# pyranha-labs/hypergrep

Measured on AMD Instinct MI355X. Metric: GiB/s scanned (256 patterns, 32 GiB synthetic log per GPU, text resident in HBM), higher is better.
Workload: dtype u8

## Files before the change

### hypergrep_amd/csrc/hg_compile.cpp

```cpp
#include "hg_compile.h"
#include "hg_comb.h"
#include "hg_core.h"

#include <algorithm>
#include <array>
#include <bitset>
#include <cmath>
#include <cstdlib>
#include <cstring>
#include <map>
#include <memory>
#include <stdexcept>
#include <unordered_map>

namespace {

using ByteSet = std::bitset<256>;

constexpr int kThisExpression = -2;
struct CompileError : std::runtime_error {
  int index;
  explicit CompileError(const std::string &what, int index = kThisExpression) : std::runtime_error(what), index(index) {}
};

// ... 650 lines not shown
  }
  return 0;
}

struct Cond { uint32_t pos, tt; };
struct Frag {
  uint32_t nullable = 0;
  std::vector<Cond> first, last;
};
struct Edge { uint32_t p, q, tt; };

class Glushkov {
 public:
  std::vector<ByteSet> pos_class;
  std::vector<Edge> edges;

  Frag build(const Node &n) {
    switch (n.kind) {
      case Node::Empty: { Frag f; f.nullable = HG_TT_ALL; return f; }
      case Node::Assert: { Frag f; f.nullable = n.tt; return f; }
      case Node::Class: {
        if (pos_class.size() >= HG_HUGE_MAX_NODES) throw CompileError("pattern too large");
        uint32_t p = static_cast<uint32_t>(pos_class.size());
        pos_class.push_back(n.cls);
        Frag f;
        f.first.push_back({p, HG_TT_ALL});
        f.last.push_back({p, HG_TT_ALL});
        return f;
      }
      case Node::Cat: {
        Frag acc;
        acc.nullable = HG_TT_ALL;
        for (auto &k : n.kids) acc = cat(std::move(acc), build(*k));
        return acc;
      }
      case Node::Alt: {
        Frag acc = build(*n.kids[0]);
        for (size_t i = 1; i < n.kids.size(); i++) acc = alt(std::move(acc), build(*n.kids[i]));
        return acc;
      }
      case Node::Rep: {
        const Node &k = *n.kids[0];
        const bool strip = nullable_tt(k) == HG_TT_ALL;
        auto copy = [&]() {
          Frag f = build(k);
          if (strip) f.nullable = 0;
          return f;
        };
        const int mn = strip ? 0 : n.min;
        Frag acc;
        acc.nullable = HG_TT_ALL;
        for (int i = 0; i < mn; i++) acc = cat(std::move(acc), copy());
        if (n.max < 0) {
          Frag loop = copy();
          link(loop.last, loop.first);
          loop.nullable = HG_TT_ALL;
          acc = cat(std::move(acc), std::move(loop));
        } else if (n.max > mn) {
          Frag opt;
          opt.nullable = HG_TT_ALL;
          for (int i = mn; i < n.max; i++) {
            opt = cat(std::move(opt), copy());
            opt.nullable = HG_TT_ALL;
          }
          acc = cat(std::move(acc), std::move(opt));
        }
        return acc;
      }
    }
    return Frag();
  }

 private:
  void link(const std::vector<Cond> &from, const std::vector<Cond> &to) {
    if (edges.size() + from.size() * to.size() > HG_HUGE_MAX_EDGES) throw CompileError("pattern too large");
    for (auto &l : from)
      for (auto &f : to) {
        uint32_t tt = l.tt & f.tt;
        if (tt) edges.push_back({l.pos, f.pos, tt});
      }
  }
  Frag cat(Frag a, Frag b) {
    link(a.last, b.first);
    Frag r;
    r.nullable = a.nullable & b.nullable;
    r.first = std::move(a.first);
    if (a.nullable)
      for (auto &f : b.first)
        if (f.tt & a.nullable) r.first.push_back({f.pos, f.tt & a.nullable});
    r.last = std::move(b.last);
    if (b.nullable)
      for (auto &l : a.last)
        if (l.tt & b.nullable) r.last.push_back({l.pos, l.tt & b.nullable});
    return r;
  }
  static Frag alt(Frag a, Frag b) {
    Frag r = std::move(a);
    r.nullable |= b.nullable;
    r.first.insert(r.first.end(), b.first.begin(), b.first.end());
    r.last.insert(r.last.end(), b.last.begin(), b.last.end());
    return r;
  }
};

struct Lit {
  std::string bytes, cmask;
  bool operator<(const Lit &o) const { return std::tie(bytes, cmask) < std::tie(o.bytes, o.cmask); }
  bool operator==(const Lit &o) const { return bytes == o.bytes && cmask == o.cmask; }
};
using LitSet = std::vector<Lit>;
constexpr size_t MAX_EXACT = 16;
constexpr size_t MAX_EXACT_LEN = 96;

struct Info {
  bool exact = false;
  LitSet set;
  bool has_cover = false;
  LitSet cover;
  long lead = 0;
};
long add_len(long a, long b) {
  if (a < 0 || b < 0 || a + b > (1 << 20)) return -1;
  return a + b;
}

int byte_commonness(unsigned char b) {
  if (b == ' ') return 10;
  if (b >= 'a' && b <= 'z') return std::strchr("etaoinsrhl", b) ? 8 : 5;
  if (b >= '0' && b <= '9') return 6;
  if (std::strchr("=:-./_", b)) return 4;
  if (b >= 'A' && b <= 'Z') return 2;
  if (b > 32 && b < 127) return 2;
  return 1;
}
size_t min_len(const LitSet &s) {
  size_t m = SIZE_MAX;
  for (auto &l : s) m = std::min(m, l.bytes.size());
  return s.empty() ? 0 : m;
}
void dedupe(LitSet &s) {
  std::sort(s.begin(), s.end());
  s.erase(std::unique(s.begin(), s.end()), s.end());
}
bool better_cover(const LitSet &a, const LitSet &b) {
  size_t ma = std::min<size_t>(min_len(a), 16), mb = std::min<size_t>(min_len(b), 16);
  if (ma != mb) return ma > mb;
  if (a.size() != b.size()) return a.size() < b.size();
  return min_len(a) > min_len(b);
}
void offer(Info &info, const LitSet &cand, long lead) {
  if (cand.empty() || min_len(cand) == 0 || cand.size() > MAX_EXACT) return;
  if (!info.has_cover || better_cover(cand, info.cover)) {
    info.has_cover = true;
    info.cover = cand;
    info.lead = lead;
  }
}
bool cross(const LitSet &a, const LitSet &b, LitSet &out) {
  if (a.size() * b.size() > MAX_EXACT) return false;
  out.clear();
  for (auto &x : a)
    for (auto &y : b) {
      if (x.bytes.size() + y.bytes.size() > MAX_EXACT_LEN) return false;
      out.push_back({x.bytes + y.bytes, x.cmask + y.cmask});
    }
  dedupe(out);
  return true;
}

Info analyze(const Node &n) {
  Info r;
  switch (n.kind) {
    case Node::Empty: case Node::Assert:
      r.exact = true;
      r.set.push_back({"", ""});
      return r;
    case Node::Class: {
      size_t cnt = n.cls.count();
      ByteSet folded;
      for (int b = 0; b < 256; b++) if (n.cls[b]) folded.set((b >= 'A' && b <= 'Z') ? b + 32 : b);
      bool case_closed = true;
      for (int b = 'a'; b <= 'z'; b++) if (n.cls[b] != n.cls[b - 32]) case_closed = false;
      if (cnt <= 10 || (case_closed && folded.count() <= 10)) {
        r.exact = true;
        for (int b = 0; b < 256; b++) {
          if (!n.cls[b]) continue;
          if (b >= 'A' && b <= 'Z' && n.cls[b + 32]) continue;
          bool both = b >= 'a' && b <= 'z' && n.cls[b - 32];
          r.set.push_back({std::string(1, static_cast<char>(b)), std::string(1, static_cast<char>(both ? 0xDF : 0xFF))});
        }
      }
      return r;
    }
    case Node::Cat: {
      LitSet run{{"", ""}};
      bool all_exact = true;
      long before = 0;
      long run_lead = 0;
      auto flush = [&]() {
        offer(r, run, run_lead);
        run = LitSet{{"", ""}};
      };
      for (auto &k : n.kids) {
        Info ki = analyze(*k);
        const long after = add_len(before, max_match_len(*k));
        if (ki.has_cover) offer(r, ki.cover, add_len(before, ki.lead));
        if (ki.exact) {
          LitSet next;
          if (cross(run, ki.set, next)) run = std::move(next);
          else {
            all_exact = false;
            flush();
            run = ki.set;
            run_lead = before;
            if (run.size() > MAX_EXACT) { run = LitSet{{"", ""}}; run_lead = after; }
          }
        } else {
          all_exact = false;
          flush();
          run_lead = after;
        }
        before = after;
      }
      if (all_exact) { r.exact = true; r.set = run; }
      offer(r, run, run_lead);
      return r;
    }
    case Node::Alt: {
      bool all_exact = true, all_cover = true;
      LitSet uni, cov;
      long cov_lead = 0;
      for (auto &k : n.kids) {
        Info ki = analyze(*k);
        if (ki.exact) { uni.insert(uni.end(), ki.set.begin(), ki.set.end()); }
        else all_exact = false;
        const LitSet *c = ki.has_cover ? &ki.cover : (ki.exact && min_len(ki.set) > 0 ? &ki.set : nullptr);
        if (ki.exact && ki.has_cover && min_len(ki.set) > 0 && better_cover(ki.set, ki.cover)) c = &ki.set;
        if (c) {
          cov.insert(cov.end(), c->begin(), c->end());
          const long l = c == &ki.cover ? ki.lead : 0;
          cov_lead = (cov_lead < 0 || l < 0) ? -1 : std::max(cov_lead, l);
        }
        else all_cover = false;
      }
      dedupe(uni);
      dedupe(cov);
      if (all_exact && uni.size() <= MAX_EXACT) { r.exact = true; r.set = uni; }
      if (all_cover) offer(r, cov, cov_lead);
      if (r.exact) offer(r, r.set, 0);
      return r;
    }
    case Node::Rep: {
      Info ki = analyze(*n.kids[0]);
      if (ki.exact && n.min == n.max && n.min <= 64) {
        LitSet acc{{"", ""}};
        bool ok = true;
        for (int i = 0; i < n.min && ok; i++) {
          LitSet next;
          ok = cross(acc, ki.set, next);
          if (ok) acc = std::move(next);
        }
        if (ok) { r.exact = true; r.set = acc; offer(r, acc, 0); return r; }
      }
      if (n.min >= 1) {
        if (ki.has_cover) offer(r, ki.cover, ki.lead);
        if (ki.exact) {
          LitSet acc{{"", ""}};
          for (int i = 0; i < std::min(n.min, 32); i++) {
            LitSet next;
            if (!cross(acc, ki.set, next)) break;
            acc = std::move(next);
          }
          offer(r, acc, 0);
        }
      }
      return r;
    }
  }
  return r;
}

Lit clip(const Lit &l, size_t *offset = nullptr) {
  if (offset) *offset = 0;
  if (l.bytes.size() <= HG_FACTOR_MAX) return l;
  size_t best = 0;
  int best_score = INT32_MAX;
  for (size_t o = 0; o + HG_FACTOR_MAX <= l.bytes.size(); o++) {
    int s = 0;
    for (size_t i = 0; i < HG_FACTOR_MAX; i++) s += byte_commonness(static_cast<unsigned char>(l.bytes[o + i]));
    if (s < best_score) { best_score = s; best = o; }
  }
  if (offset) *offset = best;
  return {l.bytes.substr(best, HG_FACTOR_MAX), l.cmask.substr(best, HG_FACTOR_MAX)};
}

struct SampleStats {
  std::unordered_map<uint32_t, uint32_t> c4;
  std::unordered_map<uint64_t, uint32_t> c6;
  size_t dwords = 0;
};

int build_filter(HgDb &db, const SampleStats *stats, std::string *err) {
  db.windows.clear();
  std::vector<std::pair<uint32_t, HgWindow>> keyed;
  std::vector<uint32_t> next16_of;
  const uint32_t fold = db.fold_mask;
  const uint32_t wbytes = db.window_bytes, wmask = db.window_mask;
  std::unordered_map<uint32_t, uint32_t> contenders;
  for (uint32_t fi = 0; fi < db.nreal_factors; fi++) {
    const HgFactor &fct = db.factors[fi];
    std::vector<uint32_t> mine;
    for (uint32_t o = 0; o + wbytes <= fct.len; o++) {
      uint32_t v = 0;
      std::memcpy(&v, fct.lit + o, wbytes);
      mine.push_back((v | fold) & wmask);
    }
    std::sort(mine.begin(), mine.end());
    mine.erase(std::unique(mine.begin(), mine.end()), mine.end());
    for (uint32_t v : mine) contenders[v]++;
  }
  auto variants = [&](const HgFactor &fct, uint32_t o, std::vector<uint32_t> &out) {
    uint32_t v = 0;
    std::memcpy(&v, fct.lit + o, wbytes);
    out.assign(1, (v | fold) & wmask);
    if (fold) return;
    for (uint32_t b = 0; b < wbytes; b++)
      if ((fct.casebits >> (o + b)) & 1u) {
        const size_t have = out.size();
        for (size_t i = 0; i < have; i++) out.push_back(out[i] ^ (0x20u << (8 * b)));
      }
  };
  std::vector<uint32_t> vars;
  for (uint32_t fi = 0; fi < db.nreal_factors; fi++) {
    const HgFactor &fct = db.factors[fi];
    Lit l{std::string(reinterpret_cast<const char *>(fct.lit), fct.len), std::string(fct.len, '\xFF')};
    for (uint32_t b = 0; b < fct.len; b++) l.cmask[b] = static_cast<char>(hg_factor_cmask(fct, b));
    if (db.dense && fct.len < wbytes) {
      std::vector<uint32_t> seen;
      for (uint32_t last = 0; last < 256; last++) {
        uint32_t v = 0;
        std::memcpy(&v, fct.lit, fct.len);
        v = ((v | (last << 24)) | fold) & wmask;
        if (std::find(seen.begin(), seen.end(), v) != seen.end()) continue;
        seen.push_back(v);
        keyed.push_back({hg_hash_window(v), HgWindow{v, fi << 8}});
        next16_of.push_back(0);
      }
      continue;
    }
    const uint32_t step = db.dense ? db.dense : 4u;
    for (uint32_t res = 0; res < step; res++) {
      int best = -1;
      long best_cost = 0;
      uint32_t best_shared = 0;
      int best_sel = -1;
      for (uint32_t o = res; o + wbytes <= fct.len; o += step) {
        uint32_t v = 0;
        std::memcpy(&v, fct.lit + o, wbytes);
        v = (v | fold) & wmask;
        long cost = 0;
        if (stats) {
          variants(fct, o, vars);
          for (uint32_t x : vars) {
            auto it = stats->c4.find(x);
            cost += it == stats->c4.end() ? 0 : it->second;
          }
        }
        const uint32_t shared = contenders[v] > 1 ? contenders[v] : 0;
        int sel = 0;
        for (int j = static_cast<int>(o); j < static_cast<int>(o + wbytes); j++) sel += 11 - byte_commonness(static_cast<unsigned char>(l.bytes[j]));
        for (int j = std::max(static_cast<int>(o) - 4, 0); j < std::min<int>(o + 7, fct.len); j++)
          sel += (11 - byte_commonness(static_cast<unsigned char>(l.bytes[j]))) / 4;
        if (best < 0 || cost < best_cost || (cost == best_cost && (shared < best_shared || (shared == best_shared && sel > best_sel)))) {
          best = static_cast<int>(o);
          best_cost = cost;
          best_shared = shared;
          best_sel = sel;
        }
      }
      if (best < 0) continue;
      variants(fct, static_cast<uint32_t>(best), vars);
      for (uint32_t x : vars) {
        keyed.push_back({hg_hash_window(x), HgWindow{x, (fi << 8) | static_cast<uint32_t>(best)}});
        next16_of.push_back(0);
      }
    }
  }
  {
    std::vector<size_t> order(keyed.size());
    for (size_t i = 0; i < order.size(); i++) order[i] = i;
    std::stable_sort(order.begin(), order.end(), [&](size_t x, size_t y) { return keyed[x].first < keyed[y].first; });
    std::vector<std::pair<uint32_t, HgWindow>> k2;
    std::vector<uint32_t> n2;
    for (size_t i : order) { k2.push_back(keyed[i]); n2.push_back(next16_of[i]); }
    keyed.swap(k2);
    next16_of.swap(n2);
  }
  db.bucket_off.assign((1u << HG_HASH_BITS) + 1, 0);
  for (auto &kw : keyed) {
    db.bucket_off[kw.first + 1]++;
    db.windows.push_back(kw.second);
  }
  for (size_t i = 1; i < db.bucket_off.size(); i++) db.bucket_off[i] += db.bucket_off[i - 1];
  if (db.windows.empty()) db.windows.push_back(HgWindow{0, 0});

  {
    db.disc.assign(size_t(1) << HG_HASH_BITS, 0);
    std::vector<std::pair<uint32_t, HgWindow>> keyed2;
    for (size_t g0 = 0; g0 < keyed.size();) {
      size_t g1 = g0;
      while (g1 < keyed.size() && keyed[g1].first == keyed[g0].first) g1++;
      const uint32_t h = keyed[g0].first;
      int best_delta = 0;
      uint32_t best_sel = 0;
      size_t best_distinct = 1;
      auto key_of = [&](const HgWindow &w, int delta, uint32_t sel) {
        const HgFactor &fct = db.factors[w.factor_off >> 8];
        const int at = static_cast<int>(w.factor_off & 0xff) + delta;
        uint32_t v = 0;
        for (int b = 0; b < 4; b++)
          if ((sel >> b) & 1u) v |= static_cast<uint32_t>(fct.lit[at + b]) << (8 * b);
        return (v | fold) & hg_disc_bytes(sel);
      };
      if (g1 - g0 > 2) {
        for (int delta = -16; delta <= 28; delta += 4) {
          if (delta == 0) continue;
          uint32_t sel = 15;
          for (size_t e = g0; e < g1; e++) {
            const HgFactor &fct = db.factors[keyed[e].second.factor_off >> 8];
            const int at = static_cast<int>(keyed[e].second.factor_off & 0xff) + delta;
            for (int b = 0; b < 4; b++) {
              if (at + b < 0 || at + b >= static_cast<int>(fct.len)) sel &= ~(1u << b);
              else if (!fold && hg_factor_cmask(fct, at + b) != 0xFF) sel &= ~(1u << b);
            }
          }
          if (!sel) continue;
          std::vector<uint32_t> ks;
          for (size_t e = g0; e < g1; e++) ks.push_back(key_of(keyed[e].second, delta, sel));
          std::sort(ks.begin(), ks.end());
          const size_t distinct = static_cast<size_t>(std::unique(ks.begin(), ks.end()) - ks.begin());
          if (distinct > best_distinct || (distinct == best_distinct && distinct > 1 && std::abs(delta) < std::abs(best_delta))) {
            best_distinct = distinct;
            best_delta = delta;
            best_sel = sel;
          }
        }
      }
      db.disc[h] = static_cast<uint16_t>((static_cast<uint32_t>(best_delta) & 0xFFu) | (best_sel << 8));
      for (size_t e = g0; e < g1; e++)
        keyed2.push_back({hg_disc_bucket(h, best_sel ? key_of(keyed[e].second, best_delta, best_sel) : 0u), keyed[e].second});
      g0 = g1;
    }
    std::stable_sort(keyed2.begin(), keyed2.end(), [](const auto &x, const auto &y) { return x.first < y.first; });
    db.bucket_off2.assign((1u << HG_HASH_BITS) + 1, 0);
    db.windows2.clear();
    for (auto &kw : keyed2) {
      db.bucket_off2[kw.first + 1]++;
      db.windows2.push_back(kw.second);
    }
    for (size_t i = 1; i < db.bucket_off2.size(); i++) db.bucket_off2[i] += db.bucket_off2[i - 1];
    if (db.windows2.empty()) db.windows2.push_back(HgWindow{0, 0});
  }

  {
    std::vector<std::pair<uint32_t, uint32_t>> vf;
    for (auto &kw : keyed) vf.push_back({kw.second.value, kw.second.factor_off});
    std::sort(vf.begin(), vf.end());
    vf.erase(std::unique(vf.begin(), vf.end()), vf.end());
    size_t distinct = 0;
    for (size_t i = 0; i < vf.size(); i++) distinct += (i == 0 || vf[i].first != vf[i - 1].first) ? 1 : 0;
    uint32_t nbuckets = 16;
    while (static_cast<size_t>(nbuckets) * HG_WTAB_WAYS < 2 * distinct) nbuckets <<= 1;
    HgWinBucket empty;
    for (uint32_t k = 0; k < HG_WTAB_WAYS; k++) { empty.value[k] = 0; empty.factor_off[k] = HG_WTAB_EMPTY; }
    db.wtab.assign(nbuckets, empty);
    db.wtab_mask = nbuckets - 1;
    db.shared_windows = 0;
    for (size_t i = 0; i < vf.size();) {
      size_t j = i;
      while (j < vf.size() && vf[j].first == vf[i].first) j++;
      const uint32_t payload = j - i == 1 ? vf[i].second : HG_WTAB_SHARED;
      db.shared_windows += j - i == 1 ? 0 : 1;
      for (uint32_t b = hg_wtab_bucket(vf[i].first, db.wtab_mask);; b = (b + 1u) & db.wtab_mask) {
        bool placed_here = false;
        for (uint32_t k = 0; k < HG_WTAB_WAYS && !placed_here; k++)
          if (db.wtab[b].factor_off[k] == HG_WTAB_EMPTY) {
            db.wtab[b].value[k] = vf[i].first;
            db.wtab[b].factor_off[k] = payload;
            placed_here = true;
          }
        if (placed_here) break;
      }
      i = j;
    }
    db.wtab_first = (distinct > 0 && static_cast<size_t>(db.shared_windows) * 20 <= distinct) ? 1u : 0u;
  }

  std::vector<uint32_t> values;
  for (auto &kw : keyed) values.push_back(kw.second.value);
  std::sort(values.begin(), values.end());
  values.erase(std::unique(values.begin(), values.end()), values.end());
  bool placed = false;
  {
    std::vector<uint32_t> cand_weights;
    for (uint32_t i = 0; i < HG_SLOT_WEIGHT_NCHOICES; i++) {
      cand_weights.push_back(HG_SLOT_WEIGHT_CHOICES[i][0] & wmask);
      cand_weights.push_back(HG_SLOT_WEIGHT_CHOICES[i][1] & wmask);
    }
    auto slot_words = [&](uint32_t k, uint32_t weights, std::vector<uint32_t> &words) -> double {
      const uint32_t byte_mask = ((1u << k) - 1u) << 2;
      words.assign(size_t(1) << k, HG_FILTER_EMPTY);
      std::vector<uint8_t> used(size_t(1) << k, 0);
      for (uint32_t v : values) {
        const uint32_t sl = hg_slot(v, weights, byte_mask) >> 2, fp = hg_hash_window(v) & 0xFFFFu;
        uint32_t &w = words[sl];
        if (!used[sl]) {
          w = 0xFFFF0000u | fp;
          used[sl] = 1;
        } else {
          const uint32_t care = (w >> 16) & ~((w ^ fp) & 0xFFFFu);
          w = (care << 16) | (w & care);
        }
      }
      double fp_rate = 0;
      for (size_t sl = 0; sl < words.size(); sl++)
        if (used[sl]) fp_rate += std::ldexp(1.0, -static_cast<int>(__builtin_popcount(words[sl] >> 16)));
      return fp_rate / static_cast<double>(words.size());
    };
    double best_rate = 1e9;
    uint32_t best_k = 0, best_w = 0;
    for (uint32_t k = HG_FILTER_MIN_LOG2; k <= HG_FILTER_MAX_LOG2 && !placed; k++) {
      if (values.size() > (size_t(1) << k)) continue;
      double k_rate = 1e9;
      uint32_t k_w = 0;
      for (uint32_t weights : cand_weights) {
        std::vector<uint32_t> words;
        const double rate = slot_words(k, weights, words);
        if (rate < k_rate) { k_rate = rate; k_w = weights; }
      }
      if (k_rate < best_rate) { best_rate = k_rate; best_k = k; best_w = k_w; }
      if (k_rate <= (k <= 12 ? 5e-4 : 3e-4)) {
        best_rate = k_rate;
        best_k = k;
        best_w = k_w;
        placed = true;
      }
    }
    if (!placed && best_k && best_rate <= 2e-3 && values.size() * 100 <= (size_t(1) << HG_FILTER_MAX_LOG2) * 45) placed = true;
    if (placed) {
      const uint32_t k = best_k, wa = best_w;
      const uint32_t byte_mask = ((1u << k) - 1u) << 2;
      slot_words(k, wa, db.filter);
      db.ext.assign(size_t(1) << k, HgSlotInfo{});
      db.filter_log2 = k;
      db.weights_a = wa;
      db.weights_b = wa;
      auto merge = [](uint32_t &val, uint32_t &mask, uint32_t v2, uint32_t m2) {
        uint32_t keep = 0;
        for (int b = 0; b < 4; b++) {
          uint32_t bm = 0xFFu << (8 * b);
          if ((mask & bm) && (m2 & bm) && ((val ^ v2) & bm) == 0) keep |= bm;
        }
        mask = keep;
        val &= keep;
      };
      for (size_t wi = 0; wi < keyed.size(); wi++) {
        const HgWindow &w = keyed[wi].second;
        const HgFactor &f = db.factors[w.factor_off >> 8];
        const int o = static_cast<int>(w.factor_off & 0xff);
        uint32_t pv = 0, pm = 0, nv = 0, nm = 0;
        for (int b = 0; b < 4; b++) {
          int jp = o - 4 + b, jn = o + static_cast<int>(wbytes) + b;
          if (jp >= 0) { pv |= static_cast<uint32_t>(f.lit[jp]) << (8 * b); pm |= 0xFFu << (8 * b); }
          if (jn < static_cast<int>(f.len)) { nv |= static_cast<uint32_t>(f.lit[jn]) << (8 * b); nm |= 0xFFu << (8 * b); }
        }
        pv = (pv | fold) & pm;
        nv = (nv | fold) & nm;
        if (!fold) {
          for (int b = 0; b < 4; b++) {
            int jp = o - 4 + b, jn = o + static_cast<int>(wbytes) + b;
            if (jp >= 0 && hg_factor_cmask(f, jp) != 0xFF) { pm &= ~(0xFFu << (8 * b)); pv &= pm; }
            if (jn < static_cast<int>(f.len) && hg_factor_cmask(f, jn) != 0xFF) { nm &= ~(0xFFu << (8 * b)); nv &= nm; }
          }
        }
        HgSlotInfo &info = db.ext[hg_slot(w.value, wa, byte_mask) >> 2];
        HgFilterExt *x = nullptr;
        bool fresh = false;
        for (uint32_t i = 0; i < info.nvalues; i++)
          if (info.value[i] == w.value) x = &info.cond[i];
        if (!x && info.nvalues < 2) {
          info.value[info.nvalues] = w.value;
          x = &info.cond[info.nvalues++];
          fresh = true;
        }
        if (!x) {
          x = &info.rest;
          fresh = !info.many;
          info.many = 1;
        }
        if (fresh) {
          *x = HgFilterExt{pv, pm, nv, nm};
        } else {
          merge(x->pv, x->pm, pv, pm);
          merge(x->nv, x->nm, nv, nm);
        }
      }
    }
  }
  db.filter_wide = 0;
  if (!placed && db.dense) {
    if (err) *err = "too many literal windows for byte-aligned probing";
    return -5;
  }
  if (!placed) {
    for (uint32_t attempt = 0; attempt < 3 * HG_SLOT_WEIGHT_NCHOICES && !placed; attempt++) {
      const uint32_t k = 13 + attempt / HG_SLOT_WEIGHT_NCHOICES;
      const uint32_t wa = HG_SLOT_WEIGHT_CHOICES[attempt % HG_SLOT_WEIGHT_NCHOICES][0], wb = HG_SLOT_WEIGHT_CHOICES[attempt % HG_SLOT_WEIGHT_NCHOICES][1];
      const size_t cells = size_t(2) << k;
      if (values.size() * 100 > cells * 85) continue;
      const uint32_t byte_mask = ((1u << k) - 1u) << 2;
      struct WEntry { uint32_t sa, sb; uint16_t fp; };
      std::vector<WEntry> entries;
      {
        std::vector<std::array<uint32_t, 3>> keys;
        for (uint32_t v : values) {
          const uint32_t a = hg_dot4(v, wa), b = hg_dot4(v, wb);
          const uint32_t sa = hg_slot_wide(a, b, byte_mask) >> 2, sb = hg_slot_wide(b, a, byte_mask) >> 2;
          keys.push_back({std::min(sa, sb), std::max(sa, sb), hg_hash_window(v) & 0xFFFFu});
        }
        std::sort(keys.begin(), keys.end());
        keys.erase(std::unique(keys.begin(), keys.end()), keys.end());
        for (auto &key : keys) entries.push_back({key[0], key[1], static_cast<uint16_t>(key[2])});
      }
      std::vector<int32_t> owner(cells, -1);
      uint64_t rng = 0x9E3779B97F4A7C15ull;
      placed = true;
      for (size_t e = 0; e < entries.size() && placed; e++) {
        int32_t cur = static_cast<int32_t>(e);
        bool ok = false;
        for (int kick = 0; kick < 8000 && !ok; kick++) {
          const uint32_t cand[4] = {entries[cur].sa * 2, entries[cur].sa * 2 + 1, entries[cur].sb * 2, entries[cur].sb * 2 + 1};
          for (uint32_t cell : cand)
            if (owner[cell] < 0) { owner[cell] = cur; ok = true; break; }
          if (ok) break;
          rng = rng * 6364136223846793005ull + 1442695040888963407ull;
          std::swap(cur, owner[cand[(rng >> 33) & 3]]);
        }
        if (!ok) placed = false;
      }
      if (!placed) continue;
      db.filter.assign(size_t(1) << k, HG_FILTER_EMPTY);
      for (size_t cell = 0; cell < cells; cell++) {
        if (owner[cell] < 0) continue;
        uint32_t &word = db.filter[cell >> 1];
        const uint32_t fp = entries[owner[cell]].fp;
        word = (cell & 1) ? ((word & 0x0000FFFFu) | (fp << 16)) : ((word & 0xFFFF0000u) | fp);
      }
      db.ext.assign(1, HgSlotInfo{});
      db.filter_log2 = k;
      db.filter_wide = 1;
      db.weights_a = wa;
      db.weights_b = wb;
    }
  }
  if (!placed) {
    if (err) *err = "too many distinct literal windows for the LDS filter (more than ~55 000)";
    return -4;
  }
  return 0;
}

struct CompileKnobs {
  bool no_ctx_groups = std::getenv("HG_NO_CTX_GROUPS") != nullptr;
  bool no_case_expand = std::getenv("HG_NO_CASE_EXPAND") != nullptr;
};

struct CombProgram {
  std::vector<uint32_t> ops;
  std::vector<uint32_t> prog;
};

CombProgram parse_combination(const std::string &text) {
  CombProgram out;
  std::vector<char> stack;
  auto prec = [](char c) { return c == '!' ? 3 : c == '&' ? 2 : c == '|' ? 1 : 0; };
  auto emit = [&](char c) { out.prog.push_back(c == '!' ? HG_COMB_NOT : c == '&' ? HG_COMB_AND : HG_COMB_OR); };
  bool want_operand = true;
  bool any = false;
  for (size_t i = 0; i < text.size();) {
    const char c = text[i];
    if (c == ' ' || c == '\t' || c == '\n' || c == '\r' || c == '\f' || c == '\v') {
      i++;
      continue;
    }
    any = true;
    if (c >= '0' && c <= '9') {
      if (!want_operand) throw CompileError("combination: two operands without an operator between them");
      uint64_t v = 0;
      for (; i < text.size() && text[i] >= '0' && text[i] <= '9'; i++) {
        v = v * 10 + static_cast<uint64_t>(text[i] - '0');
        if (v > 0xFFFFFFFFull) throw CompileError("combination: operand id above 4294967295 (UINT32_MAX)");
      }
      const uint32_t id = static_cast<uint32_t>(v);
      auto it = std::find(out.ops.begin(), out.ops.end(), id);
      if (it == out.ops.end()) {
        if (out.ops.size() == HG_COMB_MAX_OPERANDS)
          throw CompileError("combination: more than " + std::to_string(HG_COMB_MAX_OPERANDS) + " distinct operands (the limit is " +
                             std::to_string(HG_COMB_MAX_OPERANDS) + ")");
        out.ops.push_back(id);
        it = out.ops.end() - 1;
      }
      out.prog.push_back(static_cast<uint32_t>(it - out.ops.begin()));
      want_operand = false;
      continue;
    }
    i++;
    if (c == '!' || c == '(') {
      if (!want_operand) throw CompileError(std::string("combination: '") + c + "' after an operand (missing operator)");
      stack.push_back(c);
    } else if (c == '&' || c == '|') {
      if (want_operand) throw CompileError(std::string("combination: dangling operator '") + c + "'");
      while (!stack.empty() && stack.back() != '(' && prec(stack.back()) >= prec(c)) {
        emit(stack.back());
        stack.pop_back();
      }
      stack.push_back(c);
      want_operand = true;
    } else if (c == ')') {
      if (want_operand) throw CompileError(stack.empty() || stack.back() != '(' ? "combination: dangling operator before ')'" : "combination: empty parentheses");
      while (!stack.empty() && stack.back() != '(') {
        emit(stack.back());
        stack.pop_back();
      }
      if (stack.empty()) throw CompileError("combination: unbalanced parentheses (')' without '(')");
      stack.pop_back();
    } else {
      throw CompileError(std::string("combination: unexpected character '") + c + "' (operands are decimal report ids, operators ! & | and parentheses)");
    }
  }
  if (!any) throw CompileError("combination: empty formula");
  if (want_operand) throw CompileError("combination: dangling operator at the end");
  while (!stack.empty()) {
    if (stack.back() == '(') throw CompileError("combination: unbalanced parentheses ('(' without ')')");
    emit(stack.back());
    stack.pop_back();
  }
  long depth = 0, most = 0;
  for (uint32_t op : out.prog) {
    depth += op < HG_COMB_NOT ? 1 : op == HG_COMB_NOT ? 0 : -1;
    most = std::max(most, depth);
  }
  if (most > 64) throw CompileError("combination: more than 64 values on the evaluation stack (parentheses nested too deeply)");
  return out;
}

void build_slow_groups(HgDb &db, const CompileKnobs &knobs) {
  db.groups.clear();
  db.nslow_grouped = 0;
  const bool mixed = !knobs.no_ctx_groups;
  struct Bin { std::vector<uint32_t> members; uint32_t nodes = 0; bool ctx = false; };
  std::vector<Bin> bins;
  for (int pass = 0; pass < 2; pass++) {
    for (uint32_t j = 0; j < db.nslow_fast; j++) {
      const HgPattern &p = db.patterns[db.slow[j]];
      if (p.nw != 1 || p.nnodes == 0 || (p.simple != 0) != (pass == 1)) continue;
      if (pass == 0 && !mixed) continue;
      Bin *home = nullptr;
      for (Bin &b : bins)
        if (b.nodes + p.nnodes <= 32 && b.members.size() < HG_GROUP_MAX_MEMBERS) { home = &b; break; }
      if (!home) { bins.emplace_back(); home = &bins.back(); home->ctx = pass == 0; }
      home->members.push_back(db.slow[j]);
      home->nodes += p.nnodes;
    }
  }
  std::vector<uint32_t> grouped;
  for (const Bin &b : bins) {
    if (b.members.size() < 2) continue;
    HgSlowGroup g{};
    db.pool.resize((db.pool.size() + 3) & ~static_cast<size_t>(3), 0);
    g.reach_off = static_cast<uint32_t>(db.pool.size());
    db.pool.resize(db.pool.size() + 256, 0);
    g.follow_off = static_cast<uint32_t>(db.pool.size());
    db.pool.resize(db.pool.size() + b.nodes, 0);
    if (b.ctx) {
      g.ctx_off = static_cast<uint32_t>(db.pool.size());
      db.pool.resize(db.pool.size() + 36, 0);
    }
    g.nnodes = b.nodes;
    g.nmembers = static_cast<uint32_t>(b.members.size());
    bool unbounded = false;
    uint32_t shift = 0;
    for (uint32_t m = 0; m < g.nmembers; m++) {
      const HgPattern &p = db.patterns[b.members[m]];
      const uint32_t all = (p.nnodes == 32 ? 0xFFFFFFFFu : ((1u << p.nnodes) - 1u)) << shift;
      g.member[m] = b.members[m];
      g.acc[m] = b.ctx ? all : p.acc_all << shift;
      g.acc_all |= g.acc[m];
      g.init_word |= db.pool[p.init_off] << shift;
      if (p.single) g.single_mask |= 1u << m;
      if (p.max_len == 0) unbounded = true;
      g.max_len = std::max(g.max_len, p.max_len);
      for (uint32_t c = 0; c < 256; c++) db.pool[g.reach_off + c] |= db.pool[p.reach_off + c] << shift;
      for (uint32_t v = 0; v < p.nnodes; v++) db.pool[g.follow_off + shift + v] = db.pool[p.follow_off + v] << shift;
      if (b.ctx) {
        for (uint32_t i = 0; i < 16; i++) db.pool[g.ctx_off + i] |= db.pool[p.amask_off + i] << shift;
        for (uint32_t i = 0; i < 20; i++) db.pool[g.ctx_off + 16 + i] |= db.pool[p.acc_off + i] << shift;
      }
      shift += p.nnodes;
      grouped.push_back(b.members[m]);
    }
    if (unbounded) g.max_len = 0;
    db.groups.push_back(g);
  }
  if (grouped.empty()) return;
  std::vector<uint32_t> rest_fast, rest_slow;
  for (uint32_t j = 0; j < db.slow.size(); j++) {
    const uint32_t pi = db.slow[j];
    if (std::find(grouped.begin(), grouped.end(), pi) != grouped.end()) continue;
    (j < db.nslow_fast ? rest_fast : rest_slow).push_back(pi);
  }
  db.slow = grouped;
  db.slow.insert(db.slow.end(), rest_fast.begin(), rest_fast.end());
  db.slow.insert(db.slow.end(), rest_slow.begin(), rest_slow.end());
  db.nslow_grouped = static_cast<uint32_t>(grouped.size());
}

uint32_t alloc(HgDb &db, size_t words) {
  if (db.pool.size() + words > 0xFFFF0000ull) throw CompileError("pattern set too large");
  const uint32_t off = static_cast<uint32_t>(db.pool.size());
  db.pool.resize(db.pool.size() + words, 0);
  return off;
}
void setbit(HgDb &db, uint32_t base, uint32_t node) { db.pool[base + node / 32] |= 1u << (node % 32); }

HgPattern compile_combination(HgDb &db, const char *expr, uint32_t f, uint32_t id, CombProgram &program) {
  if (!expr || !expr[0]) throw CompileError("empty expression");
  db.exprs.push_back(expr);
  program = parse_combination(expr);
  if (hg_comb_eval(program.prog.data(), static_cast<uint32_t>(program.prog.size()), 0))
    throw CompileError("combination is true when none of its operands has matched: such combinations report at the end of the data, which is not supported");
  HgPattern p{};
  p.id = id;
  p.flags = f & (HG_FLAG_COMBINATION | HG_FLAG_SINGLEMATCH | HG_FLAG_QUIET);
  p.single = (f & HG_FLAG_SINGLEMATCH) ? 1 : 0;
  p.tier = HG_TIER_COMB;
  db.ncomb++;
  return p;
}

struct Automaton {
  NodeP root;
  Glushkov g;
  std::vector<Cond> first;
  std::vector<std::pair<uint32_t, uint32_t>> nodes;
  std::vector<uint32_t> node_lo;
  std::vector<uint32_t> last_tt;
  uint32_t nn = 0, nw = 1;
  uint32_t node(uint32_t pos, uint32_t tt) const {
    return static_cast<uint32_t>(std::lower_bound(nodes.begin(), nodes.end(), std::make_pair(pos, tt)) - nodes.begin());
  }
};

void index_nodes(Automaton &a, std::vector<Cond> first, const std::vector<Cond> &last) {
  std::vector<Edge> &edges = a.g.edges;
  std::sort(edges.begin(), edges.end(), [](const Edge &x, const Edge &y) { return x.p != y.p ? x.p < y.p : x.q < y.q; });
  size_t ne = 0;
  for (size_t i = 0; i < edges.size(); i++) {
    if (ne && edges[ne - 1].p == edges[i].p && edges[ne - 1].q == edges[i].q) edges[ne - 1].tt |= edges[i].tt;
    else edges[ne++] = edges[i];
  }
  edges.resize(ne);
  a.nodes.reserve(first.size() + edges.size());
  for (auto &c : first) a.nodes.push_back({c.pos, c.tt});
  for (auto &e : edges) a.nodes.push_back({e.q, e.tt});
  std::sort(a.nodes.begin(), a.nodes.end());
  a.nodes.erase(std::unique(a.nodes.begin(), a.nodes.end()), a.nodes.end());
  if (a.nodes.size() > HG_HUGE_MAX_NODES) throw CompileError("pattern too large");
  const uint32_t npos = static_cast<uint32_t>(a.g.pos_class.size());
  a.node_lo.assign(npos + 1, 0);
  for (auto &nd : a.nodes) a.node_lo[nd.first + 1]++;
  for (uint32_t q = 0; q < npos; q++) a.node_lo[q + 1] += a.node_lo[q];
  a.last_tt.assign(npos, 0);
  for (auto &l : last) a.last_tt[l.pos] |= l.tt;
  a.first = std::move(first);
  a.nn = static_cast<uint32_t>(a.nodes.size());
  a.nw = a.nn ? (a.nn + 31) / 32 : 1;
}

Automaton build_automaton(const std::string &text, uint32_t flags) {
  Automaton a;
  a.root = Parser(text, flags).parse();
  check_embedded_anchors(*a.root, false, false);
  if (program_size(*a.root) > HG_HUGE_MAX_PROGRAM) throw CompileError("pattern too large");
  Frag top = a.g.build(*a.root);
  if (a.g.pos_class.empty() && !top.nullable) throw CompileError("expression matches nothing");
  if (nullable_syntactic(*a.root)) throw CompileError("expression can match the empty string (HS_FLAG_ALLOWEMPTY is not supported)");
  index_nodes(a, std::move(top.first), top.last);
  return a;
}

constexpr uint64_t HG_EXT_FLAGS_KNOWN = HS_EXT_FLAG_MIN_OFFSET | HS_EXT_FLAG_MAX_OFFSET | HS_EXT_FLAG_MIN_LENGTH | HS_EXT_FLAG_EDIT_DISTANCE |
                                        HS_EXT_FLAG_HAMMING_DISTANCE;
constexpr uint32_t HG_EXT_MAX_DISTANCE = 16;

long min_match_len(const Node &n) {
  const long kCap = 1 << 20;
  switch (n.kind) {
    case Node::Empty:
    case Node::Assert: return 0;
// ... 345 lines not shown
    for (size_t j = 0; j <= k; j++) {
      const size_t lo = len * j / (k + 1), hi = len * (j + 1) / (k + 1);
      if (hi - lo < HG_DENSE_MIN_FACTOR) return Cover{};
      cover.lits.push_back(clip(Lit{l.bytes.substr(lo, hi - lo), l.cmask.substr(lo, hi - lo)}));
    }
  }
  dedupe(cover.lits);
  if (cover.lits.size() > MAX_EXACT) return Cover{};
  return cover;
}

void emit_som_follow(HgDb &db, HgPattern &p, bool som) {
  if (p.nw > HG_MAX_W)
    throw CompileError("HS_FLAG_SOM_LEFTMOST needs an automaton of at most " + std::to_string(HG_MAX_NODES) + " nodes (HG_MAX_NODES); this expression has " +
                       std::to_string(p.nnodes));
  p.som_follow_off = alloc(db, static_cast<size_t>(p.nnodes) * p.nw);
  for (uint32_t v = 0; v < p.nnodes; v++)
    for (uint32_t w = 0; w < p.nw; w++)
      for (uint32_t x = db.pool[p.follow_off + v * p.nw + w]; x; x &= x - 1) setbit(db, p.som_follow_off + (w * 32 + hg_ctz(x)) * p.nw, v);
  if (som) db.nsom++;
}

void link_som_ids(HgDb &db) {
  if (!db.nsom) return;
  std::map<uint32_t, uint32_t> last;
  std::map<uint32_t, uint32_t> first_plain;
  for (uint32_t i = 0; i < db.patterns.size(); i++) {
    HgPattern &p = db.patterns[i];
    if (!(p.flags & HG_FLAG_SOM_LEFTMOST)) {
      first_plain.emplace(p.id, i);
      continue;
    }
    auto it = last.find(p.id);
    if (it == last.end()) {
      p.som_next = i;
    } else {
      p.som_next = db.patterns[it->second].som_next;
      db.patterns[it->second].som_next = i;
    }
    last[p.id] = i;
  }
  for (auto &kv : last) {
    auto it = first_plain.find(kv.first);
    if (it != first_plain.end())
      throw CompileError("expressions with report id " + std::to_string(kv.first) + " must all carry HS_FLAG_SOM_LEFTMOST, or none of them",
                         static_cast<int>(std::max(it->second, kv.second)));
  }
}

void link_combinations(HgDb &db, const std::map<uint32_t, CombProgram> &programs) {
  if (!db.comb_pass()) return;
  std::map<uint32_t, std::pair<uint32_t, bool>> plain;
  std::map<uint32_t, uint32_t> comb_of;
  for (uint32_t i = 0; i < db.patterns.size(); i++) {
    const HgPattern &p = db.patterns[i];
    if (p.tier == HG_TIER_COMB) continue;
    const bool quiet = (p.flags & HG_FLAG_QUIET) != 0;
    auto ins = plain.emplace(p.id, std::make_pair(i, quiet));
    if (!ins.second && ins.first->second.second != quiet)
      throw CompileError("expressions with report id " + std::to_string(p.id) + " must all carry HS_FLAG_QUIET, or none of them", static_cast<int>(i));
  }
  for (uint32_t i = 0; i < db.patterns.size(); i++) {
    const HgPattern &p = db.patterns[i];
    if (p.tier != HG_TIER_COMB) continue;
    if (plain.count(p.id) || !comb_of.emplace(p.id, i).second)
      throw CompileError("combination report id " + std::to_string(p.id) + " is shared with another expression (a combination's id must be unique)",
                         static_cast<int>(i));
  }
  std::vector<std::pair<uint32_t, uint32_t>> feed;
  for (auto &kv : programs) {
    const uint32_t i = kv.first;
    const int at = static_cast<int>(i);
    const HgPattern &p = db.patterns[i];
    const CombProgram &cp = kv.second;
    for (uint32_t id : cp.ops) {
      if (id == p.id) throw CompileError("combination refers to its own report id " + std::to_string(id), at);
      if (comb_of.count(id))
        throw CompileError("combination refers to report id " + std::to_string(id) + " of another combination (nested combinations are not supported)", at);
      if (!plain.count(id)) throw CompileError("combination refers to report id " + std::to_string(id) + ", which no expression in the set has", at);
    }
    if (p.flags & HG_FLAG_QUIET) continue;
    HgComb c{};
    c.id = p.id;
    c.pattern = i;
    c.single = p.single;
    c.nops = static_cast<uint32_t>(cp.ops.size());
    c.ops_off = static_cast<uint32_t>(db.comb_words.size());
    db.comb_words.insert(db.comb_words.end(), cp.ops.begin(), cp.ops.end());
    c.prog_off = static_cast<uint32_t>(db.comb_words.size());
    c.prog_len = static_cast<uint32_t>(cp.prog.size());
    db.comb_words.insert(db.comb_words.end(), cp.prog.begin(), cp.prog.end());
    for (uint32_t id : cp.ops) feed.emplace_back(id, static_cast<uint32_t>(db.combs.size()));
    db.combs.push_back(c);
  }
  std::sort(feed.begin(), feed.end());
  for (auto &f : feed) db.comb_feed.push_back(f.first);
  for (auto &f : feed) db.comb_feed.push_back(f.second);
}

int assign_tiers(HgDb &db, const std::vector<Cover> &covers, const CompileKnobs &knobs, uint32_t min_factor, uint32_t dense,
                 uint32_t window_bytes, std::string *err) {
  db.dense = dense;
  db.window_bytes = window_bytes;
  db.window_mask = window_bytes == 4 ? 0xFFFFFFFFu : 0x00FFFFFFu;
  db.weights_c = HG_HASH_WEIGHTS & db.window_mask;
  db.slow.clear();
  db.factors.clear();
  db.fold_mask = 0;
  size_t ncaseless = 0;
  for (uint32_t m = 0; m < HG_CONFIRM_MODES; m++) db.n_confirm_mode[m] = 0;
  for (uint32_t i = 0; i < db.patterns.size(); i++) {
    HgPattern &p = db.patterns[i];
    if (p.tier == HG_TIER_COMB) continue;
    const LitSet &lits = covers[i].lits;
    const bool fast = !lits.empty() && min_len(lits) >= min_factor;
    p.tier = fast ? 0 : 1;
    p.literal_only = (fast && covers[i].literal_only) ? 1 : 0;
    if (fast) {
      db.n_confirm_mode[hg_confirm_mode(p)]++;
      for (auto &l : lits) {
        bool caseless = false;
        for (unsigned char m : l.cmask) caseless = caseless || m != 0xFF;
        ncaseless += caseless ? 1 : 0;
      }
    } else {
      db.slow.push_back(i);
    }
  }
  if (ncaseless) {
    const bool expand = !dense && !knobs.no_case_expand && ncaseless <= 64;
    db.fold_mask = expand ? 0u : 0x20202020u;
  }
  auto two_words = [&](uint32_t pi) { return db.patterns[pi].nw <= 2; };
  auto not_huge = [&](uint32_t pi) { return db.patterns[pi].nw <= HG_MAX_W; };
  std::stable_partition(db.slow.begin(), db.slow.end(), not_huge);
  std::stable_partition(db.slow.begin(), db.slow.end(), two_words);
  db.nslow_fast = static_cast<uint32_t>(std::count_if(db.slow.begin(), db.slow.end(), two_words));
  db.nslow_huge = static_cast<uint32_t>(db.slow.size() - std::count_if(db.slow.begin(), db.slow.end(), not_huge));
  build_slow_groups(db, knobs);
  uint32_t rank_in_mode[HG_CONFIRM_MODES] = {};
  for (uint32_t i = 0; i < db.patterns.size(); i++) {
    if (db.patterns[i].tier != 0) continue;
    const uint32_t mode = hg_confirm_mode(db.patterns[i]), rank = rank_in_mode[mode]++;
    for (auto &l : covers[i].lits) {
      HgFactor fct{};
      fct.pattern = i;
      fct.len = static_cast<uint32_t>(l.bytes.size());
      fct.mode = mode;
      fct.mode_rank = rank;
      std::memcpy(fct.lit, l.bytes.data(), fct.len);
      for (uint32_t b = 0; b < fct.len; b++)
        if (static_cast<unsigned char>(l.cmask[b]) != 0xFF) fct.casebits |= 1u << b;
      fct.id = db.patterns[i].id;
      db.factors.push_back(fct);
    }
  }
  db.nreal_factors = static_cast<uint32_t>(db.factors.size());
  if (db.factors.empty()) db.factors.push_back(HgFactor{});
  return build_filter(db, nullptr, err);
}

void choose_windows(HgDb &db, const std::vector<Cover> &covers, const CompileKnobs &knobs) {
  std::string msg;
  auto assign = [&](size_t min_factor, uint32_t dense, uint32_t window_bytes) {
    return assign_tiers(db, covers, knobs, static_cast<uint32_t>(min_factor), dense, window_bytes, &msg);
  };
  size_t shortest = SIZE_MAX;
  for (const Cover &c : covers) {
    const size_t m = c.lits.empty() ? 0 : min_len(c.lits);
    if (m >= HG_DENSE_MIN_FACTOR && m < HG_FAST_MIN_FACTOR) shortest = std::min(shortest, m);
  }
  int rc = -5;
  if (shortest != SIZE_MAX) {
    size_t set_shortest = SIZE_MAX;
    for (const Cover &c : covers)
      if (!c.lits.empty() && min_len(c.lits) >= shortest) set_shortest = std::min(set_shortest, min_len(c.lits));
    const uint32_t step = set_shortest >= HG_WINDOW_BYTES + 1 ? 2u : 1u;
    rc = assign(shortest, step, HG_WINDOW_BYTES);
    if (rc == -5 && step == 2) rc = assign(shortest, 1, HG_WINDOW_BYTES);
    if (rc == -5 && shortest < HG_WINDOW_BYTES) rc = assign(shortest, 1, HG_WINDOW_BYTES - 1);
    if (rc == -5 && shortest < HG_WINDOW_BYTES) rc = assign(HG_WINDOW_BYTES, 1, HG_WINDOW_BYTES);
  }
  if (rc == -5) rc = assign(HG_FAST_MIN_FACTOR, 0, HG_WINDOW_BYTES);
  if (rc != 0) throw CompileError(msg, -1);
}

}

int hgc_compile(const char *const *exprs, const unsigned *flags, const unsigned *ids, unsigned n, HgDb **out,
               std::string *err, int *bad_index) {
  return hgc_compile_ext(exprs, flags, ids, nullptr, n, out, err, bad_index);
}

int hgc_compile_ext(const char *const *exprs, const unsigned *flags, const unsigned *ids, const hs_expr_ext_t *const *ext, unsigned n,
                    HgDb **out, std::string *err, int *bad_index) {
  if (bad_index) *bad_index = -1;
  if (out) *out = nullptr;
  if (!exprs || !out || n == 0) {
    if (err) *err = "invalid arguments: at least one expression is required";
    return -1;
  }
  const CompileKnobs knobs;
  auto db = std::make_unique<HgDb>();
  int at = -1;
  try {
    if (n > HG_MAX_PATTERNS) throw CompileError("too many expressions (limit 16777216)", -1);
    std::vector<Cover> covers(n);
    std::map<uint32_t, CombProgram> programs;
    std::map<uint32_t, std::pair<uint32_t, uint32_t>> bounds;
    std::map<uint32_t, uint32_t> min_lengths;
    for (at = 0; at < static_cast<int>(n); at++) {
      const uint32_t f = flags ? flags[at] : 0, id = ids ? ids[at] : 0;
      if (f & ~HG_FLAGS_SUPPORTED) throw CompileError("unsupported flag bits");
      const hs_expr_ext_t *x = (ext && ext[at] && ext[at]->flags) ? ext[at] : nullptr;
      if (x) check_ext_fields(*x, f);
      if (f & HG_FLAG_COMBINATION) {
        db->patterns.push_back(compile_combination(*db, exprs[at], f, id, programs[at]));
        db->max_id = std::max(db->max_id, id);
        continue;
      }
      if ((f & HG_FLAG_SOM_LEFTMOST) && (f & HG_FLAG_SINGLEMATCH))
        throw CompileError("HS_FLAG_SOM_LEFTMOST cannot be combined with HS_FLAG_SINGLEMATCH");
      if (!exprs[at] || !exprs[at][0]) throw CompileError("empty expression");
      db->exprs.push_back(exprs[at]);
      Automaton a = build_automaton(db->exprs.back(), f);
      const bool edit = x && (x->flags & HS_EXT_FLAG_EDIT_DISTANCE);
      const uint32_t k = !x ? 0u : edit ? x->edit_distance : ((x->flags & HS_EXT_FLAG_HAMMING_DISTANCE) ? x->hamming_distance : 0u);
      std::pair<uint32_t, uint32_t> bound{0u, HG_BOUND_NONE};
      uint32_t min_length = 0;
      if (x) bound = ext_bounds(*x, check_ext_width(*x, k, edit, min_match_len(*a.root), max_match_len(*a.root), a, &min_length));
      if (bound.first || bound.second != HG_BOUND_NONE) bounds[at] = bound;
      if (min_length) min_lengths[at] = min_length;
      if (k) a = expand_approx(a, k, edit, f);
      HgPattern p{};
      p.id = id;
      p.flags = f;
      p.nnodes = a.nn;
      p.nw = a.nw;
      p.single = (f & HG_FLAG_SINGLEMATCH) && !bound.first && !min_length ? 1 : 0;
      if (a.nw > HG_MAX_W) emit_huge_tables(*db, a, p);
      else emit_dense_tables(*db, a, p);
      set_simple_flags(*db, p);
      covers[at] = k ? approx_cover(*a.root, k, p) : literal_cover(*a.root, p);
      const long ml = max_match_len(*a.root);
      p.max_len = ml > 0 ? static_cast<uint32_t>(ml + (edit ? k : 0u)) : 0;
      if ((f & HG_FLAG_SOM_LEFTMOST) || min_length) emit_som_follow(*db, p, (f & HG_FLAG_SOM_LEFTMOST) != 0);
      if (f & HG_FLAG_QUIET) db->nquiet++;
      db->max_id = std::max(db->max_id, id);
      db->patterns.push_back(p);
    }
    at = -1;
    if (!bounds.empty()) {
      db->bounds.resize(2 * static_cast<size_t>(n));
      for (uint32_t i = 0; i < n; i++) {
        auto it = bounds.find(i);
        db->bounds[2 * i] = it == bounds.end() ? 0u : it->second.first;
        db->bounds[2 * i + 1] = it == bounds.end() ? HG_BOUND_NONE : it->second.second;
      }
    }
    if (!min_lengths.empty()) {
      db->min_lengths.assign(n, 0u);
      for (auto &kv : min_lengths) db->min_lengths[kv.first] = kv.second;
    }
    link_som_ids(*db);
    link_combinations(*db, programs);
    choose_windows(*db, covers, knobs);
  } catch (const CompileError &e) {
    if (err) *err = e.what();
    if (bad_index) *bad_index = e.index == kThisExpression ? at : e.index;
    return -4;
  } catch (const std::bad_alloc &) {
    if (err) *err = "out of memory";
    if (bad_index) *bad_index = at;
    return -2;
  }
  *out = db.release();
  return 0;
}

int hgc_tune(const HgDb *db, const uint8_t *sample, size_t nbytes, HgDb **out, std::string *err) {
  if (out) *out = nullptr;
  if (!db || !out || (!sample && nbytes)) return -1;
  SampleStats st;
  const uint32_t fold = db->fold_mask;
  for (size_t p = 0; p + 4 <= nbytes; p += db->dense ? db->dense : 4) {
    uint32_t w, nx = 0;
    std::memcpy(&w, sample + p, 4);
    if (p + 8 <= nbytes) std::memcpy(&nx, sample + p + 4, 4);
    w = (w | fold) & db->window_mask;
    nx |= fold;
    st.c4[w]++;
    st.c6[static_cast<uint64_t>(w) | (static_cast<uint64_t>(nx & 0xFFFFu) << 32)]++;
  }
  st.dwords = nbytes / 4;
  std::unique_ptr<HgDb> copy;
  try {
    copy = std::make_unique<HgDb>(*db);
  } catch (const std::bad_alloc &) {
    if (err) *err = "out of memory";
    return -2;
  }
  int rc = build_filter(*copy, &st, err);
  if (rc != 0) return rc;
  copy->tuned = true;
  *out = copy.release();
  return 0;
}

void hgc_free(HgDb *db) { delete db; }
```

### hypergrep_amd/csrc/hg_compile.h

```cpp
#pragma once
#include <cstdint>
#include <string>
#include <vector>

#include "../../include/hypergrep_amd.h"
#include "hg_core.h"
#include "hg_db.h"

struct HgDb {
  std::vector<HgPattern> patterns;
  std::vector<uint32_t> pool;
  std::vector<HgFactor> factors;
  uint32_t nreal_factors = 0;
  std::vector<HgWindow> windows;
  std::vector<uint32_t> bucket_off;
  std::vector<uint16_t> disc;
  std::vector<uint32_t> bucket_off2;
  std::vector<HgWindow> windows2;
  std::vector<HgWinBucket> wtab;
  uint32_t wtab_mask = 0;
  uint32_t shared_windows = 0;
  uint32_t wtab_first = 0;
  std::vector<uint32_t> filter;
  uint32_t filter_log2 = HG_FILTER_MIN_LOG2;
  uint32_t filter_wide = 0;
  uint32_t window_bytes = HG_WINDOW_BYTES;
  uint32_t window_mask = HG_WINDOW_MASK;
  uint32_t weights_c = HG_HASH_WEIGHTS;
  uint32_t dense = 0;
  uint32_t weights_a = HG_SLOT_WEIGHT_CHOICES[0][0], weights_b = HG_SLOT_WEIGHT_CHOICES[0][1];
  std::vector<HgSlotInfo> ext;
  std::vector<uint32_t> slow;
  uint32_t nslow_fast = 0;
  std::vector<HgSlowGroup> groups;
  uint32_t nslow_grouped = 0;
  uint32_t fold_mask = 0;
  uint32_t max_nw = 1;
  uint32_t nhuge = 0;
  uint32_t huge_max_nw = 0;
  uint32_t huge_stage_words = 0;
  uint32_t nslow_huge = 0;
  uint32_t max_id = 0;
  uint32_t nsom = 0;
  uint32_t ncomb = 0, nquiet = 0;
  std::vector<HgComb> combs;
  std::vector<uint32_t> comb_words;
  std::vector<uint32_t> comb_feed;
  bool comb_pass() const { return ncomb || nquiet; }
  std::vector<uint32_t> bounds;
  std::vector<uint32_t> min_lengths;
  uint32_t n_confirm_mode[HG_CONFIRM_MODES] = {};
  std::vector<std::string> exprs;
  bool tuned = false;
};

int hgc_tune(const HgDb *db, const uint8_t *sample, size_t nbytes, HgDb **out, std::string *err);


int hgc_compile(const char *const *exprs, const unsigned *flags, const unsigned *ids, unsigned n, HgDb **out,
               std::string *err, int *bad_index);
int hgc_compile_ext(const char *const *exprs, const unsigned *flags, const unsigned *ids, const hs_expr_ext_t *const *ext, unsigned n,
                    HgDb **out, std::string *err, int *bad_index);
void hgc_free(HgDb *db);
```

### hypergrep_amd/csrc/hg_db.h

```cpp
#pragma once
#include <cstdint>

#if defined(__HIPCC__)
#define HG_HD __host__ __device__ __forceinline__
#else
#define HG_HD inline
#endif

constexpr uint32_t HG_FLAG_CASELESS = 1, HG_FLAG_DOTALL = 2, HG_FLAG_MULTILINE = 4, HG_FLAG_SINGLEMATCH = 8;
constexpr uint32_t HG_FLAG_SOM_LEFTMOST = 256;
constexpr uint32_t HG_FLAG_COMBINATION = 512, HG_FLAG_QUIET = 1024;
constexpr uint32_t HG_FLAGS_SUPPORTED = 15 | HG_FLAG_SOM_LEFTMOST | HG_FLAG_COMBINATION | HG_FLAG_QUIET;

enum : uint32_t { HG_PC_START = 0, HG_PC_NL = 1, HG_PC_WORD = 2, HG_PC_OTHER = 3 };
enum : uint32_t { HG_NC_NL = 0, HG_NC_NLFINAL = 1, HG_NC_WORD = 2, HG_NC_OTHER = 3, HG_NC_END = 4 };
constexpr uint32_t HG_TT_ALL = (1u << 20) - 1;

constexpr uint32_t HG_MAX_NODES = 1024;
constexpr uint32_t HG_MAX_W = HG_MAX_NODES / 32;
constexpr uint32_t HG_HUGE_MAX_PROGRAM = 400000;
constexpr uint32_t HG_HUGE_MAX_NODES = 1u << 19;
constexpr uint32_t HG_HUGE_STAGE_MAX = 12288;
constexpr uint32_t HG_HUGE_MAX_EDGES = 1u << 22;
constexpr uint32_t HG_MAX_PATTERNS = 1u << 24;
constexpr uint32_t HG_ALWAYS_ON_FAST_MAX_LEN = 64;
constexpr uint32_t HG_FACTOR_MAX = 32;
constexpr uint32_t HG_WINDOW_BYTES = 4;
constexpr uint32_t HG_WINDOW_MASK = HG_WINDOW_BYTES == 4 ? 0xFFFFFFFFu : 0x00FFFFFFu;
constexpr uint32_t HG_FAST_MIN_FACTOR = HG_WINDOW_BYTES + 3;
constexpr uint32_t HG_DENSE_MIN_FACTOR = HG_WINDOW_BYTES - 1;
constexpr uint32_t HG_HASH_BITS = 18;
constexpr uint32_t HG_TOP_WEIGHT_MASK = HG_WINDOW_BYTES == 4 ? 0xFFFFFFFFu : 0x00FFFFFFu;
constexpr uint32_t HG_HASH_WEIGHTS = 0xfbf1efe9u & HG_TOP_WEIGHT_MASK;
constexpr uint32_t HG_SLOT_WEIGHT_CHOICES[][2] = {
    {0x2cec94fcu & HG_TOP_WEIGHT_MASK, 0xbc34f474u & HG_TOP_WEIGHT_MASK},
    {0x74d43cb4u & HG_TOP_WEIGHT_MASK, 0xe40c9c5cu & HG_TOP_WEIGHT_MASK},
    {0xa41cf86cu & HG_TOP_WEIGHT_MASK, 0x54c4247cu & HG_TOP_WEIGHT_MASK},
    {0xdc4484f4u & HG_TOP_WEIGHT_MASK, 0x1cac6cccu & HG_TOP_WEIGHT_MASK},
};
constexpr uint32_t HG_SLOT_WEIGHT_NCHOICES = 4;
constexpr uint32_t HG_FILTER_MIN_LOG2 = 11, HG_FILTER_MAX_LOG2 = 15;
constexpr uint32_t HG_FILTER_EMPTY = 0xFFFFFFFFu;

struct HgHugeHeader {
  uint32_t cls_off;
  uint32_t ncls;
  uint32_t smask_off;
  uint32_t xsrc_off;
  uint32_t xrank_off;
  uint32_t xlist_off;
  uint32_t xt_off;
  uint32_t ctxfree;
  uint32_t init_hi;
  uint32_t nsources, nranges;
  uint32_t reserved[5];
};
static_assert(sizeof(HgHugeHeader) == 64, "HgHugeHeader layout");

struct HgPattern {
  uint32_t id;
  uint32_t single;
  uint32_t max_len;
  uint32_t lit_lead;
  uint32_t flags;
  uint32_t nnodes;
  uint32_t nw;
  uint32_t reach_off;
  uint32_t follow_off;
  uint32_t init_off;
  uint32_t amask_off;
  uint32_t acc_off;
  uint32_t tier;
  uint32_t simple;
  uint32_t acc_all;
  uint32_t init_word;
  uint32_t literal_only;
  uint32_t som_follow_off;
  uint32_t som_next;
  uint32_t reserved;
};
static_assert(sizeof(HgPattern) == 80, "HgPattern layout");
HG_HD bool hg_report_single(const HgPattern &p) { return (p.flags & HG_FLAG_SINGLEMATCH) != 0; }

constexpr uint32_t HG_TIER_COMB = 2;

constexpr uint32_t HG_COMB_MAX_OPERANDS = 64;
constexpr uint32_t HG_COMB_NOT = 64, HG_COMB_AND = 65, HG_COMB_OR = 66;
struct HgComb {
  uint32_t id;
  uint32_t pattern;
  uint32_t single;
  uint32_t nops;
  uint32_t ops_off;
  uint32_t prog_off;
  uint32_t prog_len;
  uint32_t reserved;
};
static_assert(sizeof(HgComb) == 32, "HgComb layout");

struct HgFactor {
  uint32_t pattern;
  uint32_t len;
  uint32_t mode;
  uint32_t mode_rank;
  uint8_t lit[HG_FACTOR_MAX];
  uint32_t casebits;
  uint32_t id;
  uint32_t reserved[2];
};
static_assert(sizeof(HgFactor) == 64, "HgFactor layout");
HG_HD uint32_t hg_factor_cmask(const HgFactor &f, uint32_t b) { return ((f.casebits >> b) & 1u) ? 0xDFu : 0xFFu; }
HG_HD uint32_t hg_factor_mask_dword(uint32_t casebits, uint32_t len, uint32_t j) {
  const uint32_t nib = (casebits >> (4u * j)) & 15u;
  const uint32_t spread = (nib & 1u) | ((nib & 2u) << 7) | ((nib & 4u) << 14) | ((nib & 8u) << 21);
  const uint32_t m = ~(spread << 5);
  const uint32_t valid = len > 4u * j ? len - 4u * j : 0u;
  return valid >= 4u ? m : (m & ((1u << (8u * valid)) - 1u));
}

struct HgWinBucket {
  uint32_t value[4];
  uint32_t factor_off[4];
};
static_assert(sizeof(HgWinBucket) == 32, "HgWinBucket layout");
constexpr uint32_t HG_WTAB_WAYS = 4, HG_WTAB_EMPTY = 0xFFFFFFFFu, HG_WTAB_SHARED = 0xFFFFFFFEu;
HG_HD uint32_t hg_wtab_bucket(uint32_t folded, uint32_t bucket_mask) { return ((folded * 0x9E3779B1u) >> 9) & bucket_mask; }
HG_HD uint32_t hg_wtab_find(const HgWinBucket *tab, uint32_t bucket_mask, uint32_t folded) {
  for (uint32_t b = hg_wtab_bucket(folded, bucket_mask);; b = (b + 1u) & bucket_mask) {
    const HgWinBucket &e = tab[b];
    for (uint32_t k = 0; k < HG_WTAB_WAYS; k++) {
      if (e.factor_off[k] == HG_WTAB_EMPTY) return HG_WTAB_EMPTY;
      if (e.value[k] == folded) return e.factor_off[k];
    }
  }
}

struct HgWindow {
  uint32_t value;
  uint32_t factor_off;
};

constexpr uint32_t HG_GROUP_MAX_MEMBERS = 8;
struct HgSlowGroup {
  uint32_t reach_off;
  uint32_t follow_off;
  uint32_t nnodes, init_word, acc_all;
  uint32_t max_len;
  uint32_t nmembers;
  uint32_t single_mask;
  uint32_t member[HG_GROUP_MAX_MEMBERS];
  uint32_t acc[HG_GROUP_MAX_MEMBERS];
  uint32_t ctx_off;
  uint32_t reserved;
};
static_assert(sizeof(HgSlowGroup) == 104, "HgSlowGroup layout");

HG_HD uint32_t hg_dot4(uint32_t v, uint32_t w) {
#if defined(__HIP_DEVICE_COMPILE__)
  return __builtin_amdgcn_udot4(v, w, 0u, false);
#else
  return (v & 0xff) * (w & 0xff) + ((v >> 8) & 0xff) * ((w >> 8) & 0xff) + ((v >> 16) & 0xff) * ((w >> 16) & 0xff) + (v >> 24) * (w >> 24);
#endif
}
HG_HD uint32_t hg_hash_window(uint32_t folded) { return hg_dot4(folded, HG_HASH_WEIGHTS); }
HG_HD uint32_t hg_slot(uint32_t folded, uint32_t weights, uint32_t byte_mask) { return hg_dot4(folded, weights) & byte_mask; }
HG_HD bool hg_slot_match(uint32_t slot_word, uint32_t hash_c) { return (hash_c & (slot_word >> 16)) == (slot_word & 0xFFFFu); }
HG_HD uint32_t hg_slot_wide(uint32_t sum_x, uint32_t sum_y, uint32_t byte_mask) { return (sum_x + (sum_y << 8)) & byte_mask; }

struct HgFilterExt {
  uint32_t pv, pm;
  uint32_t nv, nm;
};
HG_HD bool hg_ext_pass(const HgFilterExt &e, uint32_t prev_folded, uint32_t next_folded) {
  return (((prev_folded ^ e.pv) & e.pm) | ((next_folded ^ e.nv) & e.nm)) == 0;
}

constexpr uint32_t HG_DISC_WEIGHTS_1 = 0xc5a36b1du, HG_DISC_WEIGHTS_2 = 0x3b9d47e1u;
HG_HD uint32_t hg_disc_bytes(uint32_t sel4) {
  return ((sel4 & 1u) ? 0xFFu : 0u) | ((sel4 & 2u) ? 0xFF00u : 0u) | ((sel4 & 4u) ? 0xFF0000u : 0u) | ((sel4 & 8u) ? 0xFF000000u : 0u);
}
HG_HD uint32_t hg_disc_bucket(uint32_t h, uint32_t masked_dword) {
  return (h ^ (hg_dot4(masked_dword, HG_DISC_WEIGHTS_1) + (hg_dot4(masked_dword, HG_DISC_WEIGHTS_2) << 7))) & ((1u << HG_HASH_BITS) - 1u);
}

struct HgSlotInfo {
  uint32_t value[2];
  uint32_t nvalues;
  uint32_t many;
  HgFilterExt cond[2];
  HgFilterExt rest;
};
static_assert(sizeof(HgSlotInfo) == 64, "HgSlotInfo layout");
HG_HD bool hg_slot_pass(const HgSlotInfo &s, uint32_t folded, uint32_t prev_folded, uint32_t next_folded, uint32_t pm_keep, uint32_t nm_keep) {
  HgFilterExt e;
  if (s.nvalues > 0 && s.value[0] == folded) e = s.cond[0];
  else if (s.nvalues > 1 && s.value[1] == folded) e = s.cond[1];
  else if (s.many) e = s.rest;
  else return false;
  e.pm &= pm_keep;
  e.nm &= nm_keep;
  return hg_ext_pass(e, prev_folded, next_folded);
}

HG_HD bool hg_is_word(uint32_t b) {
  return (b - '0' < 10u) || ((b | 0x20) - 'a' < 26u) || b == '_';
}
```

### hypergrep_amd/csrc/hg_engine.h

```cpp
#pragma once
#include <hip/hip_runtime.h>

#include <memory>
#include <string>

#include "../../include/hypergrep_amd.h"
#include "hg_compile.h"
#include "hg_core.h"
#include "hg_invert.h"
#include "hg_post.h"

#ifndef HG_STREAM_WG_WAVES
#define HG_STREAM_WG_WAVES 8
#endif
constexpr uint32_t HG_STREAM_WG_WAVES_DEFAULT = HG_STREAM_WG_WAVES;

constexpr uint32_t HG_CONFIRM_SPLIT = 4;
constexpr uint32_t HG_DEFER_SHARDS = 64;

struct HgDeferred {
  uint64_t pos;
  uint32_t pattern;
  uint32_t rank;
};
enum { HG_ST_MINLEN_KEPT = 16, HG_ST_FIN_TOTAL = 24, HG_ST_SELECTED = 28, HG_ST_FINAL = 32, HG_ST_WORDS = 36, HG_ST_ZERO_WORDS = 32,
       HG_ST_BLOCK_DONE = 40 };
enum { HG_CNT_CANDS = 0, HG_CNT_HITS = 1, HG_CNT_CAND_NEED = 2, HG_CNT_HIT_NEED = 3, HG_CNT_DEFER_NEED = 4,
       HG_CNT_HITS_WRAPPED = 5,
       HG_CNT_JOIN_TILES = 6,
       HG_CNT_WORDS = 8,
       HG_CNT_CURSOR0 = 64,
       HG_CNT_CURSORS = 64,
       HG_ST_ALLOC_WORDS = 128 };
constexpr uint32_t HG_STREAM_GRAB = 2 * HG_STREAM_WG_WAVES_DEFAULT;

constexpr uint32_t HG_FIN_MAX_BUCKETS = 1u << 22;
constexpr uint32_t HG_FIN_BUCKET_CAP = 4096;
constexpr uint32_t HG_FIN_MEDIUM_CAP = 512;

#ifndef HG_CONFIRM_THREADS
#define HG_CONFIRM_THREADS 128
#endif



struct HgStreamArgs {
  const uint8_t *text;
  uint64_t nbytes, tile_begin, tile_end;
  HgDbView db;
  const uint32_t *filter;
  const HgSlotInfo *ext;
  HgTileSum *sums;
  HgCand *cands;
  uint32_t *seg_count;
  uint32_t cand_seg_cap, filter_log2;
  uint32_t weights_a, weights_b;
  uint32_t filter_wide;
  uint32_t dense;
  uint32_t weights_c;
  uint32_t alone;
  uint32_t cursor_slot;
  uint32_t *counters;
};

struct HgConfirmArgs {
  const uint8_t *text;
  uint64_t nbytes, tile_begin, tile_end, bs1;
  HgDbView db;
  const HgTileSum *sums;
  const HgTileBase *bases;
  const HgCand *cands;
  const uint32_t *seg_count;
  HgHit *hits;
  HgHitAux *aux;
  HgHit *tmp_hits;
  HgHitAux *tmp_aux;
  HgDeferred *deferred;
  uint32_t *defer_count;
  uint32_t list_of_mode[HG_CONFIRM_MODES];
  uint32_t mode_present[HG_CONFIRM_MODES];
  uint32_t *always_count;
  uint32_t always_list_cap;
  uint32_t list_spread[HG_CONFIRM_MODES];
  uint32_t cand_seg_cap, hit_cap, hit_seg_cap, defer_shard_cap;
  uint32_t join_seg0, join_seg_cap;
  uint32_t hit_direct;
  uint32_t bucket_shift, bucket_cap;
  uint32_t *bucket_fill;
  uint32_t *counters;
  uint64_t own_lo, own_hi;
};
constexpr uint32_t HG_BLOCK_SMALL_POOL = 10240;
constexpr uint32_t HG_BLOCK_SLICED_MAX = 2047;
constexpr uint32_t HG_BLOCK_SLICED_WORDS = 64;
constexpr uint32_t HG_BLOCK_SMALL_MAX = 8192;
constexpr uint32_t HG_BLOCK_SMALL_SEG = 1024;
inline uint32_t hg_block_small_grouping(uint32_t npatterns, uint32_t *ppw) {
  *ppw = npatterns <= 32u * 64u ? 32u : 256u;
  return (npatterns + *ppw - 1) / *ppw;
}
constexpr uint32_t HG_HIT_REL_SHIFT = 40;
constexpr uint32_t HG_HIT_SINGLE_BIT = 0x80000000u;

struct HgScanOutput {
  uint64_t n_hits;
  uint64_t n_pieces;
  uint64_t n_cands;
  uint64_t n_raw_hits;
  const HgHit *d_hits;
  const HgHitAux *d_aux;
  float ms_stream;
  float ms_total;
  uint32_t reruns;
  uint32_t stream_launches;
  uint32_t joiner_launches;
  uint64_t joiner_tiles;
  const uint32_t *d_from;
  float ms_invert;
};

hipError_t hg_som_launch(const uint8_t *text, const HgHit *hits, const HgHitAux *aux, uint64_t n, const HgPattern *patterns, const uint32_t *pool, uint32_t max_nw,
                         const uint32_t *min_lengths, uint32_t *from, hipStream_t stream);
hipError_t hg_minlen_launch(const uint8_t *text, const HgHit *hits, const HgHitAux *aux, uint32_t n, const HgPattern *patterns, const uint32_t *pool, uint32_t max_nw,
                            const uint32_t *min_lengths, HgHit *out_hits, HgHitAux *out_aux, uint32_t *count, hipStream_t stream);

struct HgCombArgs {
  const HgHit *hits;
  const HgHitAux *aux;
  uint64_t n;
  const HgPattern *patterns;
  const HgComb *combs;
  const uint32_t *words;
  const uint32_t *feed;
  uint32_t nfeed;
  uint32_t *count;
  const uint64_t *pos;
  HgHit *out_hits;
  HgHitAux *out_aux;
};
hipError_t hg_comb_launch(const HgCombArgs &a, bool emit, hipStream_t stream);

hipError_t hg_invert_launch(const HgInvertArgs &a, bool write, uint32_t num_cus, hipStream_t stream);

struct HgEngineKnobs {
  uint64_t fin_target = 48;
  bool no_bucket_finalize = false;
  uint64_t chunk_tiles = 0;
  uint32_t max_chunks = 0;
  std::vector<double> chunk_weights;
  long stream_wgs_per_cu = 0;
  long joiner = -1;
  bool joiner_ahead = false;
  bool no_early_finalize = false;
  uint32_t confirm_mode_mask = 0x1F;
  long confirm_blocks_per_cu = 0;
  uint64_t hit_limit = 0;
  uint64_t cand_limit = 0;
  bool verbose = false;
  static HgEngineKnobs from_env();
};

class HgScanner {
 public:
  static int create(std::shared_ptr<const HgDb> db, int device, HgScanner **out, std::string *err);
  const std::shared_ptr<const HgDb> &database() const { return db_; }
  ~HgScanner();
  int scan(const void *d_text, uint64_t nbytes, int buffer_size, uint64_t line_base, hipStream_t stream, HgScanOutput *out, bool invert = false);
  int scan_block(const void *d_text, uint64_t nbytes, hipStream_t stream, HgScanOutput *out);
  uint32_t launch_block_small(const uint8_t *h_text, uint32_t nbytes, hipStream_t stream, HgHit *h_out, uint32_t *h_counts, uint32_t *h_flag, uint32_t seq);
  const std::string &last_error() const { return err_; }
  int device() const { return device_; }
  const HgDbView &view() const { return view_; }

 private:
  HgScanner() = default;
  int init();
  int ensure(uint64_t nbytes);
  int alloc_cands(uint64_t n);
  int alloc_hits(uint64_t n);
  int scan_impl(const void *d_text, uint64_t nbytes, int buffer_size, uint64_t line_base, bool block_mode, bool invert, hipStream_t stream, HgScanOutput *out);
  struct PassRange {
    uint64_t tile_lo, tile_hi, cs0, piece0, own_lo, own_hi;
    bool last;
  };
  int scan_segments(const uint8_t *text, uint64_t nbytes, uint64_t bs1, uint64_t line_base, hipStream_t stream, HgScanOutput *out, uint32_t nsegments);
  int run_fitting(const uint8_t *text, uint64_t nbytes, uint64_t bs1, uint64_t line_base, const PassRange &range, bool block_mode, hipStream_t stream, HgScanOutput *out);
  int run_once(const uint8_t *text, uint64_t nbytes, uint64_t bs1, uint64_t line_base, const PassRange &range, bool block_mode, hipStream_t stream, HgScanOutput *out);
  struct PassPlan;
  PassPlan plan_pass(const uint8_t *text, uint64_t nbytes, uint64_t bs1, uint64_t line_base, const PassRange &range, bool block_mode, hipStream_t stream) const;
  int alloc_fin(uint32_t nb, hipStream_t stream);
  int launch_stream(PassPlan &p, uint32_t c, HgScanOutput *out);
  int launch_side(PassPlan &p, uint32_t c);
  int finalize_last(PassPlan &p, uint32_t c);
  int launch_fin(const PassPlan &p, hipStream_t s, uint32_t lo, uint32_t hi, bool beside_stream = false);
  int regrow(const PassPlan &p, uint64_t n_raw);
  int finalize_compact(const HgHit *hits, const HgHitAux *aux, uint32_t n, uint32_t id_bits, uint32_t to_bits, uint64_t line_bound, hipStream_t stream);
  int comb_pass(HgScanOutput *out, uint64_t bs1, uint64_t line_bound, hipStream_t stream);
  int minlen_pass(const uint8_t *text, uint32_t *n, hipStream_t stream);
  int invert_pass(const uint8_t *text, uint64_t nbytes, uint64_t bs1, uint64_t line_base, hipStream_t stream, HgScanOutput *out);
  int huge_lds_error() { return error(HG_ERR_HIP, "the huge-automaton kernel cannot have its LDS"); }
  bool fail(hipError_t e, const char *what);
  int error(int rc, const std::string &what) { err_ = what; return rc; }

  HgEngineKnobs knobs_;
  int device_ = 0;
  int num_cus_ = 256;
  int stream_wgs_per_cu_ = 0;
  std::string err_;
  HgDbView view_{};
  std::shared_ptr<const HgDb> db_;
  void *d_disc_ = nullptr, *d_bucket2_ = nullptr, *d_windows2_ = nullptr, *d_groups_ = nullptr, *d_wtab_ = nullptr, *d_bounds_ = nullptr;
  void *d_patterns_ = nullptr, *d_pool_ = nullptr, *d_factors_ = nullptr, *d_windows_ = nullptr, *d_bucket_ = nullptr,
       *d_filter_ = nullptr, *d_ext_ = nullptr, *d_slow_ = nullptr;
  uint64_t cap_tiles_ = 0;
  uint32_t cand_cap_ = 0, hit_cap_ = 0;
  uint64_t chunk_limit_tiles_ = 0;
  uint32_t defer_spread_boost_ = 1;
  bool hit_direct_ = false;
  HgTileSum *d_sums_ = nullptr;
  HgTileBase *d_bases_ = nullptr, *d_block_base_ = nullptr, *d_final_ = nullptr;
  HgTileElem *d_agg_ = nullptr;
  HgCand *d_cands_ = nullptr;
  HgDeferred *d_deferred_ = nullptr;
  uint32_t *d_defer_count_ = nullptr;
  HgHit *d_hits_raw_ = nullptr, *d_hits_out_ = nullptr;
  HgHitAux *d_aux_raw_ = nullptr, *d_aux_out_ = nullptr;
  HgHit *d_acc_hits_ = nullptr;
  HgHitAux *d_acc_aux_ = nullptr;
  uint64_t acc_cap_ = 0;
  bool side_bound_ = false;
  uint64_t *d_key_a_ = nullptr, *d_key_b_ = nullptr;
  uint32_t *d_perm_a_ = nullptr, *d_perm_b_ = nullptr;
  uint8_t *d_keep_ = nullptr;
  uint32_t *d_counters_ = nullptr, *d_selected_ = nullptr, *d_seg_count_ = nullptr;
  uint32_t max_segs_ = 0;
  uint32_t *d_pflags_ = nullptr;
  void *d_temp_ = nullptr;
  size_t temp_bytes_ = 0;
  uint32_t *h_counters_ = nullptr;
  HgTileBase *h_final_ = nullptr;
  hipEvent_t ev_[4] = {nullptr, nullptr, nullptr, nullptr};
  static constexpr int kMaxChunks = 64;
  hipStream_t side_stream_ = nullptr;
  hipEvent_t ev_tile_done_ = nullptr;
  hipEvent_t ev_fin_early_ = nullptr;
  hipEvent_t ev_k1_begin_[kMaxChunks] = {}, ev_k1_end_[kMaxChunks] = {}, ev_side_done_[kMaxChunks] = {};
  uint32_t *d_fin_fill_ = nullptr, *d_fin_kept_ = nullptr, *d_fin_total_ = nullptr, *d_fin_big_ = nullptr;
  bool fin_fallback_ = false;
  uint32_t fin_alloc_ = 0;
  uint32_t fin_epoch_ = 0;
  uint64_t fin_expect_hits_ = 0;
  void *d_huge_claim_ = nullptr;
  uint64_t huge_claim_slots_ = 0;
  uint32_t *d_from_ = nullptr;
  uint64_t from_cap_ = 0;
  uint32_t som_max_nw_ = 0;
  uint32_t *d_min_lengths_ = nullptr;
  HgHit *d_minlen_hits_ = nullptr;
  HgHitAux *d_minlen_aux_ = nullptr;
  uint64_t minlen_cap_ = 0;
  uint32_t minlen_max_nw_ = 0;
  HgComb *d_combs_ = nullptr;
  uint32_t *d_comb_words_ = nullptr, *d_comb_feed_ = nullptr;
  uint32_t *d_comb_count_ = nullptr;
  uint64_t *d_comb_pos_ = nullptr;
  uint64_t comb_in_cap_ = 0;
  HgHit *d_comb_hits_ = nullptr;
  HgHitAux *d_comb_aux_ = nullptr;
  uint64_t comb_out_cap_ = 0;
  uint8_t *d_comb_temp_ = nullptr;
  size_t comb_temp_bytes_ = 0;
  uint64_t *d_inv_count_ = nullptr, *d_inv_pos_ = nullptr;
  uint64_t inv_tiles_cap_ = 0;
  uint8_t *d_inv_temp_ = nullptr;
  size_t inv_temp_bytes_ = 0;
  HgHit *d_inv_hits_ = nullptr;
  HgHitAux *d_inv_aux_ = nullptr;
  uint64_t inv_cap_ = 0;
  uint32_t *d_seg_count2_ = nullptr;
  HgCand *d_cands2_ = nullptr;
};
```

### hypergrep_amd/csrc/hg_engine.hip

```cpp
#include <algorithm>
#include <array>
#include <cstdio>
#include <cstdlib>
#include <cstring>
#include <memory>

#include "hg_engine.h"
#include "hg_mem.h"

#include <rocprim/rocprim.hpp>

bool hg_launch_stream(const HgStreamArgs &a, uint32_t grid, hipStream_t stream);
bool hg_launch_stream_join(const HgStreamArgs &a, uint32_t grid, hipStream_t stream);
int hg_stream_blocks_per_cu(uint32_t filter_log2, uint32_t filter_wide, uint32_t dense);
__global__ void hg_tile_reduce_kernel(const HgTileSum *sums, uint64_t tile_begin, uint64_t tile_end, uint64_t bs1, HgTileElem *agg);
__global__ void hg_tile_spine_kernel(const HgTileElem *agg, uint32_t nblocks, uint64_t bs1, HgTileBase *block_base, HgTileBase *state);
__global__ void hg_tile_apply_kernel(const HgTileSum *sums, uint64_t tile_begin, uint64_t tile_end, uint64_t bs1, const HgTileBase *block_base,
                                     HgTileBase *bases);
__global__ void hg_tile_inner_kernel(const uint8_t *text, HgTileSum *sums, uint64_t tile_begin, uint64_t tile_end, uint64_t bs1);
__global__ void hg_verify_kernel(HgConfirmArgs a);
__global__ void hg_confirm_fast_kernel(HgConfirmArgs a, uint32_t blocks_per_mode);
__global__ void hg_confirm_generic_kernel(HgConfirmArgs a);
__global__ void hg_always_on_kernel(HgConfirmArgs a, uint32_t first, uint32_t last);
__global__ void hg_always_on_fast_kernel(HgConfirmArgs a);
__global__ void hg_always_on_finish_kernel(HgConfirmArgs a);
__global__ void hg_block_mark_kernel(HgConfirmArgs a, uint32_t *pattern_flags);
__global__ void hg_block_scan_kernel(HgConfirmArgs a, const uint32_t *pattern_flags);
__global__ void hg_block_small_kernel(HgDbView db, const uint8_t *h_text, uint32_t length, HgHit *h_out, uint32_t seg_cap, uint32_t *h_counts, uint32_t *d_done,
                                      uint32_t *h_flag, uint32_t seq, uint32_t ppw);
__global__ void hg_reset_kernel(uint32_t *state, uint32_t state_words, HgTileBase *final_state, uint64_t carry_start, uint64_t first_piece, uint32_t *fill, uint32_t nb, uint32_t *defer_count,
                                uint32_t ndefer);
__global__ void hg_fin_sort_small_kernel(const HgHit *hits, uint32_t *idx, const uint32_t *fill, uint32_t b_lo, uint32_t b_hi, uint32_t cap, uint32_t id_bits,
                                         uint32_t to_bits, uint32_t *kept_count, uint32_t *big_list, uint32_t *big_count, uint32_t big_stride);
template <uint32_t LCAP, bool IN_LDS>
__global__ void hg_fin_sort_big_kernel(const HgHit *hits, uint32_t *idx, const uint32_t *fill, const uint32_t *big_list, const uint32_t *big_count, uint32_t cap,
                                       uint32_t id_bits, uint32_t to_bits, uint32_t *kept_count, uint32_t *overflow, uint64_t *scratch_key, uint32_t *scratch_idx);
template <uint32_t THREADS>
__global__ void hg_fin_scan_kernel(uint32_t *kept_count, uint32_t b_lo, uint32_t b_hi, uint32_t *total, const uint32_t *fill, uint32_t cap, uint32_t *part, uint32_t epoch);
__global__ void hg_confirm_literal_kernel(HgConfirmArgs a);
__global__ void hg_verify_lean_kernel(HgConfirmArgs a);
__global__ void hg_fin_gather_kernel(const HgHit *hits, const HgHitAux *aux, const uint32_t *idx, const uint32_t *kept_base, const uint32_t *total, uint32_t b_lo,
                                     uint32_t b_hi, uint32_t cap, HgHit *oh, HgHitAux *oa);
__global__ void hg_key_kernel(const HgHit *hits, const HgHitAux *aux, const HgPattern *patterns, uint32_t n, uint64_t *key, uint32_t *idx);
__global__ void hg_line_key_kernel(const HgHit *hits, const uint32_t *perm, uint32_t n, uint64_t *key);
__global__ void hg_offset_kernel(uint32_t *idx, uint32_t n, uint32_t add);
__global__ void hg_key_packed_kernel(const HgHit *hits, const HgHitAux *aux, const HgPattern *patterns, uint32_t n, uint32_t id_bits, uint32_t to_bits,
                                     uint64_t *key, uint32_t *idx);
__global__ void hg_keep_kernel(const HgHit *hits, const HgHitAux *aux, const uint32_t *perm, const HgPattern *patterns, uint32_t n, uint8_t *keep);
__global__ void hg_scatter_kernel(const HgHit *hits, const HgHitAux *aux, const uint32_t *perm, const uint8_t *keep, const uint32_t *pos, uint32_t n,
                                  HgHit *oh, HgHitAux *oa, uint32_t *count);

size_t hg_huge_lds_bytes(uint32_t nw_max, uint32_t stage_cap);
bool hg_launch_confirm_huge(const HgConfirmArgs &a, uint32_t grid, uint32_t nw_max, uint32_t stage_cap, void *claim, uint32_t claim_mask, hipStream_t stream);
bool hg_launch_always_on_huge(const HgConfirmArgs &a, uint32_t grid, uint32_t nw_max, uint32_t stage_cap, uint32_t first, uint32_t last, hipStream_t stream);
bool hg_launch_block_huge(const HgConfirmArgs &a, uint32_t grid, uint32_t nw_max, uint32_t stage_cap, const uint32_t *pattern_flags, hipStream_t stream);

namespace {
constexpr int TS_BLOCK_TILES = 1024;
constexpr int STREAM_WG_WAVES = HG_STREAM_WG_WAVES;

template <typename T>
hipError_t upload(void **dst, const std::vector<T> &src, const char *name) {
  size_t bytes = std::max<size_t>(src.size() * sizeof(T), 16);
  hipError_t e = hgmem::dev_alloc(dst, bytes, name);
  if (e != hipSuccess) return e;
  if (!src.empty()) e = hipMemcpy(*dst, src.data(), src.size() * sizeof(T), hipMemcpyHostToDevice);
  return e;
}
template <typename T>
hipError_t realloc_dev(T *&ptr, size_t count, const char *name) {
  hgmem::dev_free(ptr, name);
  ptr = nullptr;
  return hgmem::dev_alloc(&ptr, std::max<size_t>(count * sizeof(T), 16), name);
}
uint32_t bits_for(uint64_t v) {
  uint32_t b = 1;
  while (b < 64 && (v >> b)) b++;
  return b;
}
}

#define HG_TRY(call, what) \
  do { if (fail((call), what)) return HG_ERR_HIP; } while (0)

HgEngineKnobs HgEngineKnobs::from_env() {
  HgEngineKnobs k;
  auto num = [](const char *name, uint64_t dflt) -> uint64_t {
    const char *env = std::getenv(name);
    return env ? std::strtoull(env, nullptr, 10) : dflt;
  };
  k.fin_target = std::max<uint64_t>(4, num("HG_FIN_TARGET", 48));
  k.no_bucket_finalize = std::getenv("HG_NO_BUCKET_FINALIZE") != nullptr;
  k.chunk_tiles = num("HG_CHUNK_TILES", 0);
  k.max_chunks = static_cast<uint32_t>(std::min<uint64_t>(num("HG_MAX_CHUNKS", 0), 1u << 20));
  if (const char *env = std::getenv("HG_CHUNK_WEIGHTS")) {
    for (const char *q = env; *q;) {
      char *e = nullptr;
      const double v = std::strtod(q, &e);
      if (e == q) break;
      if (v > 0) k.chunk_weights.push_back(v);
      q = *e ? e + 1 : e;
    }
  }
  k.stream_wgs_per_cu = static_cast<long>(num("HG_STREAM_WGS_PER_CU", 0));
  if (const char *env = std::getenv("HG_JOINER")) k.joiner = std::max(0l, std::min(2l, std::strtol(env, nullptr, 10)));
  k.joiner_ahead = std::getenv("HG_JOINER_AHEAD") != nullptr;
  k.no_early_finalize = std::getenv("HG_NO_EARLY_FINALIZE") != nullptr;
#ifdef HG_PROFILE_CONFIRM
  if (const char *env = std::getenv("HG_DEBUG_CONFIRM_MODES")) k.confirm_mode_mask = static_cast<uint32_t>(std::strtoul(env, nullptr, 0));
#endif
  k.confirm_blocks_per_cu = static_cast<long>(std::min<uint64_t>(num("HG_CONFIRM_BLOCKS_PER_CU", 0), 16));
  k.hit_limit = num("HG_HIT_LIMIT", 0);
  k.cand_limit = num("HG_CAND_LIMIT", 0);
  k.verbose = std::getenv("HG_VERBOSE") != nullptr;
  return k;
}

bool HgScanner::fail(hipError_t e, const char *what) {
  if (e == hipSuccess) return false;
  err_ = std::string(what) + ": " + hipGetErrorString(e);
  return true;
}

int HgScanner::create(std::shared_ptr<const HgDb> db, int device, HgScanner **out, std::string *err) {
  *out = nullptr;
  std::unique_ptr<HgScanner> s(new HgScanner());
  s->device_ = device;
  s->db_ = std::move(db);
  if (int rc = s->init()) {
    if (err) *err = s->err_;
    return rc;
  }
  *out = s.release();
  return HG_OK;
}

int HgScanner::init() {
  if (!db_) return error(HG_ERR_ARG, "no database");
  int count = 0;
  const hipError_t e = hipGetDeviceCount(&count);
  if (e != hipSuccess || count == 0) return error(HG_ERR_HIP, std::string("no HIP device available (") + hipGetErrorString(e) + "); the scan path has no CPU fallback");
  if (device_ < 0 || device_ >= count) return error(HG_ERR_ARG, "device index out of range");
  knobs_ = HgEngineKnobs::from_env();
  const HgDb &db = *db_;
  HG_TRY(hipSetDevice(device_), "hipSetDevice");
  hipDeviceProp_t prop;
  HG_TRY(hipGetDeviceProperties(&prop, device_), "hipGetDeviceProperties");
  num_cus_ = prop.multiProcessorCount;
  HG_TRY(upload(&d_patterns_, db.patterns, "d_patterns_"), "upload patterns");
  HG_TRY(upload(&d_pool_, db.pool, "d_pool_"), "upload tables");
  HG_TRY(upload(&d_factors_, db.factors, "d_factors_"), "upload factors");
  HG_TRY(upload(&d_windows_, db.windows, "d_windows_"), "upload windows");
  HG_TRY(upload(&d_bucket_, db.bucket_off, "d_bucket_"), "upload buckets");
  HG_TRY(upload(&d_disc_, db.disc, "d_disc_"), "upload discriminators");
  HG_TRY(upload(&d_bucket2_, db.bucket_off2, "d_bucket2_"), "upload buckets");
  HG_TRY(upload(&d_windows2_, db.windows2, "d_windows2_"), "upload windows");
  HG_TRY(upload(&d_wtab_, db.wtab, "d_wtab_"), "upload window table");
  HG_TRY(upload(&d_filter_, db.filter, "d_filter_"), "upload filter");
  HG_TRY(upload(&d_ext_, db.ext, "d_ext_"), "upload filter conditions");
  HG_TRY(upload(&d_slow_, db.slow, "d_slow_"), "upload always-on list");
  HG_TRY(upload(&d_groups_, db.groups, "d_groups_"), "upload always-on groups");
  view_.patterns = static_cast<const HgPattern *>(d_patterns_);
  view_.pool = static_cast<const uint32_t *>(d_pool_);
  view_.factors = static_cast<const HgFactor *>(d_factors_);
  view_.windows = static_cast<const HgWindow *>(d_windows_);
  view_.bucket_off = static_cast<const uint32_t *>(d_bucket_);
  view_.disc = static_cast<const uint16_t *>(d_disc_);
  view_.bucket_off2 = static_cast<const uint32_t *>(d_bucket2_);
  view_.windows2 = static_cast<const HgWindow *>(d_windows2_);
  view_.wtab = static_cast<const HgWinBucket *>(d_wtab_);
  view_.wtab_mask = db.wtab_mask;
  view_.wtab_first = db.wtab_first;
  view_.slow = static_cast<const uint32_t *>(d_slow_);
  view_.npatterns = static_cast<uint32_t>(db.patterns.size());
  view_.nslow = static_cast<uint32_t>(db.slow.size());
  view_.nslow_fast = db.nslow_fast;
  view_.nslow_grouped = db.nslow_grouped;
  view_.nslow_huge = db.nslow_huge;
  view_.ngroups = static_cast<uint32_t>(db.groups.size());
  view_.groups = static_cast<const HgSlowGroup *>(d_groups_);
  if (!db.bounds.empty()) HG_TRY(upload(&d_bounds_, db.bounds, "d_bounds_"), "upload offset bounds");
  view_.bounds = static_cast<const uint32_t *>(d_bounds_);
  if (!db.min_lengths.empty()) HG_TRY(upload(reinterpret_cast<void **>(&d_min_lengths_), db.min_lengths, "d_min_lengths_"), "upload min_length");
  for (uint32_t i = 0; i < db.patterns.size(); i++) {
    const HgPattern &p = db.patterns[i];
    if (p.flags & HG_FLAG_SOM_LEFTMOST) som_max_nw_ = std::max(som_max_nw_, p.nw);
    if (!db.min_lengths.empty() && db.min_lengths[i]) minlen_max_nw_ = std::max(minlen_max_nw_, p.nw);
  }
  if (db.comb_pass()) {
    HG_TRY(upload(reinterpret_cast<void **>(&d_combs_), db.combs, "d_combs_"), "upload combinations");
    HG_TRY(upload(reinterpret_cast<void **>(&d_comb_words_), db.comb_words, "d_comb_words_"), "upload combinations");
    HG_TRY(upload(reinterpret_cast<void **>(&d_comb_feed_), db.comb_feed, "d_comb_feed_"), "upload combinations");
  }
  view_.fold_mask = db.fold_mask;
  view_.window_mask = db.window_mask;
  static_assert(HG_CNT_CURSORS == kMaxChunks, "one tile cursor per pipeline chunk");
  HG_TRY(hgmem::dev_alloc(&d_counters_, HG_ST_ALLOC_WORDS * 4, "d_state_"), "alloc state");
  HG_TRY(hipMemset(d_counters_, 0, HG_ST_ALLOC_WORDS * 4), "clear state");
  d_fin_total_ = d_counters_ + HG_ST_FIN_TOTAL;
  d_selected_ = d_counters_ + HG_ST_SELECTED;
  d_final_ = reinterpret_cast<HgTileBase *>(d_counters_ + HG_ST_FINAL);
  HG_TRY(hgmem::dev_alloc(&d_pflags_, db.patterns.size() * 4 + 16, "d_pflags_"), "alloc pattern flags");
  HG_TRY(hgmem::host_alloc(&h_counters_, (HG_CNT_WORDS + 4 + HG_DEFER_SHARDS) * 4, "h_counters_"), "alloc pinned");
  h_final_ = reinterpret_cast<HgTileBase *>(h_counters_ + HG_ST_FINAL);
  for (auto &ev : ev_) HG_TRY(hipEventCreate(&ev), "hipEventCreate");
  HG_TRY(hipStreamCreateWithFlags(&side_stream_, hipStreamNonBlocking), "hipStreamCreate");
  HG_TRY(hipEventCreateWithFlags(&ev_fin_early_, hipEventDisableTiming), "hipEventCreate");
  HG_TRY(hipEventCreateWithFlags(&ev_tile_done_, hipEventDisableTiming), "hipEventCreate");
  return HG_OK;
}

HgScanner::~HgScanner() {
  (void)hipSetDevice(device_);
  void *ptrs[] = {d_patterns_, d_pool_, d_factors_, d_windows_, d_bucket_, d_filter_, d_ext_, d_slow_, d_sums_, d_bases_, d_block_base_,
                  d_agg_, d_cands_, d_hits_raw_, d_hits_out_, d_aux_raw_, d_aux_out_,
                  d_key_a_, d_key_b_, d_perm_a_, d_perm_b_, d_keep_, d_counters_, d_temp_, d_seg_count_, d_pflags_, d_deferred_, d_defer_count_, d_seg_count2_, d_cands2_, d_disc_, d_bucket2_, d_windows2_, d_groups_, d_acc_hits_, d_acc_aux_, d_huge_claim_, d_wtab_, d_from_, d_fin_fill_, d_fin_kept_, d_fin_big_,
                  d_combs_, d_comb_words_, d_comb_feed_, d_comb_count_, d_comb_pos_, d_comb_hits_, d_comb_aux_, d_comb_temp_, d_bounds_,
                  d_min_lengths_, d_minlen_hits_, d_minlen_aux_, d_inv_count_, d_inv_pos_, d_inv_temp_, d_inv_hits_, d_inv_aux_};
  for (void *p : ptrs) hgmem::dev_free(p, "scanner");
  hgmem::host_free(h_counters_, "h_counters_");
  for (auto &ev : ev_)
    if (ev) (void)hipEventDestroy(ev);
  for (int i = 0; i < kMaxChunks; i++) {
    if (ev_k1_begin_[i]) (void)hipEventDestroy(ev_k1_begin_[i]);
    if (ev_k1_end_[i]) (void)hipEventDestroy(ev_k1_end_[i]);
    if (ev_side_done_[i]) (void)hipEventDestroy(ev_side_done_[i]);
  }
  if (side_stream_) (void)hipStreamDestroy(side_stream_);
  if (ev_fin_early_) (void)hipEventDestroy(ev_fin_early_);
  if (ev_tile_done_) (void)hipEventDestroy(ev_tile_done_);
}

int HgScanner::alloc_cands(uint64_t n) {
  n = std::min<uint64_t>(n, 0x7FFFFFF0u);
  HG_TRY(realloc_dev(d_cands_, n, "d_cands_"), "workspace alloc (candidates)");
  HG_TRY(realloc_dev(d_cands2_, n, "d_cands2_"), "workspace alloc (candidates)");
  uint32_t modes = 0;
  for (uint32_t m = 0; m < HG_CONFIRM_MODES; m++) modes += db_->n_confirm_mode[m] ? 1 : 0;
  HG_TRY(realloc_dev(d_deferred_, std::max<uint64_t>(modes, 1) * n, "d_deferred_"), "workspace alloc (deferred)");
  hgmem::dev_free(d_huge_claim_, "d_huge_claim_");
  d_huge_claim_ = nullptr;
  huge_claim_slots_ = 0;
  if (db_->n_confirm_mode[4]) {
    uint64_t slots = 1u << 12;
    while (slots < 2 * n) slots <<= 1;
    HG_TRY(hgmem::dev_alloc(&d_huge_claim_, slots * 8, "d_huge_claim_"), "workspace alloc (claim table)");
    huge_claim_slots_ = slots;
  }
  cand_cap_ = static_cast<uint32_t>(n);
  return HG_OK;
}

int HgScanner::alloc_hits(uint64_t n64) {
  const uint32_t n = static_cast<uint32_t>(std::min<uint64_t>(n64, 0x7FFFFFF0u));
  auto re = [&](auto *&ptr, size_t count, const char *name) { return fail(realloc_dev(ptr, count, name), "workspace alloc (hits)"); };
  if (re(d_hits_raw_, n, "d_hits_raw_") || re(d_hits_out_, n, "d_hits_out_") || re(d_aux_raw_, n, "d_aux_raw_") || re(d_aux_out_, n, "d_aux_out_") ||
      re(d_key_a_, n, "d_key_a_") || re(d_key_b_, n, "d_key_b_") || re(d_perm_a_, n, "d_perm_a_") || re(d_perm_b_, n, "d_perm_b_") || re(d_keep_, n, "d_keep_"))
    return HG_ERR_HIP;
  hit_cap_ = n;
  size_t t1 = 0, t2 = 0;
  (void)rocprim::radix_sort_pairs(nullptr, t1, d_key_a_, d_key_b_, d_perm_a_, d_perm_b_, n, 0, 64, hipStream_t(nullptr));
  (void)rocprim::exclusive_scan(nullptr, t2, d_keep_, d_perm_a_, 0u, n, rocprim::plus<uint32_t>(), hipStream_t(nullptr));
  size_t t3 = 0;
  (void)rocprim::merge(nullptr, t3, d_key_a_, d_key_a_, d_key_b_, d_perm_a_, d_perm_a_, d_perm_b_, n, n, rocprim::less<uint64_t>(), hipStream_t(nullptr));
  size_t need = std::max(std::max(t1, t2), t3) + 256;
  if (need > temp_bytes_) {
    hgmem::dev_free(d_temp_, "d_temp_");
    d_temp_ = nullptr;
    HG_TRY(hgmem::dev_alloc(&d_temp_, need, "d_temp_"), "workspace alloc (sort)");
    temp_bytes_ = need;
  }
  return HG_OK;
}

int HgScanner::ensure(uint64_t nbytes) {
  uint64_t ntiles = std::max<uint64_t>((nbytes + HG_TILE_BYTES - 1) / HG_TILE_BYTES, 1);
  auto re = [&](auto *&ptr, size_t count, const char *name) { return fail(realloc_dev(ptr, count, name), "workspace alloc"); };
  if (ntiles > cap_tiles_) {
    uint64_t nblocks = (ntiles + TS_BLOCK_TILES - 1) / TS_BLOCK_TILES;
    if (re(d_sums_, ntiles, "d_sums_") || re(d_bases_, ntiles + 1, "d_bases_") || re(d_agg_, nblocks, "d_agg_") || re(d_block_base_, nblocks, "d_block_base_")) return HG_ERR_HIP;
    cap_tiles_ = ntiles;
  }
  if (!d_seg_count_) {
    max_segs_ = static_cast<uint32_t>(num_cus_) * 16;
    if (re(d_seg_count_, max_segs_, "d_seg_count_") || re(d_seg_count2_, max_segs_, "d_seg_count2_") || re(d_defer_count_, HG_CONFIRM_MODES * HG_DEFER_SHARDS, "d_defer_count_")) return HG_ERR_HIP;
  }
  uint64_t want = std::max<uint64_t>(nbytes / 1024, 1u << 16);
  if (cand_cap_ < want && alloc_cands(want)) return HG_ERR_HIP;
  if (hit_cap_ < want && alloc_hits(want)) return HG_ERR_HIP;
  return HG_OK;
}

enum { HG_SPLIT = 1000, HG_GROWN = 1001 };

struct HgScanner::PassPlan {
  const uint8_t *text;
  uint64_t nbytes, bs1, ntiles;
  PassRange range;
  bool block_mode, has_anchored;
  hipStream_t stream, side;
  uint32_t id_bits, to_bits, fin_shift = 10, fin_nb = 1, fin_cap;
  bool bucketed;
  uint32_t nchunks = 1;
  bool piped, split;
  uint64_t chunk_tiles;
  std::array<uint64_t, kMaxChunks + 1> cut;
  uint32_t wgs_alone, wgs_shared, joiner_wgs, wgs = 1;
  uint32_t cand_seg_cap[2];
  HgStreamArgs sa;
  HgConfirmArgs ca;
  uint32_t fin_done, stage_blocks = 1;
  uint32_t wgs_of(uint32_t c) const { return c == 0 ? wgs_alone : wgs_shared; }
  uint32_t joiners_of(uint32_t c) const { return c >= 1 ? joiner_wgs : 0u; }
  uint32_t set_of(uint32_t c) const { return piped ? (c & 1u) : 0u; }
  uint32_t settled_buckets(uint32_t c) const {
    const uint64_t prev_end = std::min<uint64_t>(cut[c] << HG_TILE_SHIFT, nbytes);
    const uint64_t settled = prev_end > bs1 ? prev_end - bs1 : 0;
    return static_cast<uint32_t>(std::min<uint64_t>((settled > range.own_lo ? settled - range.own_lo : 0) >> fin_shift, fin_nb));
  }
};

HgScanner::PassPlan HgScanner::plan_pass(const uint8_t *text, uint64_t nbytes, uint64_t bs1, uint64_t line_base, const PassRange &range, bool block_mode,
                                         hipStream_t stream) const {
  const uint64_t tile_lo = range.tile_lo, tile_hi = range.tile_hi, ntiles = tile_hi - tile_lo;
  PassPlan p{text, nbytes, bs1, ntiles, range, block_mode, db_->patterns.size() - db_->ncomb > db_->slow.size(), stream};
  const uint64_t own_end = std::min<uint64_t>(range.own_hi, nbytes), own_len = own_end > range.own_lo ? own_end - range.own_lo : 0;
  p.id_bits = bits_for(static_cast<uint64_t>(db_->max_id) + 1);
  p.to_bits = bits_for(bs1 + 1);
  if (own_len) {
    const uint64_t expect = std::max<uint64_t>(fin_expect_hits_, own_len >> 13);
    uint64_t want_nb = 1;
    const uint64_t per_bucket = knobs_.fin_target;
    while (want_nb * per_bucket < expect && want_nb < HG_FIN_MAX_BUCKETS) want_nb <<= 1;
    while (((own_len - 1) >> p.fin_shift) >= want_nb) p.fin_shift++;
    p.fin_nb = static_cast<uint32_t>((own_len - 1) >> p.fin_shift) + 1;
  }
  p.fin_cap = hit_cap_ / p.fin_nb;
  p.bucketed = ntiles && p.fin_cap && p.fin_shift <= 64 - HG_HIT_REL_SHIFT && p.fin_shift + p.id_bits + p.to_bits + 1 <= 64 &&
               bits_for(line_base + nbytes + 1) <= HG_HIT_REL_SHIFT && !fin_fallback_ && !knobs_.no_bucket_finalize &&
               !view_.bounds &&
               !d_min_lengths_;

  uint32_t nchunks = 1;
  constexpr uint64_t kChunkTiles = 8ull << (30 - HG_TILE_SHIFT);
  if (!block_mode && ntiles >= 2 * kChunkTiles) nchunks = static_cast<uint32_t>(std::min<uint64_t>(kMaxChunks, ntiles / kChunkTiles));
  uint64_t chunk_tiles = ((ntiles + nchunks - 1) / nchunks + TS_BLOCK_TILES - 1) / TS_BLOCK_TILES * TS_BLOCK_TILES;
  if (knobs_.chunk_tiles) {
    const uint64_t v = knobs_.chunk_tiles;
    if (!block_mode && v >= TS_BLOCK_TILES) chunk_tiles = std::max<uint64_t>(v / TS_BLOCK_TILES * TS_BLOCK_TILES, (ntiles + kMaxChunks - 1) / kMaxChunks / TS_BLOCK_TILES * TS_BLOCK_TILES + TS_BLOCK_TILES);
  }
  if (!block_mode && chunk_limit_tiles_ && chunk_tiles > chunk_limit_tiles_) chunk_tiles = chunk_limit_tiles_;
  nchunks = ntiles ? static_cast<uint32_t>((ntiles + chunk_tiles - 1) / chunk_tiles) : 1;
  uint32_t max_chunks = static_cast<uint32_t>(kMaxChunks);
  if (knobs_.max_chunks) max_chunks = std::max(1u, std::min<uint32_t>(kMaxChunks, knobs_.max_chunks));
  p.split = nchunks > max_chunks;
  if (p.split) return p;
  for (uint32_t c = 0; c <= nchunks; c++) p.cut[c] = std::min<uint64_t>(tile_lo + static_cast<uint64_t>(c) * chunk_tiles, tile_hi);
  const std::vector<double> &w = knobs_.chunk_weights;
  if (!block_mode && w.size() >= 2 && w.size() <= static_cast<size_t>(kMaxChunks) && ntiles >= w.size() * TS_BLOCK_TILES * 2) {
    double total = 0, run = 0;
    for (double v : w) total += v;
    nchunks = static_cast<uint32_t>(w.size());
    chunk_tiles = 0;
    for (uint32_t c = 0; c < nchunks; c++) {
      run += w[c];
      uint64_t end = c + 1 == nchunks ? tile_hi : tile_lo + static_cast<uint64_t>(static_cast<double>(ntiles) * run / total) / TS_BLOCK_TILES * TS_BLOCK_TILES;
      end = std::min<uint64_t>(std::max<uint64_t>(end, p.cut[c] + TS_BLOCK_TILES), tile_hi);
      p.cut[c + 1] = end;
      chunk_tiles = std::max<uint64_t>(chunk_tiles, end - p.cut[c]);
    }
  }
  p.nchunks = nchunks;
  p.chunk_tiles = chunk_tiles;
  p.piped = nchunks > 1;
  p.side = p.piped ? side_stream_ : stream;

  if (ntiles) {
    uint32_t per_cu = p.piped ? std::max(1, stream_wgs_per_cu_ - 1) : stream_wgs_per_cu_;
    if (knobs_.stream_wgs_per_cu) {
      const long v = knobs_.stream_wgs_per_cu;
      if (v >= 1 && v <= stream_wgs_per_cu_) per_cu = static_cast<uint32_t>(v);
    }
    auto grid_for = [&](uint32_t wgs_per_cu) {
      return static_cast<uint32_t>(std::min<uint64_t>((std::min<uint64_t>(chunk_tiles, ntiles) + STREAM_WG_WAVES - 1) / STREAM_WG_WAVES,
                                                      std::min<uint64_t>(static_cast<uint64_t>(num_cus_) * wgs_per_cu, max_segs_)));
    };
    p.wgs_shared = grid_for(per_cu);
    p.wgs_alone = knobs_.stream_wgs_per_cu ? p.wgs_shared : grid_for(static_cast<uint32_t>(stream_wgs_per_cu_));
    p.joiner_wgs = (p.piped && stream_wgs_per_cu_ >= 3 && per_cu < static_cast<uint32_t>(stream_wgs_per_cu_) && chunk_limit_tiles_ == 0 && !side_bound_) ? static_cast<uint32_t>(num_cus_) : 0u;
    if (knobs_.joiner >= 0) p.joiner_wgs = p.piped ? static_cast<uint32_t>(knobs_.joiner) * static_cast<uint32_t>(num_cus_) : 0u;
    if (p.wgs_shared + p.joiner_wgs > max_segs_ || db_->filter_wide || db_->filter_log2 > 13) p.joiner_wgs = 0;
    p.wgs = std::max(p.wgs_shared + p.joiner_wgs, p.wgs_alone);
    for (uint32_t c = 0; c < std::min(nchunks, 2u); c++)
      p.cand_seg_cap[c] = static_cast<uint32_t>(static_cast<uint64_t>(cand_cap_) * 4 / (4ull * p.wgs_of(c) + p.joiners_of(c)));
  }
  HgStreamArgs &sa = p.sa;
  sa.text = text;
  sa.nbytes = nbytes;
  sa.db = view_;
  sa.filter = static_cast<const uint32_t *>(d_filter_);
  sa.filter_log2 = db_->filter_log2;
  sa.weights_a = db_->weights_a;
  sa.weights_b = db_->weights_b;
  sa.filter_wide = db_->filter_wide;
  sa.dense = db_->dense;
  sa.weights_c = db_->weights_c;
  sa.ext = static_cast<const HgSlotInfo *>(d_ext_);
  sa.sums = d_sums_;
  sa.counters = d_counters_;
  HgConfirmArgs &ca = p.ca;
  ca.text = text;
  ca.nbytes = nbytes;
  ca.bs1 = bs1;
  ca.db = view_;
  ca.sums = d_sums_;
  ca.bases = d_bases_;
  ca.hits = d_hits_raw_;
  ca.aux = d_aux_raw_;
  ca.tmp_hits = d_hits_out_;
  ca.tmp_aux = d_aux_out_;
  ca.hit_cap = hit_cap_;
  ca.hit_direct = hit_direct_ ? 1u : 0u;
  ca.bucket_shift = p.fin_shift;
  ca.counters = d_counters_;
  ca.own_lo = range.own_lo;
  ca.own_hi = range.own_hi;
  if (!block_mode && p.has_anchored) {
    const uint32_t mode_mask = knobs_.confirm_mode_mask;
    ca.deferred = d_deferred_;
    ca.defer_count = d_defer_count_;
    ca.defer_shard_cap = cand_cap_ / HG_DEFER_SHARDS;
    for (uint32_t m = 0, next = 0; m < HG_CONFIRM_MODES; m++) {
      ca.mode_present[m] = (db_->n_confirm_mode[m] && ((mode_mask >> m) & 1u)) ? 1 : 0;
      ca.list_of_mode[m] = db_->n_confirm_mode[m] ? next++ : 0;
      ca.list_spread[m] = std::min<uint32_t>(HG_DEFER_SHARDS, std::max<uint32_t>(1, HG_DEFER_SHARDS / std::max<uint32_t>(1, db_->n_confirm_mode[m])) * defer_spread_boost_);
    }
  }
  return p;
}

int HgScanner::alloc_fin(uint32_t nb, hipStream_t stream) {
  uint32_t want = 1u << 16;
  while (want < nb) want <<= 1;
  fin_alloc_ = 0;
  HG_TRY(realloc_dev(d_fin_fill_, want, "d_fin_fill_"), "alloc finalize buckets");
  HG_TRY(realloc_dev(d_fin_kept_, want, "d_fin_kept_"), "alloc finalize buckets");
  HG_TRY(realloc_dev(d_fin_big_, 2 * static_cast<size_t>(want) + 3 * 128, "d_fin_big_"), "alloc finalize buckets");
  HG_TRY(hipMemsetAsync(d_fin_big_ + 2 * static_cast<size_t>(want), 0, 3 * 128 * 4, stream), "clear scan flags");
  fin_alloc_ = want;
  return HG_OK;
}

int HgScanner::launch_fin(const PassPlan &p, hipStream_t s, uint32_t lo, uint32_t hi, bool beside_stream) {
  if (hi <= lo) return HG_OK;
  const uint32_t nbk = hi - lo, cu = static_cast<uint32_t>(num_cus_), fin_cap = p.fin_cap, id_bits = p.id_bits, to_bits = p.to_bits;
  HG_TRY(hipMemsetAsync(d_fin_total_ + 2, 0, 8, s), "memset work list");
  hipLaunchKernelGGL(hg_fin_sort_small_kernel, dim3(std::min<uint32_t>((nbk + 3) / 4, cu * 8)), dim3(256), 0, s, d_hits_raw_, d_perm_a_, d_fin_fill_, lo, hi, fin_cap, id_bits, to_bits,
                     d_fin_kept_, d_fin_big_, d_fin_total_ + 2, fin_alloc_);
  hipLaunchKernelGGL((hg_fin_sort_big_kernel<HG_FIN_MEDIUM_CAP, true>), dim3(std::min<uint32_t>(nbk, cu * 4)), dim3(256), 0, s, d_hits_raw_, d_perm_a_, d_fin_fill_, d_fin_big_, d_fin_total_ + 2,
                     fin_cap, id_bits, to_bits, d_fin_kept_, d_selected_ + 1, static_cast<uint64_t *>(nullptr), static_cast<uint32_t *>(nullptr));
  const uint32_t big_blocks = std::min<uint32_t>(std::min<uint32_t>(nbk, 64u), hit_cap_ / HG_FIN_BUCKET_CAP);
  if (big_blocks)
    hipLaunchKernelGGL((hg_fin_sort_big_kernel<HG_FIN_BUCKET_CAP, false>), dim3(big_blocks), dim3(256), 0, s, d_hits_raw_, d_perm_a_, d_fin_fill_, d_fin_big_ + fin_alloc_,
                       d_fin_total_ + 3, fin_cap, id_bits, to_bits, d_fin_kept_, d_selected_ + 1, d_key_a_, d_perm_b_);
  const uint32_t scan_blocks = std::max<uint32_t>(1, std::min<uint32_t>(128, (nbk + 8191) / 8192));
  uint32_t *part = d_fin_big_ + 2 * static_cast<size_t>(fin_alloc_);
  const uint32_t epoch = ++fin_epoch_ ? fin_epoch_ : ++fin_epoch_;
  if (beside_stream) hipLaunchKernelGGL(hg_fin_scan_kernel<512u>, dim3(scan_blocks), dim3(512), 0, s, d_fin_kept_, lo, hi, d_fin_total_, d_fin_fill_, fin_cap, part, epoch);
  else hipLaunchKernelGGL(hg_fin_scan_kernel<1024u>, dim3(scan_blocks), dim3(1024), 0, s, d_fin_kept_, lo, hi, d_fin_total_, d_fin_fill_, fin_cap, part, epoch);
  hipLaunchKernelGGL(hg_fin_gather_kernel, dim3(std::min<uint32_t>((nbk + 3) / 4, cu * 8)), dim3(256), 0, s, d_hits_raw_, d_aux_raw_, d_perm_a_, d_fin_kept_, d_fin_total_, lo, hi, fin_cap,
                     d_hits_out_, d_aux_out_);
  HG_TRY(hipGetLastError(), "finalize launch");
  return HG_OK;
}

int HgScanner::launch_stream(PassPlan &p, uint32_t c, HgScanOutput *out) {
  const uint32_t wgs_c = p.wgs_of(c), joiners_c = p.joiners_of(c);
  HgStreamArgs sa = p.sa;
  sa.tile_begin = p.cut[c];
  sa.tile_end = p.cut[c + 1];
  sa.cursor_slot = HG_CNT_CURSOR0 + c;
  sa.cands = p.set_of(c) ? d_cands2_ : d_cands_;
  sa.seg_count = p.set_of(c) ? d_seg_count2_ : d_seg_count_;
  sa.cand_seg_cap = p.cand_seg_cap[c ? 1 : 0];
  sa.alone = (c == 0 && wgs_c == p.wgs_alone && !knobs_.stream_wgs_per_cu) ? 1u : 0u;
  HgStreamArgs ja = sa;
  ja.cands = sa.cands + static_cast<uint64_t>(wgs_c) * sa.cand_seg_cap;
  ja.cand_seg_cap = sa.cand_seg_cap / 4;
  ja.seg_count = sa.seg_count + wgs_c;
  ja.alone = 0;
  auto launch_joiner = [&](hipStream_t s) -> int {
    if (!hg_launch_stream_join(ja, joiners_c, s)) return HG_ERR_ARG;
    out->joiner_launches++;
    HG_TRY(hipGetLastError(), "hg_stream_kernel launch (joiner)");
    return HG_OK;
  };
  HG_TRY(hipEventRecord(p.piped ? ev_k1_begin_[c] : ev_[1], p.stream), "event");
  if (joiners_c && knobs_.joiner_ahead)
    if (int rc = launch_joiner(p.stream)) return rc;
  if (!hg_launch_stream(sa, wgs_c, p.stream)) return error(HG_ERR_ARG, "no stream kernel for this database's filter size / mode");
  HG_TRY(hipGetLastError(), "hg_stream_kernel launch");
  HG_TRY(hipEventRecord(p.piped ? ev_k1_end_[c] : ev_[2], p.stream), "event");
  if (p.piped && p.bucketed && joiners_c && c + 1 == p.nchunks && !knobs_.no_early_finalize) {
    const uint32_t lim = p.settled_buckets(c);
    if (lim > p.fin_done) {
      if (int rc = launch_fin(p, p.side, p.fin_done, lim, true)) return rc;
      p.fin_done = lim;
    }
  }
  if (joiners_c && !knobs_.joiner_ahead)
    if (int rc = launch_joiner(p.side)) return rc;
  if (p.piped) HG_TRY(hipStreamWaitEvent(p.side, ev_k1_end_[c], 0), "stream wait");
  return HG_OK;
}

int HgScanner::launch_side(PassPlan &p, uint32_t c) {
  const uint64_t t0 = p.cut[c], t1 = p.cut[c + 1];
  const uint32_t segs_c = p.wgs_of(c) + p.joiners_of(c);
  const hipStream_t side = p.side;
  HgConfirmArgs ca = p.ca;
  ca.tile_begin = t0;
  ca.tile_end = t1;
  uint32_t *seg_count = p.set_of(c) ? d_seg_count2_ : d_seg_count_;
  ca.cands = p.set_of(c) ? d_cands2_ : d_cands_;
  ca.seg_count = seg_count;
  ca.cand_seg_cap = p.cand_seg_cap[c ? 1 : 0];
  ca.join_seg0 = p.wgs_of(c);
  ca.join_seg_cap = ca.cand_seg_cap / 4;
  uint32_t confirm_blocks = 1, always_blocks = 1;
  if (p.block_mode) {
    HG_TRY(hipMemsetAsync(d_pflags_, 0, db_->patterns.size() * 4, side), "memset pattern flags");
    if (p.has_anchored) hipLaunchKernelGGL(hg_block_mark_kernel, dim3(segs_c), dim3(256), 0, side, ca, d_pflags_);
    always_blocks = std::max<uint32_t>(static_cast<uint32_t>((db_->patterns.size() + 255) / 256), std::min<uint32_t>(db_->nhuge, 1024u));
    ca.hit_seg_cap = hit_cap_ / always_blocks;
    hipLaunchKernelGGL(hg_block_scan_kernel, dim3(static_cast<uint32_t>((db_->patterns.size() + 255) / 256)), dim3(256), 0, side, ca, d_pflags_);
    if (db_->nhuge && !hg_launch_block_huge(ca, std::min<uint32_t>(db_->nhuge, 1024u), db_->huge_max_nw, db_->huge_stage_words, d_pflags_, side)) return huge_lds_error();
    HG_TRY(hipGetLastError(), "block-mode launch");
    p.stage_blocks = std::max(confirm_blocks, always_blocks);
    return HG_OK;
  }
  const uint64_t span = t1 - t0;
  const uint32_t nblocks = static_cast<uint32_t>((span + TS_BLOCK_TILES - 1) / TS_BLOCK_TILES);
  if (p.bs1 < HG_TILE_BYTES) {
    uint32_t blocks = static_cast<uint32_t>(std::min<uint64_t>((span + 255) / 256, 4096));
    hipLaunchKernelGGL(hg_tile_inner_kernel, dim3(blocks), dim3(256), 0, side, p.text, d_sums_, t0, t1, p.bs1);
  }
  hipLaunchKernelGGL(hg_tile_reduce_kernel, dim3(nblocks), dim3(256), 0, side, d_sums_, t0, t1, p.bs1, d_agg_);
  hipLaunchKernelGGL(hg_tile_spine_kernel, dim3(1), dim3(256), 0, side, d_agg_, nblocks, p.bs1, d_block_base_, d_final_);
  hipLaunchKernelGGL(hg_tile_apply_kernel, dim3(nblocks), dim3(256), 0, side, d_sums_, t0, t1, p.bs1, d_block_base_, d_bases_);
  HG_TRY(hipGetLastError(), "tile scan launch");
  if (p.piped && c + 1 == p.nchunks) HG_TRY(hipEventRecord(ev_tile_done_, side), "event");
  if (p.has_anchored) {
    const uint32_t verify_blocks = segs_c * HG_CONFIRM_SPLIT;
    uint32_t fast_modes = 0;
    const uint32_t mode_mask = knobs_.confirm_mode_mask;
    for (uint32_t m = 0; m < 3; m++) fast_modes += (db_->n_confirm_mode[m] && ((mode_mask >> m) & 1u)) ? 1 : 0;
    uint32_t per_cu = c + 1 == p.nchunks ? 6 : 3;
    if (knobs_.confirm_blocks_per_cu) per_cu = static_cast<uint32_t>(knobs_.confirm_blocks_per_cu);
    const uint32_t mode_blocks = std::max<uint32_t>(HG_DEFER_SHARDS, static_cast<uint32_t>(num_cus_) * per_cu * (256 / HG_CONFIRM_THREADS));
    const uint32_t huge_blocks = db_->n_confirm_mode[4] ? std::max<uint32_t>(HG_DEFER_SHARDS, static_cast<uint32_t>(num_cus_) * static_cast<uint32_t>(std::max<size_t>(1, std::min<size_t>(8, (160u << 10) / std::max<size_t>(hg_huge_lds_bytes(db_->huge_max_nw, db_->huge_stage_words), 1))))) : 0u;
    confirm_blocks = std::max(std::max(mode_blocks * std::max(fast_modes, 1u), verify_blocks), huge_blocks);
    ca.hit_seg_cap = hit_cap_ / confirm_blocks;
    if (c > 0) HG_TRY(hipMemsetAsync(d_defer_count_, 0, HG_CONFIRM_MODES * HG_DEFER_SHARDS * 4, side), "memset deferred counts");
    if (ca.mode_present[1] || ca.mode_present[2]) hipLaunchKernelGGL(hg_verify_kernel, dim3(verify_blocks), dim3(256), 0, side, ca);
    else hipLaunchKernelGGL(hg_verify_lean_kernel, dim3(verify_blocks), dim3(256), 0, side, ca);
    const bool literal_only_set = ca.mode_present[0] && !ca.mode_present[1] && !ca.mode_present[2];
    if (literal_only_set) {
      hipLaunchKernelGGL(hg_confirm_literal_kernel, dim3(mode_blocks), dim3(256), 0, side, ca);
    } else if (fast_modes) {
      hipLaunchKernelGGL(hg_confirm_fast_kernel, dim3(mode_blocks * fast_modes), dim3(HG_CONFIRM_THREADS), 0, side, ca, mode_blocks);
    }
    if (db_->n_confirm_mode[3]) hipLaunchKernelGGL(hg_confirm_generic_kernel, dim3(mode_blocks), dim3(256), 0, side, ca);
    if (huge_blocks && ((mode_mask >> 4) & 1u)) {
      HG_TRY(hipMemsetAsync(d_huge_claim_, 0, huge_claim_slots_ * 8, side), "memset claim table");
      if (!hg_launch_confirm_huge(ca, huge_blocks, db_->huge_max_nw, db_->huge_stage_words, d_huge_claim_, static_cast<uint32_t>(huge_claim_slots_ - 1), side)) return huge_lds_error();
    }
    HG_TRY(hipGetLastError(), "confirm launch");
  }
  if (!db_->slow.empty()) {
    always_blocks = static_cast<uint32_t>(std::min<uint64_t>((span + 3) / 4, static_cast<uint64_t>(num_cus_) * 8));
    const uint32_t huge_always_blocks = db_->nslow_huge ? static_cast<uint32_t>(std::min<uint64_t>(span, static_cast<uint64_t>(num_cus_) * 16)) : 0u;
    ca.hit_seg_cap = hit_cap_ / std::max(always_blocks, huge_always_blocks);
    const uint32_t nfast = db_->nslow_fast, nhuge = db_->nslow_huge, nall = static_cast<uint32_t>(db_->slow.size()) - nhuge;
    if (nfast) {
      ca.deferred = d_deferred_;
      ca.always_count = seg_count;
      ca.always_list_cap = cand_cap_ / always_blocks;
      hipLaunchKernelGGL(hg_always_on_fast_kernel, dim3(always_blocks), dim3(256), 0, side, ca);
      hipLaunchKernelGGL(hg_always_on_finish_kernel, dim3(always_blocks), dim3(256), 0, side, ca);
    }
    if (nall > nfast) hipLaunchKernelGGL(hg_always_on_kernel, dim3(always_blocks), dim3(256), 0, side, ca, nfast, nall);
    if (nhuge && !hg_launch_always_on_huge(ca, huge_always_blocks, db_->huge_max_nw, db_->huge_stage_words, nall, nall + nhuge, side)) return huge_lds_error();
    always_blocks = std::max(always_blocks, huge_always_blocks);
    HG_TRY(hipGetLastError(), "hg_always_on_kernel launch");
  }
  p.stage_blocks = std::max(confirm_blocks, always_blocks);
  return HG_OK;
}

int HgScanner::finalize_last(PassPlan &p, uint32_t c) {
  bool fin_early = false;
  if (p.piped && c >= 1 && !knobs_.no_early_finalize) {
    const uint32_t lim = p.settled_buckets(c);
    if (lim > p.fin_done) {
      HG_TRY(hipStreamWaitEvent(p.stream, ev_side_done_[c - 1], 0), "stream wait");
      HG_TRY(hipStreamWaitEvent(p.stream, ev_tile_done_, 0), "stream wait");
      if (int rc = launch_fin(p, p.stream, p.fin_done, lim)) return rc;
      HG_TRY(hipEventRecord(ev_fin_early_, p.stream), "event");
      p.fin_done = lim;
      fin_early = true;
    }
  }
  if (fin_early) HG_TRY(hipStreamWaitEvent(p.side, ev_fin_early_, 0), "stream wait");
  return launch_fin(p, p.side, p.fin_done, p.fin_nb);
}

int HgScanner::regrow(const PassPlan &p, uint64_t n_raw) {
  const bool block_mode = p.block_mode, bucketed = p.bucketed;
  const uint64_t cand_need = h_counters_[HG_CNT_CAND_NEED], hit_need = h_counters_[HG_CNT_HIT_NEED];
  const uint64_t defer_need = h_counters_[HG_CNT_DEFER_NEED];
  const bool fin_overflow = bucketed && h_counters_[HG_ST_SELECTED + 1] != 0;
  uint64_t kHitLimit = 1ull << 28;
  if (knobs_.hit_limit) kHitLimit = std::max<uint64_t>(1u << 10, knobs_.hit_limit);
  if (!block_mode && (n_raw > kHitLimit || h_counters_[HG_CNT_HITS_WRAPPED])) return HG_SPLIT;
  if (!(cand_need || defer_need || hit_need || fin_overflow || (!bucketed && n_raw > hit_cap_))) return HG_OK;
  if (cand_need || defer_need) {
    if (defer_need && defer_spread_boost_ < HG_DEFER_SHARDS) defer_spread_boost_ *= 4;
    uint64_t want = std::max<uint64_t>((cand_need + cand_need / 4 + 64) * p.wgs, (defer_need + defer_need / 4 + 64) * HG_DEFER_SHARDS);
    want = std::max<uint64_t>(want, static_cast<uint64_t>(cand_cap_) * 2);
    uint64_t kCandLimit = 1ull << 30;
    if (knobs_.cand_limit) kCandLimit = std::max<uint64_t>(1u << 16, knobs_.cand_limit);
    if (want > kCandLimit) {
      const uint64_t cur = (std::min<uint64_t>(p.chunk_tiles, p.ntiles) + TS_BLOCK_TILES - 1) / TS_BLOCK_TILES * TS_BLOCK_TILES;
      if (block_mode || cur <= TS_BLOCK_TILES) return error(HG_ERR_ARG, "the candidate limit is below what one 16 MiB chunk of this text produces");
      chunk_limit_tiles_ = std::max<uint64_t>(TS_BLOCK_TILES, cur / 2 / TS_BLOCK_TILES * TS_BLOCK_TILES);
      want = std::min<uint64_t>(want / 2, kCandLimit);
    }
    if (want > cand_cap_)
      if (int rc = alloc_cands(want)) return rc;
  }
  if (bucketed && (hit_need || fin_overflow)) {
    const uint64_t want = (hit_need + hit_need / 4 + 16) * p.fin_nb;
    fin_expect_hits_ = std::max<uint64_t>(fin_expect_hits_ * 2, n_raw);
    if (fin_overflow || hit_need > HG_FIN_BUCKET_CAP || want > (128ull << 20)) {
      fin_fallback_ = true;
    } else if (int rc = alloc_hits(std::max<uint64_t>(want, static_cast<uint64_t>(hit_cap_) * 2))) {
      return rc;
    }
  } else if (hit_need || n_raw > hit_cap_) {
    uint64_t want = std::max<uint64_t>((hit_need + hit_need / 4 + 64) * p.stage_blocks, n_raw + n_raw / 4);
    constexpr uint64_t kSegmentLimit = 64ull << 20;
    const uint64_t by_total = n_raw + n_raw / 4 + 4096;
    if (want > kSegmentLimit || want > 16 * by_total) {
      hit_direct_ = true;
      want = std::min<uint64_t>(want, std::max<uint64_t>(by_total, std::min<uint64_t>(16 * by_total, kSegmentLimit)));
    }
    const uint64_t most = kHitLimit + kHitLimit / 4 + 4096;
    want = std::max<uint64_t>(want, std::min<uint64_t>(static_cast<uint64_t>(hit_cap_) * 2, most));
    if (want > most && !block_mode) return HG_SPLIT;
    if (want > most) return error(HG_ERR_ARG, "more than 2^28 reports for one block");
    if (int rc = alloc_hits(want)) return rc;
  }
  return HG_GROWN;
}

int HgScanner::finalize_compact(const HgHit *hits, const HgHitAux *aux, uint32_t n, uint32_t id_bits, uint32_t to_bits, uint64_t line_bound, hipStream_t stream) {
  const HgPattern *pats = static_cast<const HgPattern *>(d_patterns_);
  uint32_t blocks = (n + 255) / 256;
  const uint32_t line_bits = bits_for(line_bound);
  const uint32_t *perm = nullptr;
  uint32_t *pos = nullptr;
  size_t tb = temp_bytes_;
  if (line_bits + id_bits + to_bits + 1 <= 64) {
    hipLaunchKernelGGL(hg_key_packed_kernel, dim3(blocks), dim3(256), 0, stream, hits, aux, pats, n, id_bits, to_bits, d_key_a_, d_perm_a_);
    HG_TRY(rocprim::radix_sort_pairs(d_temp_, tb, d_key_a_, d_key_b_, d_perm_a_, d_perm_b_, n, 0, line_bits + id_bits + to_bits + 1, stream), "radix sort");
    perm = d_perm_b_;
    pos = d_perm_a_;
  } else {
    hipLaunchKernelGGL(hg_key_kernel, dim3(blocks), dim3(256), 0, stream, hits, aux, pats, n, d_key_a_, d_perm_a_);
    HG_TRY(rocprim::radix_sort_pairs(d_temp_, tb, d_key_a_, d_key_b_, d_perm_a_, d_perm_b_, n, 0, 64, stream), "radix sort (id, to)");
    hipLaunchKernelGGL(hg_line_key_kernel, dim3(blocks), dim3(256), 0, stream, hits, d_perm_b_, n, d_key_a_);
    tb = temp_bytes_;
    HG_TRY(rocprim::radix_sort_pairs(d_temp_, tb, d_key_a_, d_key_b_, d_perm_b_, d_perm_a_, n, 0, std::min<uint32_t>(64, line_bits), stream), "radix sort (line)");
    perm = d_perm_a_;
    pos = d_perm_b_;
  }
  hipLaunchKernelGGL(hg_keep_kernel, dim3(blocks), dim3(256), 0, stream, hits, aux, perm, pats, n, d_keep_);
  tb = temp_bytes_;
  HG_TRY(rocprim::exclusive_scan(d_temp_, tb, d_keep_, pos, 0u, n, rocprim::plus<uint32_t>(), stream), "scan");
  hipLaunchKernelGGL(hg_scatter_kernel, dim3(blocks), dim3(256), 0, stream, hits, aux, perm, d_keep_, pos, n, d_hits_out_, d_aux_out_, d_selected_);
  HG_TRY(hipGetLastError(), "finalize launch");
  HG_TRY(hipMemcpyAsync(h_counters_ + HG_ST_SELECTED, d_selected_, 4, hipMemcpyDeviceToHost, stream), "copy count");
  return HG_OK;
}

int HgScanner::comb_pass(HgScanOutput *out, uint64_t bs1, uint64_t line_bound, hipStream_t stream) {
  const uint64_t n = out->n_hits;
  if (n == 0) return HG_OK;
  if (n + 1 > comb_in_cap_) {
    const uint64_t cap = std::max<uint64_t>(n + n / 4 + 1, 4096);
    comb_in_cap_ = 0;
    HG_TRY(realloc_dev(d_comb_count_, cap, "d_comb_count_"), "alloc (combination pass)");
    HG_TRY(realloc_dev(d_comb_pos_, cap, "d_comb_pos_"), "alloc (combination pass)");
    size_t tb = 0;
    HG_TRY(rocprim::exclusive_scan(nullptr, tb, d_comb_count_, d_comb_pos_, uint64_t{0}, cap, rocprim::plus<uint64_t>(), stream), "scan (combination pass)");
    if (tb > comb_temp_bytes_) {
      comb_temp_bytes_ = 0;
// ... 328 lines not shown
```

### hypergrep_amd/csrc/hg_stream.hip

```cpp
#include <hip/hip_runtime.h>
#include <cstdlib>

#include "hg_core.h"
#include "hg_engine.h"

namespace {

constexpr int WG_WAVES = HG_STREAM_WG_WAVES;
constexpr int WG_THREADS = WG_WAVES * 64;
constexpr int ITERS = HG_TILE_BYTES / 1024;

__device__ __forceinline__ uint32_t wave_inclusive_scan(uint32_t v, uint32_t lane) {
#pragma unroll
  for (int o = 1; o < 64; o <<= 1) {
    uint32_t u = __shfl_up(v, o, 64);
    if (lane >= static_cast<uint32_t>(o)) v += u;
  }
  return v;
}

}

namespace {

__device__ __forceinline__ uint32_t not_newline_bits(uint32_t w) {
  uint32_t b = ((w & 0x7f7f7f7fu) ^ 0x0a0a0a0au) + 0x7f7f7f7fu;
  return b | w | 0x7f7f7f7fu;
}

__device__ __forceinline__ uint32_t popc_add(uint32_t x, uint32_t acc) {
  uint32_t r;
  asm("v_bcnt_u32_b32 %0, %1, %2" : "=v"(r) : "v"(x), "v"(acc));
  return r;
}
__device__ __forceinline__ uint32_t opaque_sgpr(uint32_t v) {
  asm("" : "+s"(v));
  return v;
}

using lds_u32 = __attribute__((address_space(3))) uint32_t;

constexpr uint32_t queue_cap(int) { return 128u; }
constexpr bool queue_stash(int log2, bool dense) { return log2 <= 12 && !dense; }
constexpr uint32_t queue_entry_dw(int log2, bool dense) { return queue_stash(log2, dense) ? 8u : 2u; }
__device__ __forceinline__ uint32_t queue_chunk(uint32_t e0) { return e0 >> 16; }
__device__ __forceinline__ uint32_t queue_rank(uint32_t e0) { return e0 & 0xFFFFu; }

template <int LOG2, bool WIDE>
struct Probe {
  static constexpr uint32_t BYTE_MASK = ((1u << LOG2) - 1u) << 2;
  __device__ __forceinline__ static uint32_t at(const lds_u32 *filter, uint32_t byte_off) {
    return *reinterpret_cast<const lds_u32 *>(reinterpret_cast<const __attribute__((address_space(3))) uint8_t *>(filter) + byte_off);
  }
  template <bool ANY_ONLY, bool FOLD = true>
  __device__ __forceinline__ static uint32_t probe4(const lds_u32 *filter, uint32_t fold, uint32_t wa, uint32_t wb, uint4 v) {
    const uint32_t f0 = FOLD ? v.x | fold : v.x, f1 = FOLD ? v.y | fold : v.y, f2 = FOLD ? v.z | fold : v.z, f3 = FOLD ? v.w | fold : v.w;
    const uint32_t a0 = hg_dot4(f0, wa), a1 = hg_dot4(f1, wa), a2 = hg_dot4(f2, wa), a3 = hg_dot4(f3, wa);
    const uint32_t b0 = hg_dot4(f0, wb), b1 = hg_dot4(f1, wb), b2 = hg_dot4(f2, wb), b3 = hg_dot4(f3, wb);
    const uint32_t c0 = hg_dot4(f0, HG_HASH_WEIGHTS), c1 = hg_dot4(f1, HG_HASH_WEIGHTS);
    const uint32_t c2 = hg_dot4(f2, HG_HASH_WEIGHTS), c3 = hg_dot4(f3, HG_HASH_WEIGHTS);
    if (WIDE) {
      auto wide = [&](uint32_t x, uint32_t y) { return at(filter, hg_slot_wide(x, y, BYTE_MASK)); };
      const uint32_t ta0 = wide(a0, b0), tb0 = wide(b0, a0), ta1 = wide(a1, b1), tb1 = wide(b1, a1);
      const uint32_t ta2 = wide(a2, b2), tb2 = wide(b2, a2), ta3 = wide(a3, b3), tb3 = wide(b3, a3);
      auto m = [](uint32_t t, uint32_t c) { return static_cast<uint16_t>(t) == static_cast<uint16_t>(c) || static_cast<uint16_t>(t >> 16) == static_cast<uint16_t>(c); };
      const bool m0 = m(ta0, c0) || m(tb0, c0), m1 = m(ta1, c1) || m(tb1, c1), m2 = m(ta2, c2) || m(tb2, c2), m3 = m(ta3, c3) || m(tb3, c3);
      if (ANY_ONLY) return (m0 || m1 || m2 || m3) ? 1u : 0u;
      return (m0 ? 1u : 0u) | (m1 ? 2u : 0u) | (m2 ? 4u : 0u) | (m3 ? 8u : 0u);
    }
    const uint32_t t0 = at(filter, a0 & BYTE_MASK), t1 = at(filter, a1 & BYTE_MASK), t2 = at(filter, a2 & BYTE_MASK), t3 = at(filter, a3 & BYTE_MASK);
    const bool m0 = hg_slot_match(t0, c0), m1 = hg_slot_match(t1, c1), m2 = hg_slot_match(t2, c2), m3 = hg_slot_match(t3, c3);
    if (ANY_ONLY) return (m0 || m1 || m2 || m3) ? 1u : 0u;
    return (m0 ? 1u : 0u) | (m1 ? 2u : 0u) | (m2 ? 4u : 0u) | (m3 ? 8u : 0u);
  }
  template <bool FOLD>
  __device__ __forceinline__ static bool any4(const lds_u32 *filter, uint32_t fold, uint32_t wa, uint32_t wb, uint4 v, uint64_t &mask) {
    if (WIDE) {
      const bool any = probe4<true, FOLD>(filter, fold, wa, wb, v) != 0;
      mask = __builtin_amdgcn_ballot_w64(any);
      return any;
    }
    const uint32_t f0 = FOLD ? v.x | fold : v.x, f1 = FOLD ? v.y | fold : v.y, f2 = FOLD ? v.z | fold : v.z, f3 = FOLD ? v.w | fold : v.w;
    const uint32_t a0 = hg_dot4(f0, wa), a1 = hg_dot4(f1, wa), a2 = hg_dot4(f2, wa), a3 = hg_dot4(f3, wa);
    const uint32_t t0 = at(filter, a0 & BYTE_MASK), t1 = at(filter, a1 & BYTE_MASK), t2 = at(filter, a2 & BYTE_MASK), t3 = at(filter, a3 & BYTE_MASK);
    const uint32_t c0 = hg_dot4(f0, HG_HASH_WEIGHTS), c1 = hg_dot4(f1, HG_HASH_WEIGHTS);
    const uint32_t c2 = hg_dot4(f2, HG_HASH_WEIGHTS), c3 = hg_dot4(f3, HG_HASH_WEIGHTS);
    const bool m0 = hg_slot_match(t0, c0), m1 = hg_slot_match(t1, c1), m2 = hg_slot_match(t2, c2), m3 = hg_slot_match(t3, c3);
    mask = __builtin_amdgcn_ballot_w64(m0) | __builtin_amdgcn_ballot_w64(m1) | __builtin_amdgcn_ballot_w64(m2) | __builtin_amdgcn_ballot_w64(m3);
    return m0 || m1 || m2 || m3;
  }
};

template <int LOG2, int STEP>
struct ProbeBytes {
  static constexpr uint32_t BYTE_MASK = ((1u << LOG2) - 1u) << 2;
  template <bool ANY_ONLY>
  __device__ __forceinline__ static uint32_t probe16(const lds_u32 *filter, uint32_t fold, uint32_t wa, uint32_t wc, uint4 v, uint32_t nxt) {
    const uint32_t d[5] = {v.x | fold, v.y | fold, v.z | fold, v.w | fold, nxt | fold};
    uint32_t bits = 0;
#pragma unroll
    for (int j = 0; j < 4; j++) {
      uint32_t w[4], t[4];
      w[0] = d[j];
#pragma unroll
      for (int k = STEP; k < 4; k += STEP) w[k] = __builtin_amdgcn_alignbyte(d[j + 1], d[j], k);
#pragma unroll
      for (int k = 0; k < 4; k += STEP) t[k] = Probe<LOG2, false>::at(filter, hg_dot4(w[k], wa) & BYTE_MASK);
#pragma unroll
      for (int k = 0; k < 4; k += STEP) {
        const bool m = hg_slot_match(t[k], hg_dot4(w[k], wc));
        if (ANY_ONLY) bits |= m ? 1u : 0u;
        else bits |= m ? (1u << (j * 4 + k)) : 0u;
      }
    }
    return bits;
  }
};

__device__ __forceinline__ uint32_t newline_bits16(uint4 v) {
  const uint32_t w[4] = {v.x, v.y, v.z, v.w};
  uint32_t bits = 0;
#pragma unroll
  for (int k = 0; k < 4; k++) {
    const uint32_t m = hg_newline_mask(w[k]);
#pragma unroll
    for (int b = 0; b < 4; b++) bits |= ((m >> (8 * b + 7)) & 1u) << (k * 4 + b);
  }
  return bits;
}
__device__ __forceinline__ uint4 readlane4(uint4 v, uint32_t l) {
  return make_uint4(__builtin_amdgcn_readlane(v.x, l), __builtin_amdgcn_readlane(v.y, l), __builtin_amdgcn_readlane(v.z, l), __builtin_amdgcn_readlane(v.w, l));
}

__device__ __forceinline__ uint32_t load_dword_checked(const uint4 *__restrict__ text16, uint64_t nbytes, uint64_t at) {
  if (at >= nbytes) return 0u;
  uint32_t v = reinterpret_cast<const uint32_t *>(text16)[at >> 2];
  const uint64_t rest = nbytes - at;
  if (rest < 4) v &= (1u << (rest * 8)) - 1u;
  return v;
}

struct StreamCtx {
  const uint4 *text16;
  uint64_t nbytes;
  const lds_u32 *filter;
  const HgSlotInfo *ext;
  lds_u32 *queue;
  lds_u32 *cand_count;
  HgCand *seg;
  uint32_t seg_cap, fold, wa, wb;
};

#if defined(__HIP_DEVICE_COMPILE__)
static_assert(sizeof(StreamCtx) <= 64, "StreamCtx is passed by value to the out-of-line drain routine: beyond 16 dwords it travels through scratch (measured: 1.1 GB of scratch writes per 8 GiB launch, stream pass 20 % slower)");
#endif

__device__ __forceinline__ uint4 load_chunk_checked(const uint4 *__restrict__ text16, uint64_t nbytes, uint64_t g) {
  uint4 v = make_uint4(0, 0, 0, 0);
  if ((g << 4) < nbytes) {
    v = text16[g];
    const uint64_t byte0 = g << 4;
    if (byte0 + 16 > nbytes) {
      const uint32_t valid = static_cast<uint32_t>(nbytes - byte0);
      uint32_t w[4] = {v.x, v.y, v.z, v.w};
#pragma unroll
      for (int k = 0; k < 4; k++) {
        const uint32_t lo = k * 4u;
        if (valid <= lo) w[k] = 0;
        else if (valid < lo + 4) w[k] &= (1u << ((valid - lo) * 8)) - 1u;
      }
      v = make_uint4(w[0], w[1], w[2], w[3]);
    }
  }
  return v;
}

typedef uint32_t __attribute__((aligned(1))) hg_u32_unaligned;
__device__ __forceinline__ uint32_t dense_window(uint4 cur, uint32_t nxt, uint32_t k) {
  const uint32_t j = k >> 2;
  const uint32_t lo = j == 0 ? cur.x : (j == 1 ? cur.y : (j == 2 ? cur.z : cur.w));
  const uint32_t hi = j == 0 ? cur.y : (j == 1 ? cur.z : (j == 2 ? cur.w : nxt));
  return static_cast<uint32_t>(((static_cast<uint64_t>(hi) << 32) | lo) >> (8u * (k & 3u)));
}

template <int LOG2, bool WIDE, int DENSE>
__device__ __noinline__ void drain_batch(const StreamCtx cx, uint32_t first, uint32_t n, uint32_t lane) {
  const bool active = lane < n;
  uint32_t hits = 0, rank = 0;
  uint64_t g = 0;
  uint4 cur = make_uint4(0, 0, 0, 0);
  if constexpr (DENSE) {
    uint32_t nxt = 0;
    if (active) {
      const lds_u32 *e = cx.queue + (first + lane) * queue_entry_dw(LOG2, DENSE);
      const uint32_t e_lo = e[0], e_hi = e[1];
      g = static_cast<uint64_t>(e_hi) * (HG_TILE_BYTES / 16) + queue_chunk(e_lo);
      rank = queue_rank(e_lo);
      cur = load_chunk_checked(cx.text16, cx.nbytes, g);
      nxt = load_dword_checked(cx.text16, cx.nbytes, (g + 1) << 4);
      uint32_t l1 = ProbeBytes<LOG2, DENSE ? DENSE : 1>::template probe16<false>(cx.filter, cx.fold, cx.wa, cx.wb, cur, nxt);
      if ((g << 4) + 16 > cx.nbytes) l1 &= (g << 4) < cx.nbytes ? (1u << static_cast<uint32_t>(cx.nbytes - (g << 4))) - 1u : 0u;
      const uint32_t wbytes = (cx.wb >> 24) ? 4u : 3u, wmask = (cx.wb >> 24) ? 0xFFFFFFFFu : 0x00FFFFFFu;
      constexpr uint32_t BYTE_MASK = ((1u << LOG2) - 1u) << 2;
      const uint8_t *text = reinterpret_cast<const uint8_t *>(cx.text16);
      for (uint32_t todo = l1; todo; todo &= todo - 1) {
        const uint32_t k = __ffs(todo) - 1;
        const uint64_t pos = (g << 4) + k;
        const uint32_t wk = dense_window(cur, nxt, k);
        uint32_t prev = 0, next = 0;
        if (pos >= 4 && pos + 8 <= cx.nbytes) {
          prev = *reinterpret_cast<const hg_u32_unaligned *>(text + pos - 4);
          next = *reinterpret_cast<const hg_u32_unaligned *>(text + pos + wbytes);
        } else {
          for (uint32_t b = 0; b < 4; b++) {
            if (pos + b >= 4) prev |= static_cast<uint32_t>(text[pos + b - 4]) << (8 * b);
            if (pos + wbytes + b < cx.nbytes) next |= static_cast<uint32_t>(text[pos + wbytes + b]) << (8 * b);
          }
        }
        const uint32_t f = (wk | cx.fold) & wmask;
        const HgSlotInfo info = cx.ext[(hg_dot4(f, cx.wa) & BYTE_MASK) >> 2];
        if (hg_slot_pass(info, f, prev | cx.fold, next | cx.fold, 0xFFFFFFFFu, 0xFFFFFFFFu)) hits |= 1u << k;
      }
    }
    const uint32_t cnt = __popc(hits);
    if (!__builtin_amdgcn_ballot_w64(cnt != 0)) return;
    const uint32_t incl = wave_inclusive_scan(cnt, lane);
    const uint32_t total = __builtin_amdgcn_readlane(incl, 63);
    uint32_t base = 0;
    if (lane == 0) base = __hip_atomic_fetch_add(cx.cand_count, total, __ATOMIC_RELAXED, __HIP_MEMORY_SCOPE_WORKGROUP);
    base = __builtin_amdgcn_readfirstlane(base);
    uint32_t s = base + incl - cnt;
    uint32_t nl = 0;
    {
      const uint32_t words[4] = {cur.x, cur.y, cur.z, cur.w};
#pragma unroll
      for (int j = 0; j < 4; j++) {
        const uint32_t m = ~not_newline_bits(words[j]);
        nl |= (((m >> 7) & 1u) | ((m >> 14) & 2u) | ((m >> 21) & 4u) | ((m >> 28) & 8u)) << (4 * j);
      }
    }
    for (uint32_t todo = hits; todo; todo &= todo - 1, s++) {
      const uint32_t k = __ffs(todo) - 1;
      if (s < cx.seg_cap) cx.seg[s] = HgCand{(g << 4) + k, dense_window(cur, nxt, k), rank + __popc(nl & ((1u << k) - 1u))};
    }
    return;
  }
  if (active) {
    const lds_u32 *e = cx.queue + (first + lane) * queue_entry_dw(LOG2, DENSE);
    const uint32_t e_lo = e[0], e_hi = e[1];
    g = static_cast<uint64_t>(e_hi) * (HG_TILE_BYTES / 16) + queue_chunk(e_lo);
    rank = queue_rank(e_lo);
    uint32_t left = 0, right = 0;
    bool have_left = (queue_chunk(e_lo) & 63u) != 0, have_right = (queue_chunk(e_lo) & 63u) != 63u;
    if (queue_stash(LOG2, DENSE)) {
      left = e[2];
      right = e[3];
      cur = make_uint4(e[4], e[5], e[6], e[7]);
    } else {
      cur = load_chunk_checked(cx.text16, cx.nbytes, g);
      if (!WIDE) {
        const uint32_t *text32 = reinterpret_cast<const uint32_t *>(cx.text16);
        left = g ? text32[g * 4 - 1] : 0u;
        if (((g + 1) << 4) < cx.nbytes) {
          right = text32[g * 4 + 4];
          const uint64_t rest = cx.nbytes - ((g + 1) << 4);
          if (rest < 4) right &= (1u << (rest * 8)) - 1u;
        }
        have_left = have_right = true;
      }
    }
    uint32_t l1 = Probe<LOG2, WIDE>::template probe4<false>(cx.filter, cx.fold, cx.wa, cx.wb, cur);
    if ((g << 4) + 16 > cx.nbytes) l1 &= (g << 4) < cx.nbytes ? (1u << static_cast<uint32_t>((cx.nbytes - (g << 4) + 3) >> 2)) - 1u : 0u;
    if (WIDE) {
      hits = l1;
    } else if (l1) {
      constexpr uint32_t BYTE_MASK = ((1u << LOG2) - 1u) << 2;
      for (uint32_t todo = l1 & 15u; todo; todo &= todo - 1) {
        const uint32_t k = __ffs(todo) - 1;
        const uint32_t wk = k == 0 ? cur.x : (k == 1 ? cur.y : (k == 2 ? cur.z : cur.w));
        const uint32_t wp = k == 0 ? left : (k == 1 ? cur.x : (k == 2 ? cur.y : cur.z));
        const uint32_t wn = k == 0 ? cur.y : (k == 1 ? cur.z : (k == 2 ? cur.w : right));
        const uint32_t f = wk | cx.fold;
        const HgSlotInfo info = cx.ext[(hg_dot4(f, cx.wa) & BYTE_MASK) >> 2];
        const uint32_t pm_keep = (k == 0 && !have_left) ? 0u : 0xFFFFFFFFu;
        const uint32_t nm_keep = (k == 3 && !have_right) ? (HG_WINDOW_BYTES == 4 ? 0u : 0xFFu) : 0xFFFFFFFFu;
        const uint32_t prev = wp | cx.fold;
        const uint32_t next = (HG_WINDOW_BYTES == 4 ? wn : ((wk >> 24) | (wn << 8))) | cx.fold;
        if (hg_slot_pass(info, f & HG_WINDOW_MASK, prev, next, pm_keep, nm_keep)) hits |= 1u << k;
      }
    }
  }
  if (!__builtin_amdgcn_ballot_w64(hits != 0)) return;
  const uint32_t words[4] = {cur.x, cur.y, cur.z, cur.w};
  uint32_t total = 0, slot[4];
#pragma unroll
  for (int k = 0; k < 4; k++) {
    const uint64_t mk = __builtin_amdgcn_ballot_w64(((hits >> k) & 1u) != 0);
    slot[k] = total + __builtin_amdgcn_mbcnt_hi(static_cast<uint32_t>(mk >> 32), __builtin_amdgcn_mbcnt_lo(static_cast<uint32_t>(mk), 0u));
    total += __popcll(mk);
  }
  uint32_t base = 0;
  if (lane == 0) base = __hip_atomic_fetch_add(cx.cand_count, total, __ATOMIC_RELAXED, __HIP_MEMORY_SCOPE_WORKGROUP);
  base = __builtin_amdgcn_readfirstlane(base);
  const uint64_t pos = g << 4;
#pragma unroll
  for (int k = 0; k < 4; k++) {
    if ((hits >> k) & 1u) {
      const uint32_t s = base + slot[k];
      if (s < cx.seg_cap) cx.seg[s] = HgCand{pos + 4u * k, words[k], rank};
    }
    rank += __popc(~not_newline_bits(words[k]));
  }
}

template <int LOG2, bool WIDE, int DENSE, bool FULL, int DEPTH, bool FOLD>
__device__ __forceinline__ void stream_tile(const StreamCtx &cx, uint64_t tile, HgTileSum *__restrict__ sums, uint32_t lane, uint32_t &qn) {
  const uint4 *__restrict__ text16 = cx.text16;
  const uint64_t nbytes = cx.nbytes;
  const uint64_t chunk0 = tile * (HG_TILE_BYTES / 16) + lane;

  const __amdgpu_buffer_rsrc_t tile_rsrc = __builtin_amdgcn_make_buffer_rsrc(const_cast<uint4 *>(text16 + tile * (HG_TILE_BYTES / 16)), 0, HG_TILE_BYTES, 0x00020000);
  const uint32_t lane_off = lane * 16u;
  auto load_chunk = [&](int it) -> uint4 {
    const uint64_t g = chunk0 + static_cast<uint64_t>(it) * 64u;
    if (FULL) {
      if (WIDE) return text16[g];
      if (DENSE) {
        typedef uint32_t u32x4 __attribute__((ext_vector_type(4)));
        const u32x4 v = __builtin_nontemporal_load(reinterpret_cast<const u32x4 *>(text16) + g);
        return make_uint4(v.x, v.y, v.z, v.w);
      }
#if defined(HG_NO_NT_LOADS)
      return text16[g];
#else
      typedef uint32_t u32x4 __attribute__((ext_vector_type(4)));
      const u32x4 v = __builtin_amdgcn_raw_buffer_load_b128(tile_rsrc, lane_off, it * 1024, 2);
      return make_uint4(v.x, v.y, v.z, v.w);
#endif
    }
    return load_chunk_checked(text16, nbytes, g);
  };

  uint32_t seen = 0;
  uint32_t first_nl = HG_NONE32, last_nl = HG_NONE32;
  uint32_t first_it = 0, last_it = 0;
  uint64_t first_nlm = 0, last_nlm = 0;
  const uint32_t lane_key = lane << 16;

  auto load_after = [&](int it) -> uint32_t {
    if (!DENSE || lane != 63u) return 0u;
    return load_dword_checked(text16, nbytes, (chunk0 + static_cast<uint64_t>(it) * 64u + 1u) << 4);
  };

  auto body = [&](int it, uint4 cur, uint32_t after) {
    uint32_t notnl = __popc(not_newline_bits(cur.x));
    notnl = popc_add(not_newline_bits(cur.y), notnl);
    notnl = popc_add(not_newline_bits(cur.z), notnl);
    notnl = popc_add(not_newline_bits(cur.w), notnl);
#if defined(HG_ABLATE) && HG_ABLATE == 2
    const uint32_t c = cur.x == 0x0a0a0a0au ? 1u : 0u;
    const bool has_nl = c != 0, several_nl = c > 1;
#else
    const uint32_t c = 128u - notnl;
    const bool has_nl = notnl != 128u, several_nl = notnl < 127u;
#endif

#if defined(HG_ABLATE) && HG_ABLATE == 1
    bool any = (cur.x ^ cur.y ^ cur.z ^ cur.w) == 0x12345678u;
    uint64_t am = __builtin_amdgcn_ballot_w64(any);
#else
    bool any;
    uint64_t am;
    if constexpr (DENSE) {
      const uint32_t nxt = __builtin_amdgcn_update_dpp(after, cur.x, 0x130 , 0xF, 0xF, false);
      any = ProbeBytes<LOG2, DENSE ? DENSE : 1>::template probe16<true>(cx.filter, cx.fold, cx.wa, cx.wb, cur, nxt) != 0;
      am = __builtin_amdgcn_ballot_w64(any);
    } else {
      any = Probe<LOG2, WIDE>::template any4<FOLD>(cx.filter, cx.fold, cx.wa, cx.wb, cur, am);
    }
#endif

    if constexpr (!FULL) {
      any = any && ((chunk0 + static_cast<uint64_t>(it) * 64u) << 4) < nbytes;
      am = __builtin_amdgcn_ballot_w64(any);
    }

    const uint64_t nlm = __builtin_amdgcn_ballot_w64(has_nl);
    const uint64_t multi = __builtin_amdgcn_ballot_w64(several_nl);
    if constexpr (!DENSE) {
      if (nlm && first_nl == HG_NONE32) {
        const uint32_t l = __builtin_ctzll(nlm);
        first_nl = static_cast<uint32_t>(it) * 1024u + l * 16u + (__ffs(newline_bits16(readlane4(cur, l))) - 1);
      }
      if (it == ITERS - 1 && nlm) {
        const uint32_t l = 63u - __builtin_clzll(nlm);
        last_nl = static_cast<uint32_t>(it) * 1024u + l * 16u + (31 - __clz(newline_bits16(readlane4(cur, l))));
      }
    } else {
      first_it = first_nlm ? first_it : static_cast<uint32_t>(it);
      first_nlm = first_nlm ? first_nlm : nlm;
    }
    last_it = nlm ? static_cast<uint32_t>(it) : last_it;
    last_nlm = nlm ? nlm : last_nlm;
    const uint32_t key = lane_key + opaque_sgpr(seen + (static_cast<uint32_t>(it) << 22));
    uint32_t total, e0 = 0;
    if (__builtin_expect(multi == 0, 1)) {
      total = __popcll(nlm);
      e0 = __builtin_amdgcn_mbcnt_hi(static_cast<uint32_t>(nlm >> 32), __builtin_amdgcn_mbcnt_lo(static_cast<uint32_t>(nlm), key));
    } else {
      const uint32_t incl = wave_inclusive_scan(c, lane);
      total = __builtin_amdgcn_readlane(incl, 63);
      e0 = key + incl - c;
    }
    if (am) {
      const uint32_t left = __builtin_amdgcn_mov_dpp(cur.w, 0x138 , 0xF, 0xF, true);
      const uint32_t right = __builtin_amdgcn_mov_dpp(cur.x, 0x130 , 0xF, 0xF, true);
      if (any) {
        const uint32_t idx = __builtin_amdgcn_mbcnt_hi(static_cast<uint32_t>(am >> 32), __builtin_amdgcn_mbcnt_lo(static_cast<uint32_t>(am), 0u));
        lds_u32 *e = (cx.queue + qn * queue_entry_dw(LOG2, DENSE)) + idx * queue_entry_dw(LOG2, DENSE);
        e[0] = e0;
        e[1] = static_cast<uint32_t>(tile);
        if (queue_stash(LOG2, DENSE)) {
          e[2] = left;
          e[3] = right;
          e[4] = cur.x;
          e[5] = cur.y;
          e[6] = cur.z;
          e[7] = cur.w;
        }
      }
      qn += __popcll(am);
      if (qn >= queue_cap(LOG2) - 64u) {
        const uint32_t n = qn < 64u ? qn : 64u;
        qn -= n;
        drain_batch<LOG2, WIDE, DENSE>(cx, qn, n, lane);
      }
    }
    seen += total;
  };

  if constexpr (FULL) {
    uint4 buf[DEPTH];
    uint32_t abuf[DEPTH];
#pragma unroll
    for (int d = 0; d < DEPTH; d++) { buf[d] = load_chunk(d); abuf[d] = load_after(d); }
#pragma unroll
    for (int it = 0; it < ITERS; it++) {
      const uint4 cur = buf[it % DEPTH];
      const uint32_t after = abuf[it % DEPTH];
      if (it + DEPTH < ITERS) { buf[it % DEPTH] = load_chunk(it + DEPTH); abuf[it % DEPTH] = load_after(it + DEPTH); }
      body(it, cur, after);
    }
  } else {
#pragma unroll 1
    for (int it = 0; it < ITERS; it++) body(it, load_chunk(it), load_after(it));
  }

  const uint32_t nl_count = seen;
  if (nl_count && first_nl == HG_NONE32) {
    const uint32_t l = __builtin_ctzll(first_nlm);
    const uint4 v = load_chunk_checked(text16, nbytes, tile * (HG_TILE_BYTES / 16) + first_it * 64u + l);
    first_nl = first_it * 1024u + l * 16u + (__ffs(newline_bits16(v)) - 1);
  }
  if (nl_count && last_nl == HG_NONE32) {
    const uint32_t l = 63u - __builtin_clzll(last_nlm);
    const uint4 v = load_chunk_checked(text16, nbytes, tile * (HG_TILE_BYTES / 16) + last_it * 64u + l);
    last_nl = last_it * 1024u + l * 16u + (31 - __clz(newline_bits16(v)));
  }
  if (lane == 0) sums[tile] = HgTileSum{nl_count, first_nl, last_nl, nl_count ? nl_count - 1 : 0};
}

}

#ifndef HG_STREAM_WAVES
#define HG_STREAM_WAVES 6
#endif
#ifndef HG_DEPTH_ALONE
#define HG_DEPTH_ALONE 3
#endif
#ifndef HG_DEPTH_SHARED
#define HG_DEPTH_SHARED 3
#endif
template <int LOG2, bool WIDE, int DENSE, int DEPTH, bool JOIN, bool FOLD>
__device__ __forceinline__ void stream_body(const uint4 *__restrict__ text16, uint64_t nbytes, uint64_t tile_begin, uint64_t tile_end, const uint4 *__restrict__ filter16,
                                            const uint4 *__restrict__ ext16, uint32_t fold, uint32_t wa, uint32_t wb, HgTileSum *__restrict__ sums, HgCand *__restrict__ cands,
                                            uint32_t seg_cap, uint32_t *__restrict__ seg_count, uint32_t *__restrict__ counters, uint32_t cursor_slot) {
  constexpr uint32_t FILTER_U4 = (4u << LOG2) / 16, QUEUE_U4 = WG_WAVES * queue_cap(LOG2) * queue_entry_dw(LOG2, DENSE) * 4 / 16;
  __shared__ uint4 s_mem[FILTER_U4 + QUEUE_U4 + 1];
  {
    for (uint32_t i = threadIdx.x; i < FILTER_U4; i += WG_THREADS) s_mem[i] = filter16[i];
    if (threadIdx.x == 0) s_mem[FILTER_U4 + QUEUE_U4] = make_uint4(0, 0, 0, 0);
  }
  __syncthreads();
  const uint32_t lane = threadIdx.x & 63u;
  const uint32_t wave = __builtin_amdgcn_readfirstlane(threadIdx.x >> 6);
  StreamCtx cx;
  cx.text16 = text16;
  cx.nbytes = nbytes;
  cx.filter = (const lds_u32 *)(&s_mem[0]);
  cx.queue = (lds_u32 *)(&s_mem[FILTER_U4]) + wave * queue_cap(LOG2) * queue_entry_dw(LOG2, DENSE);
  cx.cand_count = (lds_u32 *)(&s_mem[FILTER_U4 + QUEUE_U4]);
  cx.ext = reinterpret_cast<const HgSlotInfo *>(ext16);
  cx.seg = cands + static_cast<uint64_t>(blockIdx.x) * seg_cap;
  cx.seg_cap = seg_cap;
  cx.fold = fold;
  cx.wa = wa;
  cx.wb = wb;
  const uint64_t full_tiles = nbytes >> HG_TILE_SHIFT;
  lds_u32 *s_run = cx.cand_count + 1;
  const uint32_t ntile = static_cast<uint32_t>(tile_end - tile_begin);
  const uint32_t nfull = full_tiles > tile_begin ? static_cast<uint32_t>(full_tiles - tile_begin < ntile ? full_tiles - tile_begin : ntile) : 0u;
  uint32_t qn = 0, joined = 0;
  for (;;) {
    if (threadIdx.x == 0) *s_run = atomicAdd(&counters[cursor_slot], HG_STREAM_GRAB);
    __syncthreads();
    const uint32_t r0 = __builtin_amdgcn_readfirstlane(*s_run);
    __syncthreads();
    if (r0 >= ntile) break;
    const uint32_t r1 = r0 + HG_STREAM_GRAB < ntile ? r0 + HG_STREAM_GRAB : ntile;
    if (JOIN) joined += r1 - r0;
    for (uint32_t r = r0 + wave; r < r1; r += WG_WAVES) {
      if (r < nfull) stream_tile<LOG2, WIDE, DENSE, true, DEPTH, FOLD>(cx, tile_begin + r, sums, lane, qn);
      else stream_tile<LOG2, WIDE, DENSE, false, DEPTH, FOLD>(cx, tile_begin + r, sums, lane, qn);
    }
  }
  if (qn) drain_batch<LOG2, WIDE, DENSE>(cx, 0u, qn, lane);
  __syncthreads();
  if (threadIdx.x == 0) {
    const uint32_t n = *cx.cand_count;
    seg_count[blockIdx.x] = n < seg_cap ? n : seg_cap;
    atomicAdd(&counters[HG_CNT_CANDS], n < seg_cap ? n : seg_cap);
    if (n > seg_cap) atomicMax(&counters[HG_CNT_CAND_NEED], n);
    if (JOIN && joined) atomicAdd(&counters[HG_CNT_JOIN_TILES], joined);
  }
}
template <int LOG2, bool WIDE, int DENSE, int DEPTH, bool FOLD = true>
__global__ __launch_bounds__(WG_THREADS) __attribute__((amdgpu_waves_per_eu(HG_STREAM_WAVES, 8))) void hg_stream_kernel(
    const uint4 *__restrict__ text16, uint64_t nbytes, uint64_t tile_begin, uint64_t tile_end, const uint4 *__restrict__ filter16, const uint4 *__restrict__ ext16, uint32_t fold,
    uint32_t wa, uint32_t wb, HgTileSum *__restrict__ sums, HgCand *__restrict__ cands, uint32_t seg_cap, uint32_t *__restrict__ seg_count, uint32_t *__restrict__ counters,
    uint32_t cursor_slot) {
#ifdef HG_STREAM_PRIO
  __builtin_amdgcn_s_setprio(HG_STREAM_PRIO);
#endif
  stream_body<LOG2, WIDE, DENSE, DEPTH, false, FOLD>(text16, nbytes, tile_begin, tile_end, filter16, ext16, fold, wa, wb, sums, cands, seg_cap, seg_count, counters, cursor_slot);
}
template <int LOG2, int DENSE, bool FOLD = true>
__global__ __launch_bounds__(WG_THREADS) __attribute__((amdgpu_waves_per_eu(HG_STREAM_WAVES, 8))) void hg_stream_join_kernel(
    const uint4 *__restrict__ text16, uint64_t nbytes, uint64_t tile_begin, uint64_t tile_end, const uint4 *__restrict__ filter16, const uint4 *__restrict__ ext16, uint32_t fold,
    uint32_t wa, uint32_t wb, HgTileSum *__restrict__ sums, HgCand *__restrict__ cands, uint32_t seg_cap, uint32_t *__restrict__ seg_count, uint32_t *__restrict__ counters,
    uint32_t cursor_slot) {
#ifdef HG_STREAM_PRIO
  __builtin_amdgcn_s_setprio(HG_STREAM_PRIO);
#endif
  stream_body<LOG2, false, DENSE, HG_DEPTH_SHARED, true, FOLD>(text16, nbytes, tile_begin, tile_end, filter16, ext16, fold, wa, wb, sums, cands, seg_cap, seg_count, counters, cursor_slot);
}

namespace {
template <int L, bool W, int B, int D>
void launch_depth(const HgStreamArgs &a, uint32_t grid, hipStream_t stream) {
  const uint4 *t = reinterpret_cast<const uint4 *>(a.text);
  const uint4 *f = reinterpret_cast<const uint4 *>(a.filter);
  const uint4 *x = reinterpret_cast<const uint4 *>(a.ext);
  if constexpr (!W && !B) {
    if (a.db.fold_mask == 0) {
      hipLaunchKernelGGL((hg_stream_kernel<L, W, B, D, false>), dim3(grid), dim3(WG_THREADS), 0, stream, t, a.nbytes, a.tile_begin, a.tile_end, f, x, a.db.fold_mask,
                         a.weights_a, a.dense ? a.weights_c : a.weights_b, a.sums, a.cands, a.cand_seg_cap, a.seg_count, a.counters, a.cursor_slot);
      return;
    }
  }
  hipLaunchKernelGGL((hg_stream_kernel<L, W, B, D, true>), dim3(grid), dim3(WG_THREADS), 0, stream, t, a.nbytes, a.tile_begin, a.tile_end, f, x, a.db.fold_mask,
                     a.weights_a, a.dense ? a.weights_c : a.weights_b, a.sums, a.cands, a.cand_seg_cap, a.seg_count, a.counters, a.cursor_slot);
}
template <int L, bool W, int B>
void launch_one(const HgStreamArgs &a, uint32_t grid, hipStream_t stream) {
  if (!W && !B && L <= 12 && a.alone) launch_depth<L, W, B, (!W && !B && L <= 12) ? HG_DEPTH_ALONE : HG_DEPTH_SHARED>(a, grid, stream);
  else launch_depth<L, W, B, HG_DEPTH_SHARED>(a, grid, stream);
}
template <int L, bool W, int B>
int blocks_one() {
  int n = 0;
  (void)hipOccupancyMaxActiveBlocksPerMultiprocessor(&n, (hg_stream_kernel<L, W, B, (!W && !B && L <= 12) ? HG_DEPTH_ALONE : HG_DEPTH_SHARED>), WG_THREADS, 0);
  return n > 0 ? n : 1;
}
}
namespace {
template <int L, int B>
void launch_join(const HgStreamArgs &a, uint32_t grid, hipStream_t stream) {
  if constexpr (B == 0) {
    if (a.db.fold_mask == 0) {
      hipLaunchKernelGGL((hg_stream_join_kernel<L, B, false>), dim3(grid), dim3(WG_THREADS), 0, stream, reinterpret_cast<const uint4 *>(a.text), a.nbytes, a.tile_begin, a.tile_end,
                         reinterpret_cast<const uint4 *>(a.filter), reinterpret_cast<const uint4 *>(a.ext), a.db.fold_mask, a.weights_a, a.dense ? a.weights_c : a.weights_b, a.sums,
                         a.cands, a.cand_seg_cap, a.seg_count, a.counters, a.cursor_slot);
      return;
    }
  }
  hipLaunchKernelGGL((hg_stream_join_kernel<L, B, true>), dim3(grid), dim3(WG_THREADS), 0, stream, reinterpret_cast<const uint4 *>(a.text), a.nbytes, a.tile_begin, a.tile_end,
                     reinterpret_cast<const uint4 *>(a.filter), reinterpret_cast<const uint4 *>(a.ext), a.db.fold_mask, a.weights_a, a.dense ? a.weights_c : a.weights_b, a.sums,
                     a.cands, a.cand_seg_cap, a.seg_count, a.counters, a.cursor_slot);
}
}
bool hg_launch_stream_join(const HgStreamArgs &a, uint32_t grid, hipStream_t stream) {
  if (a.filter_wide || a.filter_log2 < 11 || a.filter_log2 > 13 || a.dense > 2) return false;
  switch (a.filter_log2 * 4 + a.dense) {
    case 11 * 4 + 0: launch_join<11, 0>(a, grid, stream); break;
    case 11 * 4 + 1: launch_join<11, 1>(a, grid, stream); break;
    case 11 * 4 + 2: launch_join<11, 2>(a, grid, stream); break;
    case 12 * 4 + 0: launch_join<12, 0>(a, grid, stream); break;
    case 12 * 4 + 1: launch_join<12, 1>(a, grid, stream); break;
    case 12 * 4 + 2: launch_join<12, 2>(a, grid, stream); break;
    case 13 * 4 + 0: launch_join<13, 0>(a, grid, stream); break;
    case 13 * 4 + 1: launch_join<13, 1>(a, grid, stream); break;
    case 13 * 4 + 2: launch_join<13, 2>(a, grid, stream); break;
    default: return false;
  }
  return true;
}
bool hg_launch_stream(const HgStreamArgs &a, uint32_t grid, hipStream_t stream) {
  if (a.filter_wide) {
    switch (a.filter_log2) {
      case 13: launch_one<13, true, 0>(a, grid, stream); break;
      case 14: launch_one<14, true, 0>(a, grid, stream); break;
      case 15: launch_one<15, true, 0>(a, grid, stream); break;
      default: return false;
    }
    return true;
  }
  if (a.dense == 1) {
    switch (a.filter_log2) {
      case 11: launch_one<11, false, 1>(a, grid, stream); break;
      case 12: launch_one<12, false, 1>(a, grid, stream); break;
      case 13: launch_one<13, false, 1>(a, grid, stream); break;
      case 14: launch_one<14, false, 1>(a, grid, stream); break;
      case 15: launch_one<15, false, 1>(a, grid, stream); break;
      default: return false;
    }
    return true;
  }
  if (a.dense == 2) {
    switch (a.filter_log2) {
      case 11: launch_one<11, false, 2>(a, grid, stream); break;
      case 12: launch_one<12, false, 2>(a, grid, stream); break;
      case 13: launch_one<13, false, 2>(a, grid, stream); break;
      case 14: launch_one<14, false, 2>(a, grid, stream); break;
      case 15: launch_one<15, false, 2>(a, grid, stream); break;
      default: return false;
    }
    return true;
  }
  switch (a.filter_log2) {
    case 11: launch_one<11, false, 0>(a, grid, stream); break;
    case 12: launch_one<12, false, 0>(a, grid, stream); break;
    case 13: launch_one<13, false, 0>(a, grid, stream); break;
    case 14: launch_one<14, false, 0>(a, grid, stream); break;
    case 15: launch_one<15, false, 0>(a, grid, stream); break;
    default: return false;
  }
  return true;
}
int hg_stream_blocks_per_cu(uint32_t filter_log2, uint32_t filter_wide, uint32_t dense) {
  if (filter_wide) return filter_log2 == 13 ? blocks_one<13, true, 0>() : (filter_log2 == 14 ? blocks_one<14, true, 0>() : blocks_one<15, true, 0>());
  if (dense == 1) {
    switch (filter_log2) {
      case 11: return blocks_one<11, false, 1>();
      case 12: return blocks_one<12, false, 1>();
      case 13: return blocks_one<13, false, 1>();
      case 14: return blocks_one<14, false, 1>();
      default: return blocks_one<15, false, 1>();
    }
  }
  if (dense == 2) {
    switch (filter_log2) {
      case 11: return blocks_one<11, false, 2>();
      case 12: return blocks_one<12, false, 2>();
      case 13: return blocks_one<13, false, 2>();
      case 14: return blocks_one<14, false, 2>();
      default: return blocks_one<15, false, 2>();
    }
  }
  switch (filter_log2) {
    case 11: return blocks_one<11, false, 0>();
    case 12: return blocks_one<12, false, 0>();
    case 13: return blocks_one<13, false, 0>();
    case 14: return blocks_one<14, false, 0>();
    default: return blocks_one<15, false, 0>();
  }
}
```

Baseline: 5049.

## Add context-byte filter variant that folds next byte into slot fingerprint

Builds a second single-probe filter whose fingerprint also checks the byte after each 4-byte window when all values in a slot agree on it. This rejects more false candidates in the streaming pass, so fewer windows go to the drain/verify stage. Tuning runs on a sample and turns the mode on only if it cuts candidate rows enough; otherwise a separate plain kernel runs. It also recomputes the lane id inside cold paths to relieve register pressure, at the cost of extra ALU work per probe and extra kernel instantiations.

```diff
diff --git a/hypergrep_amd/csrc/hg_compile.cpp b/hypergrep_amd/csrc/hg_compile.cpp
--- a/hypergrep_amd/csrc/hg_compile.cpp
+++ b/hypergrep_amd/csrc/hg_compile.cpp
@@ -976,6 +976,8 @@
 
 int build_filter(HgDb &db, const SampleStats *stats, std::string *err) {
   db.windows.clear();
+  db.filter_ctx.clear();
+  db.filter_use_ctx = 0;
   std::vector<std::pair<uint32_t, HgWindow>> keyed;
   std::vector<uint32_t> next16_of;
   const uint32_t fold = db.fold_mask;
@@ -1279,6 +1281,26 @@
           merge(x->nv, x->nm, nv, nm);
         }
       }
+      if (!db.dense && wbytes == 4) {
+        db.filter_ctx.assign(size_t(1) << k, HG_FILTER_EMPTY);
+        const uint32_t high = 0xFFFFu & ~HG_CTX_LOW;
+        for (size_t sl = 0; sl < db.ext.size(); sl++) {
+          const HgSlotInfo &info = db.ext[sl];
+          if (!info.nvalues) continue;
+          uint32_t care = (db.filter[sl] >> 16) & HG_CTX_LOW, fp = db.filter[sl] & HG_CTX_LOW;
+          uint32_t agree = info.many ? 0u : high, first = 0;
+          for (uint32_t i = 0; i < info.nvalues && agree; i++) {
+            if ((info.cond[i].nm & 0xFFu) != 0xFFu) { agree = 0; break; }
+            const uint32_t t = hg_ctx_value(hg_hash_window(info.value[i]), info.cond[i].nv & 0xFFu);
+            if (i == 0) first = t;
+            agree &= ~(first ^ t);
+          }
+          care |= agree;
+          fp |= first & agree;
+          db.filter_ctx[sl] = (care << 16) | fp;
+        }
+        db.filter_use_ctx = 1;
+      }
     }
   }
   db.filter_wide = 0;
@@ -2230,6 +2252,25 @@
   }
   int rc = build_filter(*copy, &st, err);
   if (rc != 0) return rc;
+  if (copy->filter_use_ctx) {
+    const uint32_t byte_mask = ((1u << copy->filter_log2) - 1u) << 2;
+    size_t rows = 0, rows_plain = 0, rows_ctx = 0;
+    for (size_t r = 0; r + 1024 <= nbytes; r += 1024, rows++) {
+      bool any_plain = false, any_ctx = false;
+      for (size_t p = r; p < r + 1024 && !(any_plain && any_ctx); p += 4) {
+        uint32_t w, nx = 0;
+        std::memcpy(&w, sample + p, 4);
+        if (p + 8 <= nbytes) std::memcpy(&nx, sample + p + 4, 4);
+        w |= fold;
+        const uint32_t sl = hg_slot(w, copy->weights_a, byte_mask) >> 2, key = hg_hash_window(w);
+        any_plain = any_plain || hg_slot_match(copy->filter[sl], key);
+        any_ctx = any_ctx || hg_slot_match_ctx(copy->filter_ctx[sl], key, nx | fold, p + 4 < r + 1024);
+      }
+      rows_plain += any_plain;
+      rows_ctx += any_ctx;
+    }
+    if (rows && (rows_plain < rows_ctx || (rows_plain - rows_ctx) * 4 < rows)) copy->filter_use_ctx = 0;
+  }
   copy->tuned = true;
   *out = copy.release();
   return 0;
diff --git a/hypergrep_amd/csrc/hg_compile.h b/hypergrep_amd/csrc/hg_compile.h
--- a/hypergrep_amd/csrc/hg_compile.h
+++ b/hypergrep_amd/csrc/hg_compile.h
@@ -22,6 +22,8 @@
   uint32_t shared_windows = 0;
   uint32_t wtab_first = 0;
   std::vector<uint32_t> filter;
+  std::vector<uint32_t> filter_ctx;
+  uint32_t filter_use_ctx = 0;
   uint32_t filter_log2 = HG_FILTER_MIN_LOG2;
   uint32_t filter_wide = 0;
   uint32_t window_bytes = HG_WINDOW_BYTES;
diff --git a/hypergrep_amd/csrc/hg_db.h b/hypergrep_amd/csrc/hg_db.h
--- a/hypergrep_amd/csrc/hg_db.h
+++ b/hypergrep_amd/csrc/hg_db.h
@@ -165,6 +165,15 @@
 HG_HD uint32_t hg_hash_window(uint32_t folded) { return hg_dot4(folded, HG_HASH_WEIGHTS); }
 HG_HD uint32_t hg_slot(uint32_t folded, uint32_t weights, uint32_t byte_mask) { return hg_dot4(folded, weights) & byte_mask; }
 HG_HD bool hg_slot_match(uint32_t slot_word, uint32_t hash_c) { return (hash_c & (slot_word >> 16)) == (slot_word & 0xFFFFu); }
+#ifndef HG_CTX_SHIFT
+#define HG_CTX_SHIFT 12
+#endif
+constexpr uint32_t HG_CTX_LOW = (1u << HG_CTX_SHIFT) - 1u;
+constexpr uint32_t HG_CTX_EDGE_KEEP = HG_CTX_LOW * 0x10001u;
+HG_HD uint32_t hg_ctx_value(uint32_t hash_c, uint32_t next_folded) { return hash_c + (next_folded << HG_CTX_SHIFT); }
+HG_HD bool hg_slot_match_ctx(uint32_t ctx_word, uint32_t hash_c, uint32_t next_folded, bool have_next) {
+  return hg_slot_match(have_next ? ctx_word : (ctx_word & HG_CTX_EDGE_KEEP), hg_ctx_value(hash_c, next_folded));
+}
 HG_HD uint32_t hg_slot_wide(uint32_t sum_x, uint32_t sum_y, uint32_t byte_mask) { return (sum_x + (sum_y << 8)) & byte_mask; }
 
 struct HgFilterExt {
diff --git a/hypergrep_amd/csrc/hg_engine.h b/hypergrep_amd/csrc/hg_engine.h
--- a/hypergrep_amd/csrc/hg_engine.h
+++ b/hypergrep_amd/csrc/hg_engine.h
@@ -57,6 +57,7 @@
   uint32_t weights_a, weights_b;
   uint32_t filter_wide;
   uint32_t dense;
+  uint32_t ctx;
   uint32_t weights_c;
   uint32_t alone;
   uint32_t cursor_slot;
diff --git a/hypergrep_amd/csrc/hg_engine.hip b/hypergrep_amd/csrc/hg_engine.hip
--- a/hypergrep_amd/csrc/hg_engine.hip
+++ b/hypergrep_amd/csrc/hg_engine.hip
@@ -156,8 +156,18 @@
   HG_TRY(upload(&d_bucket2_, db.bucket_off2, "d_bucket2_"), "upload buckets");
   HG_TRY(upload(&d_windows2_, db.windows2, "d_windows2_"), "upload windows");
   HG_TRY(upload(&d_wtab_, db.wtab, "d_wtab_"), "upload window table");
-  HG_TRY(upload(&d_filter_, db.filter, "d_filter_"), "upload filter");
-  HG_TRY(upload(&d_ext_, db.ext, "d_ext_"), "upload filter conditions");
+  if (db.filter_use_ctx) {
+    if (db.filter_wide || db.dense || db.filter_ctx.size() != (size_t(1) << db.filter_log2) || db.ext.size() != db.filter_ctx.size() || db.filter.size() != db.filter_ctx.size())
+      return error(HG_ERR_ARG, "the database's single-probe filter has no context slots");
+    HG_TRY(upload(&d_filter_, db.filter_ctx, "d_filter_"), "upload filter");
+    std::vector<uint32_t> ext_words(db.ext.size() * (sizeof(HgSlotInfo) / 4) + db.filter.size());
+    std::memcpy(ext_words.data(), db.ext.data(), db.ext.size() * sizeof(HgSlotInfo));
+    std::memcpy(ext_words.data() + db.ext.size() * (sizeof(HgSlotInfo) / 4), db.filter.data(), db.filter.size() * 4);
+    HG_TRY(upload(&d_ext_, ext_words, "d_ext_"), "upload filter conditions");
+  } else {
+    HG_TRY(upload(&d_filter_, db.filter, "d_filter_"), "upload filter");
+    HG_TRY(upload(&d_ext_, db.ext, "d_ext_"), "upload filter conditions");
+  }
   HG_TRY(upload(&d_slow_, db.slow, "d_slow_"), "upload always-on list");
   HG_TRY(upload(&d_groups_, db.groups, "d_groups_"), "upload always-on groups");
   view_.patterns = static_cast<const HgPattern *>(d_patterns_);
@@ -403,6 +413,7 @@
   sa.weights_a = db_->weights_a;
   sa.weights_b = db_->weights_b;
   sa.filter_wide = db_->filter_wide;
+  sa.ctx = db_->filter_use_ctx;
   sa.dense = db_->dense;
   sa.weights_c = db_->weights_c;
   sa.ext = static_cast<const HgSlotInfo *>(d_ext_);
diff --git a/hypergrep_amd/csrc/hg_stream.hip b/hypergrep_amd/csrc/hg_stream.hip
--- a/hypergrep_amd/csrc/hg_stream.hip
+++ b/hypergrep_amd/csrc/hg_stream.hip
@@ -10,13 +10,20 @@
 constexpr int WG_THREADS = WG_WAVES * 64;
 constexpr int ITERS = HG_TILE_BYTES / 1024;
 
+template <bool OWN_LANE = false>
 __device__ __forceinline__ uint32_t wave_inclusive_scan(uint32_t v, uint32_t lane) {
 #pragma unroll
-  for (int o = 1; o < 64; o <<= 1) {
-    uint32_t u = __shfl_up(v, o, 64);
-    if (lane >= static_cast<uint32_t>(o)) v += u;
+  for (uint32_t o = 1; o < 64; o <<= 1) {
+    const uint32_t u = OWN_LANE ? static_cast<uint32_t>(__builtin_amdgcn_ds_bpermute(static_cast<int>((lane - o) << 2), static_cast<int>(v))) : __shfl_up(v, o, 64);
+    if (lane >= o) v += u;
   }
   return v;
+}
+
+__device__ __forceinline__ uint32_t lane_here() {
+  uint32_t l;
+  asm volatile("v_mbcnt_lo_u32_b32 %0, -1, 0\n\tv_mbcnt_hi_u32_b32 %0, -1, %0" : "=v"(l));
+  return l;
 }
 
 }
@@ -46,14 +53,17 @@
 __device__ __forceinline__ uint32_t queue_chunk(uint32_t e0) { return e0 >> 16; }
 __device__ __forceinline__ uint32_t queue_rank(uint32_t e0) { return e0 & 0xFFFFu; }
 
-template <int LOG2, bool WIDE>
+static_assert(HG_WINDOW_BYTES == 4, "the single-probe filter's context byte is the low byte of the dword after a 4-byte window");
+template <int LOG2, bool WIDE, bool CTX>
 struct Probe {
+  static_assert(!(WIDE && CTX), "wide filters have no context byte");
+  __device__ __forceinline__ static uint32_t value(uint32_t c, uint32_t next) { return CTX ? hg_ctx_value(c, next) : c; }
   static constexpr uint32_t BYTE_MASK = ((1u << LOG2) - 1u) << 2;
   __device__ __forceinline__ static uint32_t at(const lds_u32 *filter, uint32_t byte_off) {
     return *reinterpret_cast<const lds_u32 *>(reinterpret_cast<const __attribute__((address_space(3))) uint8_t *>(filter) + byte_off);
   }
   template <bool ANY_ONLY, bool FOLD = true>
-  __device__ __forceinline__ static uint32_t probe4(const lds_u32 *filter, uint32_t fold, uint32_t wa, uint32_t wb, uint4 v) {
+  __device__ __forceinline__ static uint32_t probe4(const lds_u32 *filter, uint32_t fold, uint32_t wa, uint32_t wb, uint4 v, uint32_t right, uint32_t keep3) {
     const uint32_t f0 = FOLD ? v.x | fold : v.x, f1 = FOLD ? v.y | fold : v.y, f2 = FOLD ? v.z | fold : v.z, f3 = FOLD ? v.w | fold : v.w;
     const uint32_t a0 = hg_dot4(f0, wa), a1 = hg_dot4(f1, wa), a2 = hg_dot4(f2, wa), a3 = hg_dot4(f3, wa);
     const uint32_t b0 = hg_dot4(f0, wb), b1 = hg_dot4(f1, wb), b2 = hg_dot4(f2, wb), b3 = hg_dot4(f3, wb);
@@ -68,23 +78,25 @@
       if (ANY_ONLY) return (m0 || m1 || m2 || m3) ? 1u : 0u;
       return (m0 ? 1u : 0u) | (m1 ? 2u : 0u) | (m2 ? 4u : 0u) | (m3 ? 8u : 0u);
     }
-    const uint32_t t0 = at(filter, a0 & BYTE_MASK), t1 = at(filter, a1 & BYTE_MASK), t2 = at(filter, a2 & BYTE_MASK), t3 = at(filter, a3 & BYTE_MASK);
-    const bool m0 = hg_slot_match(t0, c0), m1 = hg_slot_match(t1, c1), m2 = hg_slot_match(t2, c2), m3 = hg_slot_match(t3, c3);
+    const uint32_t fr = FOLD ? right | fold : right;
+    const uint32_t t0 = at(filter, a0 & BYTE_MASK), t1 = at(filter, a1 & BYTE_MASK), t2 = at(filter, a2 & BYTE_MASK), t3 = CTX ? at(filter, a3 & BYTE_MASK) & keep3 : at(filter, a3 & BYTE_MASK);
+    const bool m0 = hg_slot_match(t0, value(c0, f1)), m1 = hg_slot_match(t1, value(c1, f2));
+    const bool m2 = hg_slot_match(t2, value(c2, f3)), m3 = hg_slot_match(t3, value(c3, fr));
     if (ANY_ONLY) return (m0 || m1 || m2 || m3) ? 1u : 0u;
     return (m0 ? 1u : 0u) | (m1 ? 2u : 0u) | (m2 ? 4u : 0u) | (m3 ? 8u : 0u);
   }
   template <bool FOLD>
-  __device__ __forceinline__ static bool any4(const lds_u32 *filter, uint32_t fold, uint32_t wa, uint32_t wb, uint4 v, uint64_t &mask) {
+  __device__ __forceinline__ static bool any4(const lds_u32 *filter, uint32_t fold, uint32_t wa, uint32_t wb, uint4 v, uint32_t fr, uint32_t keep3, uint64_t &mask) {
     if (WIDE) {
-      const bool any = probe4<true, FOLD>(filter, fold, wa, wb, v) != 0;
+      const bool any = probe4<true, FOLD>(filter, fold, wa, wb, v, 0u, 0xFFFFFFFFu) != 0;
       mask = __builtin_amdgcn_ballot_w64(any);
       return any;
     }
     const uint32_t f0 = FOLD ? v.x | fold : v.x, f1 = FOLD ? v.y | fold : v.y, f2 = FOLD ? v.z | fold : v.z, f3 = FOLD ? v.w | fold : v.w;
     const uint32_t a0 = hg_dot4(f0, wa), a1 = hg_dot4(f1, wa), a2 = hg_dot4(f2, wa), a3 = hg_dot4(f3, wa);
-    const uint32_t t0 = at(filter, a0 & BYTE_MASK), t1 = at(filter, a1 & BYTE_MASK), t2 = at(filter, a2 & BYTE_MASK), t3 = at(filter, a3 & BYTE_MASK);
-    const uint32_t c0 = hg_dot4(f0, HG_HASH_WEIGHTS), c1 = hg_dot4(f1, HG_HASH_WEIGHTS);
-    const uint32_t c2 = hg_dot4(f2, HG_HASH_WEIGHTS), c3 = hg_dot4(f3, HG_HASH_WEIGHTS);
+    const uint32_t t0 = at(filter, a0 & BYTE_MASK), t1 = at(filter, a1 & BYTE_MASK), t2 = at(filter, a2 & BYTE_MASK), t3 = CTX ? at(filter, a3 & BYTE_MASK) & keep3 : at(filter, a3 & BYTE_MASK);
+    const uint32_t c0 = value(hg_dot4(f0, HG_HASH_WEIGHTS), f1), c1 = value(hg_dot4(f1, HG_HASH_WEIGHTS), f2);
+    const uint32_t c2 = value(hg_dot4(f2, HG_HASH_WEIGHTS), f3), c3 = value(hg_dot4(f3, HG_HASH_WEIGHTS), fr);
     const bool m0 = hg_slot_match(t0, c0), m1 = hg_slot_match(t1, c1), m2 = hg_slot_match(t2, c2), m3 = hg_slot_match(t3, c3);
     mask = __builtin_amdgcn_ballot_w64(m0) | __builtin_amdgcn_ballot_w64(m1) | __builtin_amdgcn_ballot_w64(m2) | __builtin_amdgcn_ballot_w64(m3);
     return m0 || m1 || m2 || m3;
@@ -105,7 +117,7 @@
 #pragma unroll
       for (int k = STEP; k < 4; k += STEP) w[k] = __builtin_amdgcn_alignbyte(d[j + 1], d[j], k);
 #pragma unroll
-      for (int k = 0; k < 4; k += STEP) t[k] = Probe<LOG2, false>::at(filter, hg_dot4(w[k], wa) & BYTE_MASK);
+      for (int k = 0; k < 4; k += STEP) t[k] = Probe<LOG2, false, false>::at(filter, hg_dot4(w[k], wa) & BYTE_MASK);
 #pragma unroll
       for (int k = 0; k < 4; k += STEP) {
         const bool m = hg_slot_match(t[k], hg_dot4(w[k], wc));
@@ -183,8 +195,9 @@
   return static_cast<uint32_t>(((static_cast<uint64_t>(hi) << 32) | lo) >> (8u * (k & 3u)));
 }
 
-template <int LOG2, bool WIDE, int DENSE>
-__device__ __noinline__ void drain_batch(const StreamCtx cx, uint32_t first, uint32_t n, uint32_t lane) {
+template <int LOG2, bool WIDE, int DENSE, bool CTX>
+__device__ __noinline__ void drain_batch(const StreamCtx cx, uint32_t first, uint32_t n) {
+  const uint32_t lane = lane_here();
   const bool active = lane < n;
   uint32_t hits = 0, rank = 0;
   uint64_t g = 0;
@@ -269,7 +282,7 @@
         have_left = have_right = true;
       }
     }
-    uint32_t l1 = Probe<LOG2, WIDE>::template probe4<false>(cx.filter, cx.fold, cx.wa, cx.wb, cur);
+    uint32_t l1 = Probe<LOG2, WIDE, CTX>::template probe4<false>(cx.filter, cx.fold, cx.wa, cx.wb, cur, right, have_right ? 0xFFFFFFFFu : HG_CTX_EDGE_KEEP);
     if ((g << 4) + 16 > cx.nbytes) l1 &= (g << 4) < cx.nbytes ? (1u << static_cast<uint32_t>((cx.nbytes - (g << 4) + 3) >> 2)) - 1u : 0u;
     if (WIDE) {
       hits = l1;
@@ -281,7 +294,12 @@
         const uint32_t wp = k == 0 ? left : (k == 1 ? cur.x : (k == 2 ? cur.y : cur.z));
         const uint32_t wn = k == 0 ? cur.y : (k == 1 ? cur.z : (k == 2 ? cur.w : right));
         const uint32_t f = wk | cx.fold;
-        const HgSlotInfo info = cx.ext[(hg_dot4(f, cx.wa) & BYTE_MASK) >> 2];
+        const uint32_t sl = (hg_dot4(f, cx.wa) & BYTE_MASK) >> 2;
+        const HgSlotInfo info = cx.ext[sl];
+        if (CTX && info.many && !(info.nvalues > 0 && info.value[0] == f) && !(info.nvalues > 1 && info.value[1] == f)) {
+          const uint32_t *plain = reinterpret_cast<const uint32_t *>(cx.ext + (1u << LOG2));
+          if (!hg_slot_match(plain[sl], hg_hash_window(f))) continue;
+        }
         const uint32_t pm_keep = (k == 0 && !have_left) ? 0u : 0xFFFFFFFFu;
         const uint32_t nm_keep = (k == 3 && !have_right) ? (HG_WINDOW_BYTES == 4 ? 0u : 0xFFu) : 0xFFFFFFFFu;
         const uint32_t prev = wp | cx.fold;
@@ -313,43 +331,49 @@
   }
 }
 
-template <int LOG2, bool WIDE, int DENSE, bool FULL, int DEPTH, bool FOLD>
+template <int LOG2, bool WIDE, int DENSE, bool FULL, int DEPTH, bool FOLD, bool CTX>
 __device__ __forceinline__ void stream_tile(const StreamCtx &cx, uint64_t tile, HgTileSum *__restrict__ sums, uint32_t lane, uint32_t &qn) {
   const uint4 *__restrict__ text16 = cx.text16;
   const uint64_t nbytes = cx.nbytes;
-  const uint64_t chunk0 = tile * (HG_TILE_BYTES / 16) + lane;
+  constexpr bool LANE_KEPT = WIDE || DENSE != 0;
+  const uint32_t lane_tile = (!LANE_KEPT && !FULL) ? lane_here() : 0u;
+  auto lane_cold = [&]() -> uint32_t {
+    if constexpr (LANE_KEPT) return lane;
+    else if constexpr (!FULL) return lane_tile;
+    else return lane_here();
+  };
+  auto chunk_at = [&](int it) -> uint64_t { return tile * (HG_TILE_BYTES / 16) + static_cast<uint64_t>(it) * 64u + lane_cold(); };
 
   const __amdgpu_buffer_rsrc_t tile_rsrc = __builtin_amdgcn_make_buffer_rsrc(const_cast<uint4 *>(text16 + tile * (HG_TILE_BYTES / 16)), 0, HG_TILE_BYTES, 0x00020000);
   const uint32_t lane_off = lane * 16u;
   auto load_chunk = [&](int it) -> uint4 {
-    const uint64_t g = chunk0 + static_cast<uint64_t>(it) * 64u;
     if (FULL) {
-      if (WIDE) return text16[g];
+      if (WIDE) return text16[chunk_at(it)];
       if (DENSE) {
         typedef uint32_t u32x4 __attribute__((ext_vector_type(4)));
-        const u32x4 v = __builtin_nontemporal_load(reinterpret_cast<const u32x4 *>(text16) + g);
+        const u32x4 v = __builtin_nontemporal_load(reinterpret_cast<const u32x4 *>(text16) + chunk_at(it));
         return make_uint4(v.x, v.y, v.z, v.w);
       }
 #if defined(HG_NO_NT_LOADS)
-      return text16[g];
+      return text16[chunk_at(it)];
 #else
       typedef uint32_t u32x4 __attribute__((ext_vector_type(4)));
       const u32x4 v = __builtin_amdgcn_raw_buffer_load_b128(tile_rsrc, lane_off, it * 1024, 2);
       return make_uint4(v.x, v.y, v.z, v.w);
 #endif
     }
-    return load_chunk_checked(text16, nbytes, g);
+    return load_chunk_checked(text16, nbytes, chunk_at(it));
   };
 
   uint32_t seen = 0;
   uint32_t first_nl = HG_NONE32, last_nl = HG_NONE32;
   uint32_t first_it = 0, last_it = 0;
   uint64_t first_nlm = 0, last_nlm = 0;
-  const uint32_t lane_key = lane << 16;
+  const uint32_t keep3 = lane_off == 63u * 16u ? HG_CTX_EDGE_KEEP : 0xFFFFFFFFu;
 
   auto load_after = [&](int it) -> uint32_t {
     if (!DENSE || lane != 63u) return 0u;
-    return load_dword_checked(text16, nbytes, (chunk0 + static_cast<uint64_t>(it) * 64u + 1u) << 4);
+    return load_dword_checked(text16, nbytes, (chunk_at(it) + 1u) << 4);
   };
 
   auto body = [&](int it, uint4 cur, uint32_t after) {
@@ -365,6 +389,12 @@
     const bool has_nl = notnl != 128u, several_nl = notnl < 127u;
 #endif
 
+    uint32_t right = 0;
+#if defined(HG_ABLATE) && HG_ABLATE == 1
+    constexpr bool HAVE_RIGHT = false;
+#else
+    constexpr bool HAVE_RIGHT = CTX;
+#endif
 #if defined(HG_ABLATE) && HG_ABLATE == 1
     bool any = (cur.x ^ cur.y ^ cur.z ^ cur.w) == 0x12345678u;
     uint64_t am = __builtin_amdgcn_ballot_w64(any);
@@ -376,12 +406,13 @@
       any = ProbeBytes<LOG2, DENSE ? DENSE : 1>::template probe16<true>(cx.filter, cx.fold, cx.wa, cx.wb, cur, nxt) != 0;
       am = __builtin_amdgcn_ballot_w64(any);
     } else {
-      any = Probe<LOG2, WIDE>::template any4<FOLD>(cx.filter, cx.fold, cx.wa, cx.wb, cur, am);
+      if constexpr (CTX) right = __builtin_amdgcn_mov_dpp(FOLD ? cur.x | cx.fold : cur.x, 0x130 , 0xF, 0xF, true);
+      any = Probe<LOG2, WIDE, CTX>::template any4<FOLD>(cx.filter, cx.fold, cx.wa, cx.wb, cur, right, keep3, am);
     }
 #endif
 
     if constexpr (!FULL) {
-      any = any && ((chunk0 + static_cast<uint64_t>(it) * 64u) << 4) < nbytes;
+      any = any && (chunk_at(it) << 4) < nbytes;
       am = __builtin_amdgcn_ballot_w64(any);
     }
 
@@ -402,19 +433,19 @@
     }
     last_it = nlm ? static_cast<uint32_t>(it) : last_it;
     last_nlm = nlm ? nlm : last_nlm;
-    const uint32_t key = lane_key + opaque_sgpr(seen + (static_cast<uint32_t>(it) << 22));
+    const uint32_t key = (lane_off << 12) + opaque_sgpr(seen + (static_cast<uint32_t>(it) << 22));
     uint32_t total, e0 = 0;
     if (__builtin_expect(multi == 0, 1)) {
       total = __popcll(nlm);
       e0 = __builtin_amdgcn_mbcnt_hi(static_cast<uint32_t>(nlm >> 32), __builtin_amdgcn_mbcnt_lo(static_cast<uint32_t>(nlm), key));
     } else {
-      const uint32_t incl = wave_inclusive_scan(c, lane);
+      const uint32_t incl = wave_inclusive_scan<!LANE_KEPT>(c, lane_cold());
       total = __builtin_amdgcn_readlane(incl, 63);
       e0 = key + incl - c;
     }
     if (am) {
       const uint32_t left = __builtin_amdgcn_mov_dpp(cur.w, 0x138 , 0xF, 0xF, true);
-      const uint32_t right = __builtin_amdgcn_mov_dpp(cur.x, 0x130 , 0xF, 0xF, true);
+      if constexpr (!HAVE_RIGHT) right = __builtin_amdgcn_mov_dpp(cur.x, 0x130 , 0xF, 0xF, true);
       if (any) {
         const uint32_t idx = __builtin_amdgcn_mbcnt_hi(static_cast<uint32_t>(am >> 32), __builtin_amdgcn_mbcnt_lo(static_cast<uint32_t>(am), 0u));
         lds_u32 *e = (cx.queue + qn * queue_entry_dw(LOG2, DENSE)) + idx * queue_entry_dw(LOG2, DENSE);
@@ -433,7 +464,7 @@
       if (qn >= queue_cap(LOG2) - 64u) {
         const uint32_t n = qn < 64u ? qn : 64u;
         qn -= n;
-        drain_batch<LOG2, WIDE, DENSE>(cx, qn, n, lane);
+        drain_batch<LOG2, WIDE, DENSE, CTX>(cx, qn, n);
       }
     }
     seen += total;
@@ -467,7 +498,7 @@
     const uint4 v = load_chunk_checked(text16, nbytes, tile * (HG_TILE_BYTES / 16) + last_it * 64u + l);
     last_nl = last_it * 1024u + l * 16u + (31 - __clz(newline_bits16(v)));
   }
-  if (lane == 0) sums[tile] = HgTileSum{nl_count, first_nl, last_nl, nl_count ? nl_count - 1 : 0};
+  if (lane_off == 0) sums[tile] = HgTileSum{nl_count, first_nl, last_nl, nl_count ? nl_count - 1 : 0};
 }
 
 }
@@ -481,7 +512,7 @@
 #ifndef HG_DEPTH_SHARED
 #define HG_DEPTH_SHARED 3
 #endif
-template <int LOG2, bool WIDE, int DENSE, int DEPTH, bool JOIN, bool FOLD>
+template <int LOG2, bool WIDE, int DENSE, int DEPTH, bool JOIN, bool FOLD, bool CTX>
 __device__ __forceinline__ void stream_body(const uint4 *__restrict__ text16, uint64_t nbytes, uint64_t tile_begin, uint64_t tile_end, const uint4 *__restrict__ filter16,
                                             const uint4 *__restrict__ ext16, uint32_t fold, uint32_t wa, uint32_t wb, HgTileSum *__restrict__ sums, HgCand *__restrict__ cands,
                                             uint32_t seg_cap, uint32_t *__restrict__ seg_count, uint32_t *__restrict__ counters, uint32_t cursor_slot) {
@@ -520,11 +551,11 @@
     const uint32_t r1 = r0 + HG_STREAM_GRAB < ntile ? r0 + HG_STREAM_GRAB : ntile;
     if (JOIN) joined += r1 - r0;
     for (uint32_t r = r0 + wave; r < r1; r += WG_WAVES) {
-      if (r < nfull) stream_tile<LOG2, WIDE, DENSE, true, DEPTH, FOLD>(cx, tile_begin + r, sums, lane, qn);
-      else stream_tile<LOG2, WIDE, DENSE, false, DEPTH, FOLD>(cx, tile_begin + r, sums, lane, qn);
-    }
-  }
-  if (qn) drain_batch<LOG2, WIDE, DENSE>(cx, 0u, qn, lane);
+      if (r < nfull) stream_tile<LOG2, WIDE, DENSE, true, DEPTH, FOLD, CTX>(cx, tile_begin + r, sums, lane, qn);
+      else stream_tile<LOG2, WIDE, DENSE, false, DEPTH, FOLD, CTX>(cx, tile_begin + r, sums, lane, qn);
+    }
+  }
+  if (qn) drain_batch<LOG2, WIDE, DENSE, CTX>(cx, 0u, qn);
   __syncthreads();
   if (threadIdx.x == 0) {
     const uint32_t n = *cx.cand_count;
@@ -542,7 +573,7 @@
 #ifdef HG_STREAM_PRIO
   __builtin_amdgcn_s_setprio(HG_STREAM_PRIO);
 #endif
-  stream_body<LOG2, WIDE, DENSE, DEPTH, false, FOLD>(text16, nbytes, tile_begin, tile_end, filter16, ext16, fold, wa, wb, sums, cands, seg_cap, seg_count, counters, cursor_slot);
+  stream_body<LOG2, WIDE, DENSE, DEPTH, false, FOLD, !WIDE && DENSE == 0>(text16, nbytes, tile_begin, tile_end, filter16, ext16, fold, wa, wb, sums, cands, seg_cap, seg_count, counters, cursor_slot);
 }
 template <int LOG2, int DENSE, bool FOLD = true>
 __global__ __launch_bounds__(WG_THREADS) __attribute__((amdgpu_waves_per_eu(HG_STREAM_WAVES, 8))) void hg_stream_join_kernel(
@@ -552,7 +583,21 @@
 #ifdef HG_STREAM_PRIO
   __builtin_amdgcn_s_setprio(HG_STREAM_PRIO);
 #endif
-  stream_body<LOG2, false, DENSE, HG_DEPTH_SHARED, true, FOLD>(text16, nbytes, tile_begin, tile_end, filter16, ext16, fold, wa, wb, sums, cands, seg_cap, seg_count, counters, cursor_slot);
+  stream_body<LOG2, false, DENSE, HG_DEPTH_SHARED, true, FOLD, DENSE == 0>(text16, nbytes, tile_begin, tile_end, filter16, ext16, fold, wa, wb, sums, cands, seg_cap, seg_count, counters, cursor_slot);
+}
+template <int LOG2, int DEPTH, bool FOLD>
+__global__ __launch_bounds__(WG_THREADS) __attribute__((amdgpu_waves_per_eu(HG_STREAM_WAVES, 8))) void hg_stream_plain_kernel(
+    const uint4 *__restrict__ text16, uint64_t nbytes, uint64_t tile_begin, uint64_t tile_end, const uint4 *__restrict__ filter16, const uint4 *__restrict__ ext16, uint32_t fold,
+    uint32_t wa, uint32_t wb, HgTileSum *__restrict__ sums, HgCand *__restrict__ cands, uint32_t seg_cap, uint32_t *__restrict__ seg_count, uint32_t *__restrict__ counters,
+    uint32_t cursor_slot) {
+  stream_body<LOG2, false, 0, DEPTH, false, FOLD, false>(text16, nbytes, tile_begin, tile_end, filter16, ext16, fold, wa, wb, sums, cands, seg_cap, seg_count, counters, cursor_slot);
+}
+template <int LOG2, bool FOLD>
+__global__ __launch_bounds__(WG_THREADS) __attribute__((amdgpu_waves_per_eu(HG_STREAM_WAVES, 8))) void hg_stream_plain_join_kernel(
+    const uint4 *__restrict__ text16, uint64_t nbytes, uint64_t tile_begin, uint64_t tile_end, const uint4 *__restrict__ filter16, const uint4 *__restrict__ ext16, uint32_t fold,
+    uint32_t wa, uint32_t wb, HgTileSum *__restrict__ sums, HgCand *__restrict__ cands, uint32_t seg_cap, uint32_t *__restrict__ seg_count, uint32_t *__restrict__ counters,
+    uint32_t cursor_slot) {
+  stream_body<LOG2, false, 0, HG_DEPTH_SHARED, true, FOLD, false>(text16, nbytes, tile_begin, tile_end, filter16, ext16, fold, wa, wb, sums, cands, seg_cap, seg_count, counters, cursor_slot);
 }
 
 namespace {
@@ -562,6 +607,17 @@
   const uint4 *f = reinterpret_cast<const uint4 *>(a.filter);
   const uint4 *x = reinterpret_cast<const uint4 *>(a.ext);
   if constexpr (!W && !B) {
+    if (!a.ctx) {
+      if (a.db.fold_mask == 0)
+        hipLaunchKernelGGL((hg_stream_plain_kernel<L, D, false>), dim3(grid), dim3(WG_THREADS), 0, stream, t, a.nbytes, a.tile_begin, a.tile_end, f, x, a.db.fold_mask,
+                           a.weights_a, a.weights_b, a.sums, a.cands, a.cand_seg_cap, a.seg_count, a.counters, a.cursor_slot);
+      else
+        hipLaunchKernelGGL((hg_stream_plain_kernel<L, D, true>), dim3(grid), dim3(WG_THREADS), 0, stream, t, a.nbytes, a.tile_begin, a.tile_end, f, x, a.db.fold_mask,
+                           a.weights_a, a.weights_b, a.sums, a.cands, a.cand_seg_cap, a.seg_count, a.counters, a.cursor_slot);
+      return;
+    }
+  }
+  if constexpr (!W && !B) {
     if (a.db.fold_mask == 0) {
       hipLaunchKernelGGL((hg_stream_kernel<L, W, B, D, false>), dim3(grid), dim3(WG_THREADS), 0, stream, t, a.nbytes, a.tile_begin, a.tile_end, f, x, a.db.fold_mask,
                          a.weights_a, a.dense ? a.weights_c : a.weights_b, a.sums, a.cands, a.cand_seg_cap, a.seg_count, a.counters, a.cursor_slot);
@@ -586,6 +642,18 @@
 namespace {
 template <int L, int B>
 void launch_join(const HgStreamArgs &a, uint32_t grid, hipStream_t stream) {
+  if constexpr (B == 0) {
+    if (!a.ctx) {
+      const uint4 *t = reinterpret_cast<const uint4 *>(a.text), *f = reinterpret_cast<const uint4 *>(a.filter), *x = reinterpret_cast<const uint4 *>(a.ext);
+      if (a.db.fold_mask == 0)
+        hipLaunchKernelGGL((hg_stream_plain_join_kernel<L, false>), dim3(grid), dim3(WG_THREADS), 0, stream, t, a.nbytes, a.tile_begin, a.tile_end, f, x, a.db.fold_mask,
+                           a.weights_a, a.weights_b, a.sums, a.cands, a.cand_seg_cap, a.seg_count, a.counters, a.cursor_slot);
+      else
+        hipLaunchKernelGGL((hg_stream_plain_join_kernel<L, true>), dim3(grid), dim3(WG_THREADS), 0, stream, t, a.nbytes, a.tile_begin, a.tile_end, f, x, a.db.fold_mask,
+                           a.weights_a, a.weights_b, a.sums, a.cands, a.cand_seg_cap, a.seg_count, a.counters, a.cursor_slot);
+      return;
+    }
+  }
   if constexpr (B == 0) {
     if (a.db.fold_mask == 0) {
       hipLaunchKernelGGL((hg_stream_join_kernel<L, B, false>), dim3(grid), dim3(WG_THREADS), 0, stream, reinterpret_cast<const uint4 *>(a.text), a.nbytes, a.tile_begin, a.tile_end,
```

Result: faster. 5311 (median of 6 runs) (+5.2%).
